# xxlong0/NeuralUDF

Measured on AMD Instinct MI355X. Metric: ray-samples/sec (train step), higher is better.
Workload: dtype f32 emulated on the 16-bit matrix pipe, f32 accumulate, f32 state / epilogues / optimizer.  Forward-order sweeps (UDF value, input gradient, colour / NeRF forward): f16x2 (x = hi + 2^-11 lo in fp16, 3 fp16 MFMA products, correction terms in their own accumulator).  Backward sweeps (tangent, adjoint

## Files before the change

include/nudf.h:

```cpp
#ifndef NUDF_H
#define NUDF_H
#include <stdint.h>

#ifdef __cplusplus
extern "C" {
#endif

int nudf_version(void);
const char* nudf_last_error(void);

enum {
  NUDF_STATUS_NONFINITE_RENDER = 1,
  NUDF_STATUS_NONFINITE_SAMPLES = 2,
  NUDF_STATUS_NONFINITE_LOSS = 4
};
int nudf_set_status_flag(int32_t* device_word);
int32_t* nudf_status_flag(void);

enum {
  NUDF_EPI_NONE = 0,
  NUDF_EPI_SOFTPLUS = 1,
  NUDF_EPI_RELU = 2,
  NUDF_EPI_MUL = 3,
  NUDF_EPI_MULMASK = 4,
// ... 10 lines not shown
typedef struct NudfGemmNN {
  const float* A; int32_t lda;
  const float* B; int32_t ldb;
  const float* bias;
  float* C1; int32_t ldc1;
  float* C2; int32_t ldc2;
  float* C3; int32_t ldc3;
  const float* X1; int32_t ldx1;
  const float* X2; int32_t ldx2;
  int32_t M, N, K;
  int32_t epi;
  int32_t iparam;
  float scale;
  float xscale;
} NudfGemmNN;

int nudf_gemm_nn(const NudfGemmNN* args, void* stream);
int nudf_set_gemm_variant(int variant);

typedef struct NudfGemmTN {
  const float* A1; int32_t lda1; int32_t na1;
  const float* B1; int32_t ldb1;
  const float* A2; int32_t lda2; int32_t na2;
  const float* B2; int32_t ldb2;
  float* C; int32_t ldc;
  float* dbias;
  int32_t M, NA, NB;
  int32_t rows_per_block;
  int32_t prec;
} NudfGemmTN;

int nudf_gemm_tn(const NudfGemmTN* args, void* stream);

#define NUDF_TN_MAX_PROBLEMS 12
typedef struct NudfGemmTNProblem {
  const float* A1; const float* B1;
  float* C; float* dbias;
  int32_t lda1, ldb1, ldc, NA, NB;
  int32_t tile_start;
  int32_t flags;
} NudfGemmTNProblem;
#define NUDF_TN_A16 1
#define NUDF_TN_B16 2
#define NUDF_TN_A_BLK 4
#define NUDF_TN_B_BLK 8
#define NUDF_TN_A_P4 16
#define NUDF_TN_B_P4 32
typedef struct NudfGemmTNGroup {
  int32_t n_problems, M, rows_per_block, total_tiles;
  int32_t prec;
  NudfGemmTNProblem prob[NUDF_TN_MAX_PROBLEMS];
  float* workspace;
  int64_t workspace_floats;
  int32_t assign;
  const float* amax_a;
  const float* amax_b;
} NudfGemmTNGroup;
int nudf_gemm_tn_grouped(const NudfGemmTNGroup* args, void* stream);
int64_t nudf_gemm_tn_grouped_workspace(const NudfGemmTNGroup* args);
int nudf_gemm_tn_grouped_plan(const NudfGemmTNGroup* args, int32_t* out, int capacity);
int nudf_set_tn_flags(int flags);
int nudf_set_tn_debug(void* buf);


typedef struct NudfComposite {
  const float* rays_o; const float* rays_d;
  const float* z;
  const float* udf;
  const float* grad;
  const float* color;
  const float* color_base;
  const float* bg_z;
  const float* bg_sigma;
  const float* bg_color;
  const float* scal;
  const float* sample_dist;
  const float* background_rgb;
  int32_t N, S, n_out, s_nominal;
  int32_t has_anneal; float cos_anneal;
  float flip_saturation;
  int32_t use_norm_grad;
  float sparse_scale;
  int32_t alpha_type;
  float* weights;
  float* out_color; float* out_color_base;
  float* out_depth;
  float* out_normals;
  float* out_wsum; float* out_wsum_all;
  float* sums;
  float* ws;
  float* o_alpha; float* o_alpha_plus; float* o_alpha_minus; float* o_vis_prob;
  float* o_alpha_occ; float* o_raw_occ; float* o_true_cos; float* o_grad_mag;
  float* o_mid_z; float* o_dists; float* o_inside; float* o_flip;
  const float* sched;
  const float* p_variance; const float* p_beta; const float* p_gamma;
  float beta_hi;
  int32_t defer_sums;
  float* scal_out; float* recip_out;
} NudfComposite;

typedef struct NudfCompositeGrad {
  const float* d_color; const float* d_color_base;
  const float* d_weights;
  const float* d_depth;
  const float* d_normals;
  const float* d_wsum; const float* d_wsum_all;
  const float* d_sums;
  float* o_d_udf;
  float* o_d_grad;
  float* o_d_color; float* o_d_color_base;
  float* o_d_bg_sigma;
  float* o_d_bg_color;
  float* o_d_scal;
  float* ws;
  float* o_d_param;
} NudfCompositeGrad;

int nudf_composite_fwd(const NudfComposite* args, void* stream);
int nudf_composite_bwd(const NudfComposite* args, const NudfCompositeGrad* grads, void* stream);
int nudf_partial_sums(const float* ws, int nblk, int K, float* out, void* stream);
int nudf_composite_colour_finish(const float* sums_color, const float* sums_color_base, int N, int S,
                                 const float* background_rgb, const float* wsum_all, float* out_color,
                                 float* out_color_base, void* stream);
void nudf_set_composite_blocked(int on);

typedef struct NudfUpsample {
  const float* rays_o; const float* rays_d;
  const float* z; const float* udf;
  const float* u;
  const float* sample_dist;
  const float* gamma_dev;
  int32_t N, M, K, mode;
  float inv_s, beta, gamma;
  float* z_new;
  float* pts_new;
  float* dbg;
  const float* prev_z; const float* prev_udf;
  const float* add_z; const float* add_udf;
  float* z_merged; float* udf_merged;
  int32_t merge_K;
} NudfUpsample;
#define NUDF_UP_DBG_ROWS 7
#define NUDF_UP_THEORICAL 256
#define NUDF_UP_SERIAL 512
#define NUDF_UP_NOCONTRACT 1024
#define NUDF_UP_SLEEF 2048
#define NUDF_UP_EXPCR 4096
int nudf_upsample(const NudfUpsample* args, void* stream);
int nudf_merge(const float* z, const float* udf, const float* z_new, const float* udf_new, int N, int M,
               int K, float* z_out, float* udf_out, void* stream);
int nudf_merge_points(const float* z, const float* z_new, int N, int M, int K, float* z_out, const float* rays_o,
                      const float* rays_d, const float* sample_dist, float* pts, float* xrows, int ldx, int xcols,
                      void* stream);

typedef struct NudfPixelBlend {
  const float* pts;
  const float* logits; int32_t nl;
  const float* proj;
  const float* imgs;
  int32_t P, V, H, W;
  float* pix;
  int32_t img_layout;
} NudfPixelBlend;
int nudf_pixel_blend_fwd(const NudfPixelBlend* a, void* stream);
int nudf_pixel_blend_bwd(const NudfPixelBlend* a, const float* d_pix, float* d_logits, void* stream);

typedef struct NudfPixelComposite {
  const float* w;
  const float* pix;
  const float* pts;
  const float* bg_in;
  const float* bg_tail;
  int32_t N, S, n_out;
  float* out;
} NudfPixelComposite;
int nudf_pixel_composite_fwd(const NudfPixelComposite* a, void* stream);
int nudf_pixel_composite_bwd(const NudfPixelComposite* a, const float* d_out, float* d_w, float* d_pix,
                             float* d_bg_in, float* d_bg_tail, void* stream);

typedef struct NudfPatchBlend {
  const float* pts;
  const float* grad;
  const float* rays_d;
  const float* uv;
  const float* logits; int32_t nl;
  const float* w; int32_t ldw;
  const float* ref_cam;
  const float* src_cam;
  const float* imgs;
  int32_t N, S, V, H, W, hps;
  float* patch_colors;
  float* patch_mask;
  int32_t img_layout;
} NudfPatchBlend;
int nudf_patch_blend_fwd(const NudfPatchBlend* a, void* stream);
int nudf_patch_blend_bwd(const NudfPatchBlend* a, const float* d_patch, float* d_logits, float* d_w, void* stream);

int nudf_pixel_warp(const NudfPixelBlend* a , float* colors ,
                    float* mask , void* stream);
typedef struct NudfPatchWarp {
  const float* pts;
  const float* normals;
  const float* uv;
  const float* ref_cam;
  const float* src_cam;
  const float* imgs;
  int32_t N, S, V, H, W, hps, img_layout;
  float* colors;
  float* mask;
} NudfPatchWarp;
int nudf_patch_warp(const NudfPatchWarp* a, void* stream);

int nudf_ssim_patch(const float* pred, const float* gt, const float* window, int N, int Npx, float* out,
                    const float* d_out, float* d_pred, void* stream);
int nudf_patch_metric(int type, const float* pred, const float* gt, const float* window, int N, int Npx, float* out,
                      const float* d_out, float* d_pred, void* stream);

typedef struct NudfBlendLoss {
  const float* cb; const float* c; const float* pix; const float* gt;
  const float* err;
  const float* patch_mask;
  const float* weight_sum;
  const float* err_sorted;
  const int64_t* order;
  float* m;
  float* err_masked;
  float* sums;
  const float* sums_ws;
  const float* w_dev;
  float* out;
  const float* d_total;
  float* d_cb; float* d_c; float* d_pix;
  float* d_err;
  float* d_sums;
  int32_t N, sums_nblk;
  float n_rays, trim_ratio;
} NudfBlendLoss;
int nudf_blend_loss_prepare(const NudfBlendLoss* args, void* stream);
int nudf_blend_loss_fwd(const NudfBlendLoss* args, void* stream);
int nudf_blend_loss_bwd(const NudfBlendLoss* args, void* stream);

int nudf_coarse_z(const float* near, const float* far, int nf_stride, const float* t_rand, int N, int S,
                  float* z, float* sample_dist, void* stream);
int nudf_coarse_start(const float* near, const float* far, int nf_stride, const float* t_rand, int center, int N, int S,
                      float* z, float* sample_dist, const float* rays_o, const float* rays_d, float* pts, void* stream);
int nudf_outside_z(const float* far, int f_stride, const float* lin, int N, int n_out, int n_samples,
                   float* z_out, void* stream);
int nudf_ray_points(const float* rays_o, const float* rays_d, const float* z, const float* sample_dist, int N,
                    int S, int mode, float* pts, void* stream);

int nudf_posenc(const float* x, int xld, int xdiv, const float* tangent, int D, int L, float in_scale, int P,
                float* dst1, int ld1, float scale1, float* dst2, int ld2, float scale2, void* stream);
int nudf_posenc_vjp(const float* x, int xld, int D, int L, float in_scale, int P, const float* src1, int ld1,
                    float scale1, const float* src2, int ld2, float scale2, float* g, void* stream);
int nudf_copy_cols(const float* src, int lds, int sdiv, float* dst, int ldd, int ncols, int P, float scale,
                   void* stream);
int nudf_add_cols(const float* a, int lda, const float* b, int ldb, float* out, int ldo, int P, int C, void* stream);

int nudf_udf_grad_seed(const float* sign, const float* w_row0, const float* h, int ldh, float hscale, int P, int C,
                       float inv_scale, float* out, int ldo, void* stream);
int nudf_udf_head_bwd(const float* sign, const float* dudf, const float* dfeat, int ldf, int P, int F,
                      float scale, float* out, int ldo, void* stream);
int nudf_signed_colsum(const float* sign, const float* R, int ldr, int P, int C, float scale, float* out,
                       void* stream);
int nudf_sigmoid_head_bwd(const float* y, const float* dy, const float* dy_extra, int ldx, int nsig,
                          const float* draw, int ldr, int nraw, int P, float* out, int ldo, void* stream);

int nudf_weightnorm_pack(const float* v, const float* g, int out, int in, const int* perm, float* W, int ldw,
                         float* Wt, int ldwt, float* inv_norm, void* stream);
int nudf_weightnorm_unpack_grad(const float* dW, int ldw, const float* v, const float* g, const float* inv_norm,
                                int out, int in, const int* perm, float* dv, float* dg, void* stream);

#define NUDF_ADAM_MAX_TENSORS 64
#define NUDF_ADAM_MAX_GROUPS 4
typedef struct NudfAdamTensor {
  float* p; const float* g; float* m; float* v;
  int32_t n;
  int32_t group;
  float neg_step_size;
  float bc2_sqrt;
} NudfAdamTensor;
typedef struct NudfAdamGroup {
  float one_minus_beta1, beta2, one_minus_beta2, eps;
} NudfAdamGroup;
typedef struct NudfAdam {
  int32_t n_tensors; int32_t pad_;
  NudfAdamTensor t[NUDF_ADAM_MAX_TENSORS];
  int32_t block_start[NUDF_ADAM_MAX_TENSORS + 1];
  int32_t pad2_;
  NudfAdamGroup group[NUDF_ADAM_MAX_GROUPS];
  const float* dyn;
} NudfAdam;
int nudf_adam_step(const NudfAdam* args, void* stream);
int nudf_adam_chunk(void);

enum {
  NUDF_CH_NONE = 0,
  NUDF_CH_SOFTPLUS = 1,
  NUDF_CH_MULSP = 2,
  NUDF_CH_TANGENT = 3,
  NUDF_CH_BWD = 4,
  NUDF_CH_UDFHEAD = 5,
  NUDF_CH_RELU = 6,
  NUDF_CH_SIGMOIDN = 7,
  NUDF_CH_MULMASK = 8,
  NUDF_CH_ADDMASK = 9,
  NUDF_CH_RELUADD = 10
};
enum {
  NUDF_CH_INIT_LOAD = 0,
  NUDF_CH_INIT_POSENC = 1,
  NUDF_CH_INIT_SEED = 2
};
#define NUDF_CH_MAX_STEPS 14
typedef struct NudfChainStep {
  const float* Bp;
  const float* bias;
  const float* X1; const float* X2;
  float* C1; float* C2;
  const float* r1_row;
  const float* r1_col;
  int32_t K, N;
  int32_t epi;
  int32_t iparam;
  int32_t ldx1, ldx2, ldc1, ldc2;
  int32_t ldr1;
  int32_t prec;
  int32_t act_write;
  int32_t act_col0;
  int32_t pe_tail_col;
  int32_t ld_pe;
  float* pe_dst;
  float pe_tail_scale;
  float scale, xscale;
  int32_t layout;
  const float* row_w;
  float* row_sums;
  const float* X3;
  int32_t ldx3;
} NudfChainStep;
#define NUDF_CH_BLK_X1 1
#define NUDF_CH_BLK_X2 2
#define NUDF_CH_BLK_C1 4
#define NUDF_CH_BLK_C2 8
#define NUDF_CH_BLK_PE 16
#define NUDF_CH_STATE16 32
#define NUDF_CH_P4_X1 64
#define NUDF_CH_P4_C1 128
typedef struct NudfChain {
  int32_t P, n_steps;
  int32_t init;
  int32_t k0;
  int32_t x_div;
  int32_t tile_rows;
  int32_t lda0, ldg0;
  int32_t pe_L, pe_jvp;
  int32_t init_state16;
  float pe_in_scale;
  float seed_scale, seed_xscale;
  const float* A0;
  float* G0;
  const float* x;
  const float* v;
  const float* seed_sign;
  const float* seed_wrow;
  unsigned long long* dbg;
  float* absmax_out;
  const float* tile_amax_in;
  float* tile_amax_out;
  int32_t tile_scale;
  int32_t reserved0;
  NudfChainStep step[NUDF_CH_MAX_STEPS];
} NudfChain;
int nudf_mlp_chain(const NudfChain* args, void* stream);
int nudf_set_chain_t16(int on);
int nudf_pack_frag(const float* B, int ldb, int K, int N, float* out, void* stream);

#define NUDF_PACK_MAX_LAYERS 16
#define NUDF_PACK_MAX_FRAGS 4
typedef struct NudfPackFrag {
  float* dst;
  int32_t transpose;
  int32_t o0, i0;
  int32_t K, N;
  int32_t dtype;
} NudfPackFrag;
typedef struct NudfPackLayer {
  const float* v; const float* g;
  const int32_t* perm;
  float* W; float* Wt;
  float* inv_norm;
  int32_t out, in, ldw, ldwt;
  int32_t nfrag, row_start;
  NudfPackFrag frag[NUDF_PACK_MAX_FRAGS];
} NudfPackLayer;
typedef struct NudfPackMulti {
  int32_t n_layers, total_rows;
  NudfPackLayer layer[NUDF_PACK_MAX_LAYERS];
// ... 188 lines not shown
```

neuraludf_amd/_lib.py:

```python
from __future__ import annotations

import ctypes as C
import os

import torch

_HERE = os.path.dirname(os.path.abspath(__file__))
LIB_PATH = os.environ.get("NUDF_LIB") or os.path.join(_HERE, "libnudf.so")
ABI_VERSION = 108

c_fp = C.c_void_p
i32 = C.c_int32
f32 = C.c_float


class NudfError(RuntimeError):
    pass


class GemmNN(C.Structure):
    _fields_ = [("A", c_fp), ("lda", i32), ("B", c_fp), ("ldb", i32), ("bias", c_fp),
                ("C1", c_fp), ("ldc1", i32), ("C2", c_fp), ("ldc2", i32), ("C3", c_fp), ("ldc3", i32),
                ("X1", c_fp), ("ldx1", i32), ("X2", c_fp), ("ldx2", i32),
                ("M", i32), ("N", i32), ("K", i32), ("epi", i32), ("iparam", i32), ("scale", f32), ("xscale", f32)]


class GemmTN(C.Structure):
    _fields_ = [("A1", c_fp), ("lda1", i32), ("na1", i32), ("B1", c_fp), ("ldb1", i32),
                ("A2", c_fp), ("lda2", i32), ("na2", i32), ("B2", c_fp), ("ldb2", i32),
                ("C", c_fp), ("ldc", i32), ("dbias", c_fp), ("M", i32), ("NA", i32), ("NB", i32),
                ("rows_per_block", i32), ("prec", i32)]


TN_MAX_PROBLEMS = 12


class GemmTNProblem(C.Structure):
    _fields_ = [("A1", c_fp), ("B1", c_fp), ("C", c_fp), ("dbias", c_fp), ("lda1", i32), ("ldb1", i32), ("ldc", i32),
                ("NA", i32), ("NB", i32), ("tile_start", i32), ("flags", i32)]


class GemmTNGroup(C.Structure):
    _fields_ = [("n_problems", i32), ("M", i32), ("rows_per_block", i32), ("total_tiles", i32), ("prec", i32),
                ("prob", GemmTNProblem * TN_MAX_PROBLEMS), ("workspace", c_fp), ("workspace_floats", C.c_int64),
                ("assign", i32), ("amax_a", c_fp), ("amax_b", c_fp)]


class BlendLoss(C.Structure):
    _fields_ = [("cb", c_fp), ("c", c_fp), ("pix", c_fp), ("gt", c_fp), ("err", c_fp), ("patch_mask", c_fp),
                ("weight_sum", c_fp), ("err_sorted", c_fp), ("order", c_fp), ("m", c_fp), ("err_masked", c_fp), ("sums", c_fp),
                ("sums_ws", c_fp), ("w_dev", c_fp), ("out", c_fp), ("d_total", c_fp), ("d_cb", c_fp), ("d_c", c_fp),
                ("d_pix", c_fp), ("d_err", c_fp), ("d_sums", c_fp), ("N", i32), ("sums_nblk", i32), ("n_rays", f32),
                ("trim_ratio", f32)]


class RayBatch(C.Structure):
    _fields_ = [("image", c_fp), ("mask", c_fp), ("intrinsics_inv", c_fp), ("pose", c_fp), ("pixels_x", c_fp),
                ("pixels_y", c_fp), ("N", i32), ("H", i32), ("W", i32), ("h_patch_size", i32), ("rays", c_fp),
                ("ndc_uv", c_fp), ("xyz_cam", c_fp), ("near", c_fp), ("far", c_fp), ("patch_color", c_fp),
                ("patch_mask", c_fp)]


class Composite(C.Structure):
    _fields_ = [("rays_o", c_fp), ("rays_d", c_fp), ("z", c_fp), ("udf", c_fp), ("grad", c_fp),
                ("color", c_fp), ("color_base", c_fp), ("bg_z", c_fp), ("bg_sigma", c_fp), ("bg_color", c_fp),
                ("scal", c_fp), ("sample_dist", c_fp), ("background_rgb", c_fp),
                ("N", i32), ("S", i32), ("n_out", i32), ("s_nominal", i32),
                ("has_anneal", i32), ("cos_anneal", f32), ("flip_saturation", f32),
                ("use_norm_grad", i32), ("sparse_scale", f32), ("alpha_type", i32),
                ("weights", c_fp), ("out_color", c_fp), ("out_color_base", c_fp), ("out_depth", c_fp),
                ("out_normals", c_fp), ("out_wsum", c_fp), ("out_wsum_all", c_fp), ("sums", c_fp), ("ws", c_fp),
                ("o_alpha", c_fp), ("o_alpha_plus", c_fp), ("o_alpha_minus", c_fp), ("o_vis_prob", c_fp),
                ("o_alpha_occ", c_fp), ("o_raw_occ", c_fp), ("o_true_cos", c_fp), ("o_grad_mag", c_fp),
                ("o_mid_z", c_fp), ("o_dists", c_fp), ("o_inside", c_fp), ("o_flip", c_fp), ("sched", c_fp),
                ("p_variance", c_fp), ("p_beta", c_fp), ("p_gamma", c_fp), ("beta_hi", f32), ("defer_sums", i32),
                ("scal_out", c_fp), ("recip_out", c_fp)]


class CompositeGrad(C.Structure):
    _fields_ = [("d_color", c_fp), ("d_color_base", c_fp), ("d_weights", c_fp), ("d_depth", c_fp),
                ("d_normals", c_fp), ("d_wsum", c_fp), ("d_wsum_all", c_fp), ("d_sums", c_fp),
                ("o_d_udf", c_fp), ("o_d_grad", c_fp), ("o_d_color", c_fp), ("o_d_color_base", c_fp),
                ("o_d_bg_sigma", c_fp), ("o_d_bg_color", c_fp), ("o_d_scal", c_fp), ("ws", c_fp), ("o_d_param", c_fp)]


class Upsample(C.Structure):
    _fields_ = [("rays_o", c_fp), ("rays_d", c_fp), ("z", c_fp), ("udf", c_fp), ("u", c_fp),
                ("sample_dist", c_fp), ("gamma_dev", c_fp),
                ("N", i32), ("M", i32), ("K", i32), ("mode", i32),
                ("inv_s", f32), ("beta", f32), ("gamma", f32),
                ("z_new", c_fp), ("pts_new", c_fp), ("dbg", c_fp),
                ("prev_z", c_fp), ("prev_udf", c_fp), ("add_z", c_fp), ("add_udf", c_fp),
                ("z_merged", c_fp), ("udf_merged", c_fp), ("merge_K", i32)]


class PixelBlend(C.Structure):
    _fields_ = [("pts", c_fp), ("logits", c_fp), ("nl", i32), ("proj", c_fp), ("imgs", c_fp),
                ("P", i32), ("V", i32), ("H", i32), ("W", i32), ("pix", c_fp), ("img_layout", i32)]


class PixelComposite(C.Structure):
    _fields_ = [("w", c_fp), ("pix", c_fp), ("pts", c_fp), ("bg_in", c_fp), ("bg_tail", c_fp),
                ("N", i32), ("S", i32), ("n_out", i32), ("out", c_fp)]


class PatchBlend(C.Structure):
    _fields_ = [("pts", c_fp), ("grad", c_fp), ("rays_d", c_fp), ("uv", c_fp), ("logits", c_fp), ("nl", i32),
                ("w", c_fp), ("ldw", i32), ("ref_cam", c_fp), ("src_cam", c_fp), ("imgs", c_fp),
                ("N", i32), ("S", i32), ("V", i32), ("H", i32), ("W", i32), ("hps", i32),
                ("patch_colors", c_fp), ("patch_mask", c_fp), ("img_layout", i32)]


class PatchWarp(C.Structure):
    _fields_ = [("pts", c_fp), ("normals", c_fp), ("uv", c_fp), ("ref_cam", c_fp), ("src_cam", c_fp), ("imgs", c_fp),
                ("N", i32), ("S", i32), ("V", i32), ("H", i32), ("W", i32), ("hps", i32), ("img_layout", i32),
                ("colors", c_fp), ("mask", c_fp)]


ADAM_MAX_TENSORS = 64
ADAM_MAX_GROUPS = 4


class AdamTensor(C.Structure):
    _fields_ = [("p", c_fp), ("g", c_fp), ("m", c_fp), ("v", c_fp), ("n", i32), ("group", i32), ("neg_step_size", f32), ("bc2_sqrt", f32)]


class AdamGroup(C.Structure):
    _fields_ = [("one_minus_beta1", f32), ("beta2", f32), ("one_minus_beta2", f32), ("eps", f32)]


class Adam(C.Structure):
    _fields_ = [("n_tensors", i32), ("pad_", i32), ("t", AdamTensor * ADAM_MAX_TENSORS),
                ("block_start", i32 * (ADAM_MAX_TENSORS + 1)), ("pad2_", i32), ("group", AdamGroup * ADAM_MAX_GROUPS),
                ("dyn", c_fp)]


CH_MAX_STEPS = 14
CH_STATE16 = 32
CH_P4_X1, CH_P4_C1 = 64, 128
CH = dict(NONE=0, SOFTPLUS=1, MULSP=2, TANGENT=3, BWD=4, UDFHEAD=5, RELU=6, SIGMOIDN=7, MULMASK=8, ADDMASK=9, RELUADD=10)
CH_INIT = dict(LOAD=0, POSENC=1, SEED=2)


class ChainStep(C.Structure):
    _fields_ = [("Bp", c_fp), ("bias", c_fp), ("X1", c_fp), ("X2", c_fp), ("C1", c_fp), ("C2", c_fp),
                ("r1_row", c_fp), ("r1_col", c_fp), ("K", i32), ("N", i32), ("epi", i32), ("iparam", i32),
                ("ldx1", i32), ("ldx2", i32), ("ldc1", i32), ("ldc2", i32), ("ldr1", i32), ("prec", i32), ("act_write", i32),
                ("act_col0", i32), ("pe_tail_col", i32), ("ld_pe", i32), ("pe_dst", c_fp), ("pe_tail_scale", f32),
                ("scale", f32), ("xscale", f32), ("layout", i32), ("row_w", c_fp), ("row_sums", c_fp), ("X3", c_fp),
                ("ldx3", i32)]


class Chain(C.Structure):
    _fields_ = [("P", i32), ("n_steps", i32), ("init", i32), ("k0", i32), ("x_div", i32), ("tile_rows", i32), ("lda0", i32),
                ("ldg0", i32), ("pe_L", i32), ("pe_jvp", i32), ("init_state16", i32), ("pe_in_scale", f32), ("seed_scale", f32),
                ("seed_xscale", f32), ("A0", c_fp), ("G0", c_fp), ("x", c_fp), ("v", c_fp), ("seed_sign", c_fp),
                ("seed_wrow", c_fp), ("dbg", c_fp), ("absmax_out", c_fp), ("tile_amax_in", c_fp),
                ("tile_amax_out", c_fp), ("tile_scale", C.c_int32), ("reserved0", C.c_int32), ("step", ChainStep * CH_MAX_STEPS)]


PACK_MAX_LAYERS = 16
PACK_MAX_FRAGS = 4


class PackFrag(C.Structure):
    _fields_ = [("dst", c_fp), ("transpose", i32), ("o0", i32), ("i0", i32), ("K", i32), ("N", i32), ("dtype", i32)]


class PackLayer(C.Structure):
    _fields_ = [("v", c_fp), ("g", c_fp), ("perm", c_fp), ("W", c_fp), ("Wt", c_fp), ("inv_norm", c_fp),
                ("out", i32), ("in_", i32), ("ldw", i32), ("ldwt", i32), ("nfrag", i32), ("row_start", i32),
                ("frag", PackFrag * PACK_MAX_FRAGS)]


class PackMulti(C.Structure):
    _fields_ = [("n_layers", i32), ("total_rows", i32), ("layer", PackLayer * PACK_MAX_LAYERS)]


class UnpackLayer(C.Structure):
    _fields_ = [("dW", c_fp), ("v", c_fp), ("g", c_fp), ("inv_norm", c_fp), ("perm", c_fp), ("dv", c_fp),
                ("dg", c_fp), ("db_in", c_fp), ("db_out", c_fp), ("out", i32), ("in_", i32), ("ldw", i32), ("row_start", i32)]


class UnpackMulti(C.Structure):
    _fields_ = [("n_layers", i32), ("total_rows", i32), ("layer", UnpackLayer * PACK_MAX_LAYERS)]


class MeshUDF(C.Structure):
    _fields_ = [("U", c_fp), ("G", c_fp), ("axes", c_fp), ("cell_case", c_fp), ("cell_ntri", c_fp), ("edge_flag", c_fp),
                ("cells", c_fp), ("face_off", c_fp), ("edge_scan", c_fp), ("faces", c_fp), ("edges", c_fp), ("verts", c_fp),
                ("n_cells", C.c_int64), ("n_edges", C.c_int64), ("n_faces", C.c_int64), ("N", i32), ("mean_thr", f32),
                ("max_thr", f32), ("pad_", i32)]


class PointCloud(C.Structure):
    _fields_ = [("verts", c_fp), ("faces", c_fp), ("tri_n", c_fp), ("tri_off", c_fp), ("out", c_fp),
                ("n_verts", C.c_int64), ("n_faces", C.c_int64), ("n_out", C.c_int64), ("out_base", C.c_int64),
                ("cap", C.c_int64), ("density", C.c_double),
                ("pts", c_fp), ("n", C.c_int64), ("origin", C.c_double * 3), ("cell", C.c_double), ("grid", i32 * 3),
                ("pad_", i32), ("keys", c_fp), ("cell_key", c_fp), ("cell_start", c_fp), ("cell_count", c_fp),
                ("n_cells", C.c_int64), ("hash_key", c_fp), ("hash_row", c_fp), ("hash_cap", C.c_int64),
                ("rank", c_fp), ("state", c_fp), ("undecided", c_fp), ("r2", C.c_double),
                ("query", c_fp), ("query_idx", c_fp), ("n_query", C.c_int64), ("bound", C.c_double),
                ("box_bound2", C.c_double), ("box_lo", C.c_double * 3), ("box_hi", C.c_double * 3),
                ("dist", c_fp), ("idx", c_fp)]


class MeshTopo(C.Structure):
    _fields_ = [("faces", c_fp), ("he_key", c_fp), ("he_id", c_fp), ("edge_start", c_fp), ("edges", c_fp), ("he_edge", c_fp),
                ("edge_key", c_fp), ("nbr_off", c_fp), ("nbr", c_fp), ("bverts", c_fp), ("new_count", c_fp), ("new_off", c_fp),
                ("new_faces", c_fp), ("pos", c_fp), ("pos_out", c_fp), ("labels", c_fp), ("changed", c_fp), ("proj", c_fp),
                ("masks", c_fp), ("vis_count", c_fp), ("n_faces", C.c_int64), ("n_verts", C.c_int64), ("n_edges", C.c_int64),
                ("n_bverts", C.c_int64), ("n_new", C.c_int64), ("lam", C.c_double), ("max_loop", i32), ("n_views", i32),
                ("H", i32), ("W", i32), ("border", i32), ("pad_", i32)]


LW = dict(color_base=0, color=1, color_pixel=2, color_patch=3, igr=4, igr_ns=5, sparse=6, mask=7, color_sum=8)
LW_COUNT = 16

EPI = dict(NONE=0, SOFTPLUS=1, RELU=2, MUL=3, MULMASK=4, TANGENT=5, BWD=6, SIGMOID=7, UDFHEAD=8,
           SKIPSPLIT=9, RELU_DUAL=10, ADDMASK=11, MULSP=12)

SYMBOLS = [
    "nudf_version", "nudf_last_error", "nudf_set_status_flag", "nudf_status_flag", "nudf_gemm_nn", "nudf_set_gemm_variant", "nudf_gemm_tn", "nudf_gemm_tn_grouped", "nudf_gemm_tn_grouped_workspace", "nudf_gemm_tn_grouped_plan", "nudf_set_tn_flags", "nudf_patch_metric", "nudf_set_tn_debug", "nudf_composite_fwd",
    "nudf_composite_bwd", "nudf_partial_sums", "nudf_composite_colour_finish", "nudf_set_composite_blocked", "nudf_upsample", "nudf_merge", "nudf_merge_points", "nudf_coarse_z", "nudf_coarse_start", "nudf_outside_z",
    "nudf_ray_points", "nudf_posenc", "nudf_posenc_vjp", "nudf_copy_cols", "nudf_add_cols",
    "nudf_udf_grad_seed", "nudf_udf_head_bwd", "nudf_signed_colsum", "nudf_sigmoid_head_bwd",
    "nudf_weightnorm_pack", "nudf_weightnorm_unpack_grad",
    "nudf_pixel_blend_fwd", "nudf_pixel_blend_bwd", "nudf_pixel_composite_fwd", "nudf_pixel_composite_bwd",
    "nudf_patch_blend_fwd", "nudf_patch_blend_bwd", "nudf_ssim_patch", "nudf_pixel_warp", "nudf_patch_warp",
    "nudf_adam_step", "nudf_adam_chunk", "nudf_mlp_chain", "nudf_set_chain_t16", "nudf_pack_frag",
    "nudf_weightnorm_pack_multi", "nudf_weightnorm_unpack_grad_multi",
    "nudf_scalars_fwd", "nudf_scalars_bwd", "nudf_l1_sum_fwd", "nudf_l1_sum_bwd",
    "nudf_sums_errors_fwd", "nudf_sums_errors_bwd", "nudf_color_loss_fwd", "nudf_color_loss_bwd",
    "nudf_gen_ray_batch", "nudf_color_loss_sums", "nudf_color_loss_finish",
    "nudf_step_loss_fwd", "nudf_step_loss_bwd", "nudf_col0_seed4",
    "nudf_blend_loss_prepare", "nudf_blend_loss_fwd", "nudf_blend_loss_bwd",
    "nudf_meshudf_classify", "nudf_meshudf_emit", "nudf_meshudf_vertices",
    "nudf_pc_tri_count", "nudf_pc_tri_emit", "nudf_pc_keys", "nudf_pc_cells", "nudf_pc_thin_round", "nudf_pc_nearest",
    "nudf_meshtopo_edges", "nudf_meshtopo_fill_count", "nudf_meshtopo_fill_emit", "nudf_meshtopo_smooth",
    "nudf_meshtopo_cc_hook", "nudf_meshtopo_cc_jump", "nudf_meshtopo_views",
]

_P, _I, _F = C.c_void_p, C.c_int, C.c_float
_ARGTYPES = {
    "nudf_gemm_nn": [C.POINTER(GemmNN), _P],
    "nudf_gemm_tn": [C.POINTER(GemmTN), _P],
    "nudf_gemm_tn_grouped": [C.POINTER(GemmTNGroup), _P],
    "nudf_gemm_tn_grouped_workspace": [C.POINTER(GemmTNGroup)],
    "nudf_gemm_tn_grouped_plan": [C.POINTER(GemmTNGroup), C.POINTER(C.c_int32), i32],
    "nudf_set_tn_flags": [i32],
    "nudf_set_tn_debug": [_P],
    "nudf_composite_fwd": [C.POINTER(Composite), _P],
    "nudf_composite_bwd": [C.POINTER(Composite), C.POINTER(CompositeGrad), _P],
    "nudf_partial_sums": [_P, _I, _I, _P, _P],
    "nudf_composite_colour_finish": [_P, _P, _I, _I, _P, _P, _P, _P, _P],
    "nudf_upsample": [C.POINTER(Upsample), _P],
    "nudf_merge": [_P, _P, _P, _P, _I, _I, _I, _P, _P, _P],
    "nudf_coarse_z": [_P, _P, _I, _P, _I, _I, _P, _P, _P],
    "nudf_coarse_start": [_P, _P, _I, _P, _I, _I, _I, _P, _P, _P, _P, _P, _P],
    "nudf_merge_points": [_P, _P, _I, _I, _I, _P, _P, _P, _P, _P, _P, _I, _I, _P],
    "nudf_outside_z": [_P, _I, _P, _I, _I, _I, _P, _P],
    "nudf_ray_points": [_P, _P, _P, _P, _I, _I, _I, _P, _P],
    "nudf_posenc": [_P, _I, _I, _P, _I, _I, _F, _I, _P, _I, _F, _P, _I, _F, _P],
    "nudf_posenc_vjp": [_P, _I, _I, _I, _F, _I, _P, _I, _F, _P, _I, _F, _P, _P],
    "nudf_copy_cols": [_P, _I, _I, _P, _I, _I, _I, _F, _P],
    "nudf_add_cols": [_P, _I, _P, _I, _P, _I, _I, _I, _P],
    "nudf_udf_grad_seed": [_P, _P, _P, _I, _F, _I, _I, _F, _P, _I, _P],
    "nudf_udf_head_bwd": [_P, _P, _P, _I, _I, _I, _F, _P, _I, _P],
    "nudf_signed_colsum": [_P, _P, _I, _I, _I, _F, _P, _P],
    "nudf_sigmoid_head_bwd": [_P, _P, _P, _I, _I, _P, _I, _I, _I, _P, _I, _P],
    "nudf_weightnorm_pack": [_P, _P, _I, _I, _P, _P, _I, _P, _I, _P, _P],
    "nudf_weightnorm_unpack_grad": [_P, _I, _P, _P, _P, _I, _I, _P, _P, _P, _P],
    "nudf_pixel_blend_fwd": [C.POINTER(PixelBlend), _P],
    "nudf_pixel_blend_bwd": [C.POINTER(PixelBlend), _P, _P, _P],
    "nudf_pixel_composite_fwd": [C.POINTER(PixelComposite), _P],
    "nudf_pixel_composite_bwd": [C.POINTER(PixelComposite), _P, _P, _P, _P, _P, _P],
    "nudf_patch_blend_fwd": [C.POINTER(PatchBlend), _P],
    "nudf_patch_blend_bwd": [C.POINTER(PatchBlend), _P, _P, _P, _P],
    "nudf_pixel_warp": [C.POINTER(PixelBlend), _P, _P, _P],
    "nudf_patch_warp": [C.POINTER(PatchWarp), _P],
    "nudf_ssim_patch": [_P, _P, _P, _I, _I, _P, _P, _P, _P],
    "nudf_patch_metric": [_I] + [_P, _P, _P, _I, _I, _P, _P, _P, _P],
    "nudf_adam_step": [C.POINTER(Adam), _P],
    "nudf_mlp_chain": [C.POINTER(Chain), _P],
    "nudf_pack_frag": [_P, _I, _I, _I, _P, _P],
    "nudf_weightnorm_pack_multi": [C.POINTER(PackMulti), _P],
    "nudf_weightnorm_unpack_grad_multi": [C.POINTER(UnpackMulti), _P],
    "nudf_scalars_fwd": [_P, _P, _P, _F, _P, _P, _P],
    "nudf_scalars_bwd": [_P, _P, _P, _F, _P, _P, _P],
    "nudf_l1_sum_fwd": [_P, _P, _I, _P, _P],
    "nudf_l1_sum_bwd": [_P, _P, _I, _P, _P, _P],
    "nudf_sums_errors_fwd": [_P, _F, _P, _P],
    "nudf_sums_errors_bwd": [_P, _F, _P, _P, _P],
    "nudf_color_loss_fwd": [_P, _P, _P, _I, _P, _I, _F, _F, _F, _P, _P, _P, _P],
    "nudf_color_loss_bwd": [_P, _P, _P, _I, _P, _F, _F, _F, _P, _P, _P, _P, _P],
    "nudf_gen_ray_batch": [C.POINTER(RayBatch), _P],
    "nudf_color_loss_sums": [_P, _P, _P, _I, _P, _I, _P, _P],
    "nudf_color_loss_finish": [_P, _I, _F, _F, _F, _P, _P, _P, _P],
    "nudf_step_loss_fwd": [_P, _P, _P, _I, _P, _I, _P, _F, _F, _F, _F, _F, _F, _F, _P, _P, _P, _P, _I, _P],
    "nudf_step_loss_bwd": [_P, _P, _P, _I, _P, _P, _F, _F, _F, _F, _F, _F, _F, _P, _P, _P, _P, _P, _P, _P],
    "nudf_col0_seed4": [_P, _P, _F, _I, _I, _P, _P, _P],
    "nudf_blend_loss_prepare": [C.POINTER(BlendLoss), _P],
    "nudf_blend_loss_fwd": [C.POINTER(BlendLoss), _P],
    "nudf_blend_loss_bwd": [C.POINTER(BlendLoss), _P],
    "nudf_meshudf_classify": [C.POINTER(MeshUDF), _P],
    "nudf_meshudf_emit": [C.POINTER(MeshUDF), _P],
    "nudf_meshudf_vertices": [C.POINTER(MeshUDF), _P],
    **{n: [C.POINTER(PointCloud), _P] for n in ("nudf_pc_tri_count", "nudf_pc_tri_emit", "nudf_pc_keys", "nudf_pc_cells",
                                                "nudf_pc_thin_round", "nudf_pc_nearest")},
    **{n: [C.POINTER(MeshTopo), _P] for n in ("nudf_meshtopo_edges", "nudf_meshtopo_fill_count", "nudf_meshtopo_fill_emit",
                                              "nudf_meshtopo_smooth", "nudf_meshtopo_cc_hook", "nudf_meshtopo_cc_jump",
                                              "nudf_meshtopo_views")},
}

_lib = None


def _bind(l):
    for name, at in _ARGTYPES.items():
        fn = getattr(l, name)
        fn.argtypes = at
        fn.restype = C.c_int


def lib():
    global _lib
    if _lib is None:
        if not os.path.exists(LIB_PATH):
            raise NudfError(
                f"{LIB_PATH} not found: build it with `python -m neuraludf_amd.build` "
                "(the NeuralUDF hot path has no CPU/PyTorch fallback)")
        try:
            _lib = C.CDLL(LIB_PATH)
        except OSError as e:
            raise NudfError(f"cannot load {LIB_PATH}: {e}") from e
        _lib.nudf_last_error.restype = C.c_char_p
        _lib.nudf_version.restype = C.c_int
        _lib.nudf_adam_chunk.restype = C.c_int
        if _lib.nudf_version() != ABI_VERSION:
            v, _lib = _lib.nudf_version(), None
            raise NudfError(f"{LIB_PATH} is ABI version {v}, this package binds {ABI_VERSION}: rebuild with "
                            "`python -m neuraludf_amd.build --force`")
        _bind(_lib)
        _lib.nudf_gemm_tn_grouped_workspace.restype = C.c_int64
        _lib.nudf_set_chain_t16.argtypes = [C.c_int]
        _lib.nudf_set_chain_t16.restype = C.c_int
        _lib.nudf_set_status_flag.argtypes = [C.c_void_p]
        _lib.nudf_set_status_flag.restype = C.c_int
        _lib.nudf_status_flag.argtypes = []
        _lib.nudf_status_flag.restype = C.c_void_p
    return _lib


STATUS_NONFINITE_RENDER, STATUS_NONFINITE_SAMPLES, STATUS_NONFINITE_LOSS = 1, 2, 4
_STATUS_WORDS = {}
_STATUS_BOUND = None


def bind_status(dev):
    global _STATUS_BOUND
    if dev.type != "cuda":
        raise NudfError("libnudf kernels need device tensors (got a CPU tensor): run on an MI355X")
    idx = dev.index if dev.index is not None else torch.cuda.current_device()
    if _STATUS_BOUND == idx:
        return _STATUS_WORDS[idx]
    w = _STATUS_WORDS.get(idx)
    if w is None:
        w = torch.zeros(1, dtype=torch.int32, device=torch.device("cuda", idx))
        _STATUS_WORDS[idx] = w
    check(lib().nudf_set_status_flag(C.c_void_p(w.data_ptr())), "nudf_set_status_flag")
    _STATUS_BOUND = idx
    return w


def read_status(dev, clear=False):
    w = bind_status(dev)
    v = int(w.item())
    if clear and v:
        w.zero_()
    return v


def status_text(bits):
    names = [(STATUS_NONFINITE_SAMPLES, "non-finite new samples in the hierarchical re-sampling (nudf_upsample)"),
             (STATUS_NONFINITE_RENDER, "non-finite composited ray outputs or renderer scalars (nudf_composite_fwd)"),
             (STATUS_NONFINITE_LOSS, "non-finite loss (nudf_step_loss_fwd)")]
    return "; ".join(t for b, t in names if bits & b) or "finite"


def ptr(t):
    if t is None:
        return None
    if not t.is_cuda:
        raise NudfError("libnudf kernels need device tensors (got a CPU tensor): run on an MI355X")
    if not t.is_contiguous():
        raise NudfError("libnudf kernels need contiguous tensors")
    return t.data_ptr()


HOST_FAST = os.environ.get("NUDF_HOST_FAST", "1") != "0"
_raw_stream = getattr(torch._C, "_cuda_getCurrentRawStream", None)
_raw_device = getattr(torch._C, "_cuda_getDevice", None)


def stream():
    if HOST_FAST and _raw_stream is not None and _raw_device is not None:
        return C.c_void_p(_raw_stream(_raw_device()))
    return C.c_void_p(torch.cuda.current_stream().cuda_stream)


def check(rc, what=""):
    if rc != 0:
        msg = lib().nudf_last_error()
# ... 14 lines not shown
```

neuraludf_amd/csrc/rays_embed.hip:

```cpp
#include "nudf_common.h"
#include "../../include/nudf.h"

static inline int nblocks(long long n, int bs) { return (int)((n + bs - 1) / bs); }

__global__ void coarse_z_kernel(const float* near, const float* far, int nf_stride, const float* t_rand,
                                int N, int S, float* z) {
  int idx = blockIdx.x * blockDim.x + threadIdx.x;
  if (idx >= N * S) return;
  int r = idx / S, s = idx - r * S;
  float nr = near[r * nf_stride], fr = far[r * nf_stride];
  float step = 1.0f / (float)(S - 1);
  float t = (s < S / 2) ? s * step : 1.0f - (S - 1 - s) * step;
  float v = nr + (fr - nr) * t;
  if (t_rand) v = v + t_rand[r] * 2.0f / (float)S;
  z[idx] = v;
}

__global__ void sample_dist_kernel(const float* near, const float* far, int n, int S, float* out) {
  __shared__ float red[256];
  float acc = 0.f;
  for (int i = threadIdx.x; i < n; i += blockDim.x) acc += (far[i] - near[i]) / (float)S;
  red[threadIdx.x] = acc;
  __syncthreads();
  for (int s = 128; s > 0; s >>= 1) {
    if (threadIdx.x < s) red[threadIdx.x] += red[threadIdx.x + s];
    __syncthreads();
  }
  if (threadIdx.x == 0) out[0] = red[0] / (float)n;
}

extern "C" int nudf_coarse_z(const float* near, const float* far, int nf_stride, const float* t_rand, int N, int S,
                             float* z, float* sample_dist, void* stream) {
  hipStream_t st = (hipStream_t)stream;
  hipLaunchKernelGGL(coarse_z_kernel, dim3(nblocks((long long)N * S, 256)), dim3(256), 0, st, near, far, nf_stride,
                     t_rand, N, S, z);
  if (sample_dist)
    hipLaunchKernelGGL(sample_dist_kernel, dim3(1), dim3(256), 0, st, near, far, nf_stride ? N : 1, S, sample_dist);
  NUDF_CHECK_LAUNCH("nudf_coarse_z");
  return 0;
}

__global__ __launch_bounds__(256) void coarse_start_kernel(const float* near, const float* far, int nf_stride,
                                                           const float* t_rand, int center, int N, int S, float* z,
                                                           float* sample_dist, const float* __restrict__ o,
                                                           const float* __restrict__ d, float* __restrict__ pts) {
  const int idx = blockIdx.x * blockDim.x + threadIdx.x;
  if (idx < N * S) {
    const int r = idx / S, s = idx - r * S;
    const float nr = near[r * nf_stride], fr = far[r * nf_stride];
    const float step = 1.0f / (float)(S - 1);
    const float t = (s < S / 2) ? s * step : 1.0f - (S - 1 - s) * step;
    float v = nr + (fr - nr) * t;
    if (t_rand) {
      const float tr = center ? __fsub_rn(t_rand[r], 0.5f) : t_rand[r];
      v = v + tr * 2.0f / (float)S;
    }
    z[idx] = v;
    if (pts) {
      pts[(size_t)idx * 3 + 0] = o[r * 3 + 0] + d[r * 3 + 0] * v;
      pts[(size_t)idx * 3 + 1] = o[r * 3 + 1] + d[r * 3 + 1] * v;
      pts[(size_t)idx * 3 + 2] = o[r * 3 + 2] + d[r * 3 + 2] * v;
    }
  }
  if (blockIdx.x == 0 && sample_dist) {
    __shared__ float red[256];
    const int n = nf_stride ? N : 1;
    float acc = 0.f;
    for (int i = threadIdx.x; i < n; i += 256) acc += (far[i] - near[i]) / (float)S;
    red[threadIdx.x] = acc;
    __syncthreads();
    for (int s = 128; s > 0; s >>= 1) {
      if (threadIdx.x < s) red[threadIdx.x] += red[threadIdx.x + s];
      __syncthreads();
    }
    if (threadIdx.x == 0) sample_dist[0] = red[0] / (float)n;
  }
}
extern "C" int nudf_coarse_start(const float* near, const float* far, int nf_stride, const float* t_rand, int center, int N,
                                 int S, float* z, float* sample_dist, const float* rays_o, const float* rays_d, float* pts,
                                 void* stream) {
  if (N <= 0 || S < 2) {
    nudf_set_error("nudf_coarse_start: N >= 1 and S >= 2 required", hipErrorInvalidValue);
    return (int)hipErrorInvalidValue;
  }
  hipLaunchKernelGGL(coarse_start_kernel, dim3(nblocks((long long)N * S, 256)), dim3(256), 0, (hipStream_t)stream, near, far,
                     nf_stride, t_rand, center, N, S, z, sample_dist, rays_o, rays_d, pts);
  NUDF_CHECK_LAUNCH("nudf_coarse_start");
  return 0;
}

__global__ void outside_z_kernel(const float* far, int f_stride, const float* lin, int N, int n_out, float inv_ns,
                                 float* z_out) {
  int idx = blockIdx.x * blockDim.x + threadIdx.x;
  if (idx >= N * n_out) return;
  int r = idx / n_out, j = idx - r * n_out;
  z_out[idx] = far[r * f_stride] / lin[n_out - 1 - j] + inv_ns;
}
extern "C" int nudf_outside_z(const float* far, int f_stride, const float* lin, int N, int n_out, int n_samples,
                              float* z_out, void* stream) {
  hipLaunchKernelGGL(outside_z_kernel, dim3(nblocks((long long)N * n_out, 256)), dim3(256), 0, (hipStream_t)stream,
                     far, f_stride, lin, N, n_out, 1.0f / (float)n_samples, z_out);
  NUDF_CHECK_LAUNCH("nudf_outside_z");
  return 0;
}

__global__ void ray_points_kernel(const float* __restrict__ o, const float* __restrict__ d, const float* __restrict__ z,
                                  const float* sample_dist, int N, int S, int mode, float* __restrict__ pts) {
  int idx = blockIdx.x * blockDim.x + threadIdx.x;
  if (idx >= N * S) return;
  int r = idx / S, s = idx - r * S;
  float t = z[idx];
  if (mode >= 1) {
    float dist = (s < S - 1) ? (z[idx + 1] - t) : sample_dist[0];
    t = t + dist * 0.5f;
  }
  float px = o[r * 3 + 0] + d[r * 3 + 0] * t;
  float py = o[r * 3 + 1] + d[r * 3 + 1] * t;
  float pz = o[r * 3 + 2] + d[r * 3 + 2] * t;
  if (mode == 2) {
    float rr = sqrtf(px * px + py * py + pz * pz);
    rr = fminf(fmaxf(rr, 1.0f), 1e10f);
    pts[(size_t)idx * 4 + 0] = px / rr;
    pts[(size_t)idx * 4 + 1] = py / rr;
    pts[(size_t)idx * 4 + 2] = pz / rr;
    pts[(size_t)idx * 4 + 3] = 1.0f / rr;
  } else {
    pts[(size_t)idx * 3 + 0] = px;
    pts[(size_t)idx * 3 + 1] = py;
    pts[(size_t)idx * 3 + 2] = pz;
  }
}
extern "C" int nudf_ray_points(const float* rays_o, const float* rays_d, const float* z, const float* sample_dist, int N,
                               int S, int mode, float* pts, void* stream) {
  if (N * S == 0) return 0;
  hipLaunchKernelGGL(ray_points_kernel, dim3(nblocks((long long)N * S, 256)), dim3(256), 0, (hipStream_t)stream, rays_o,
                     rays_d, z, sample_dist, N, S, mode, pts);
  NUDF_CHECK_LAUNCH("nudf_ray_points");
  return 0;
}

__global__ void posenc_kernel(const float* __restrict__ x, int xld, int xdiv, const float* __restrict__ v, int D, int L,
                              float in_scale, int P, float* d1, int ld1, float s1, float* d2, int ld2, float s2,
                              int mode) {
  const int E = D * (2 * L + 1);
  long long idx = (long long)blockIdx.x * blockDim.x + threadIdx.x;
  if (idx >= (long long)P * E) return;
  int p = (int)(idx / E), e = (int)(idx - (long long)p * E);
  int blk = e / D, j = e - blk * D;
  float xv = x[(size_t)(p / xdiv) * xld + j] * in_scale;
  float val;
  if (blk == 0) {
    val = (mode == 0) ? xv : v[(size_t)p * D + j] * in_scale;
  } else {
    int k = (blk - 1) >> 1;
    float f = (float)(1 << k);
    float a = xv * f;
    bool is_sin = ((blk - 1) & 1) == 0;
    if (mode == 0) val = is_sin ? sinf(a) : cosf(a);
    else val = (is_sin ? cosf(a) : -sinf(a)) * f * v[(size_t)p * D + j] * in_scale;
  }
  if (d1) d1[(size_t)p * ld1 + e] = val * s1;
  if (d2) d2[(size_t)p * ld2 + e] = val * s2;
}
extern "C" int nudf_posenc(const float* x, int xld, int xdiv, const float* tangent, int D, int L, float in_scale, int P,
                           float* dst1, int ld1, float scale1, float* dst2, int ld2, float scale2, void* stream) {
  if (P == 0) return 0;
  const int E = D * (2 * L + 1);
  hipLaunchKernelGGL(posenc_kernel, dim3(nblocks((long long)P * E, 256)), dim3(256), 0, (hipStream_t)stream, x, xld,
                     xdiv, tangent, D, L, in_scale, P, dst1, ld1, scale1, dst2, ld2, scale2, tangent ? 1 : 0);
  NUDF_CHECK_LAUNCH("nudf_posenc");
  return 0;
}

#define PV_PTS 64
#define PV_MAXE 96
__global__ __launch_bounds__(256) void posenc_vjp_kernel(const float* __restrict__ x, int xld, int D, int L,
                                                         float in_scale, int P, const float* __restrict__ s1, int ld1,
                                                         float c1, const float* __restrict__ s2, int ld2, float c2,
                                                         float* __restrict__ g) {
  __shared__ float de[PV_PTS][PV_MAXE + 1];
  const int E = D * (2 * L + 1);
  const int p0 = blockIdx.x * PV_PTS;
  for (int idx = threadIdx.x; idx < PV_PTS * E; idx += 256) {
    const int r = idx / E, e = idx - r * E;
    const int p = min(p0 + r, P - 1);
    float t = 0.f;
    if (s1) t += s1[(size_t)p * ld1 + e] * c1;
    if (s2) t += s2[(size_t)p * ld2 + e] * c2;
    de[r][e] = t;
  }
  __syncthreads();
  for (int idx = threadIdx.x; idx < PV_PTS * D; idx += 256) {
    const int r = idx / D, j = idx - r * D;
    const int p = p0 + r;
    if (p >= P) continue;
    const float xv = x[(size_t)p * xld + j] * in_scale;
    float acc = de[r][j];
    for (int k = 0; k < L; ++k) {
      const float f = (float)(1 << k);
      float sn, cs;
      sincosf(xv * f, &sn, &cs);
      acc += f * (de[r][D * (1 + 2 * k) + j] * cs - de[r][D * (2 + 2 * k) + j] * sn);
    }
    g[(size_t)p * D + j] = acc * in_scale;
  }
}
extern "C" int nudf_posenc_vjp(const float* x, int xld, int D, int L, float in_scale, int P, const float* src1, int ld1,
                               float scale1, const float* src2, int ld2, float scale2, float* g, void* stream) {
  if (P == 0) return 0;
  if (D * (2 * L + 1) > PV_MAXE) {
    nudf_set_error("nudf_posenc_vjp: encoding wider than 96", hipErrorInvalidValue);
    return (int)hipErrorInvalidValue;
  }
  hipLaunchKernelGGL(posenc_vjp_kernel, dim3(nblocks(P, PV_PTS)), dim3(256), 0, (hipStream_t)stream, x, xld, D, L,
                     in_scale, P, src1, ld1, scale1, src2, ld2, scale2, g);
  NUDF_CHECK_LAUNCH("nudf_posenc_vjp");
  return 0;
}

__global__ void copy_cols_kernel(const float* __restrict__ src, int lds, int sdiv, float* __restrict__ dst, int ldd,
                                 int ncols, int P, float scale) {
  long long idx = (long long)blockIdx.x * blockDim.x + threadIdx.x;
  if (idx >= (long long)P * ncols) return;
  int p = (int)(idx / ncols), c = (int)(idx - (long long)p * ncols);
  dst[(size_t)p * ldd + c] = src[(size_t)(p / sdiv) * lds + c] * scale;
}
extern "C" int nudf_copy_cols(const float* src, int lds, int sdiv, float* dst, int ldd, int ncols, int P, float scale,
                              void* stream) {
  if (P == 0) return 0;
  hipLaunchKernelGGL(copy_cols_kernel, dim3(nblocks((long long)P * ncols, 256)), dim3(256), 0, (hipStream_t)stream, src,
                     lds, sdiv, dst, ldd, ncols, P, scale);
  NUDF_CHECK_LAUNCH("nudf_copy_cols");
  return 0;
}

__global__ void udf_grad_seed_kernel(const float* __restrict__ sign, const float* __restrict__ wrow,
                                     const float* __restrict__ h, int ldh, float hscale, int P, int C,
                                     float inv_scale, float* __restrict__ out, int ldo) {
  long long idx = (long long)blockIdx.x * blockDim.x + threadIdx.x;
  if (idx >= (long long)P * C) return;
// ... 904 lines not shown
```

neuraludf_amd/csrc/upsample.hip:

```cpp
#include "nudf_common.h"
#include "../../include/nudf.h"

#define UP_MAX_M 512
#define UP_NC (UP_MAX_M / 64)

namespace up_fast {
#include "upsample_body.inc"
}
#pragma clang fp contract(off)
namespace up_exact {
#include "upsample_body.inc"
}
#pragma clang fp contract(fast)

extern "C" int nudf_upsample(const NudfUpsample* args, void* stream) {
  const NudfUpsample& p = *args;
  if (p.N <= 0) return 0;
  if (p.M < 2 || p.M > UP_MAX_M || p.K < 1) {
    nudf_set_error("nudf_upsample: 2 <= M <= 512 and K >= 1 required", hipErrorInvalidValue);
    return (int)hipErrorInvalidValue;
  }
  if (p.merge_K < 0 || p.merge_K >= p.M ||
      (p.merge_K > 0 && (!p.prev_z || !p.prev_udf || !p.add_z || !p.add_udf || !p.z_merged || !p.udf_merged))) {
    nudf_set_error("nudf_upsample: merge_K in [0, M) with all six merge arrays required", hipErrorInvalidValue);
    return (int)hipErrorInvalidValue;
  }
  dim3 grid((p.N + 3) / 4), block(256);
  hipStream_t st = (hipStream_t)stream;
  const int nc = (p.M + 63) / 64;
  int32_t* status = nudf_status_flag();
  if (p.mode & NUDF_UP_NOCONTRACT) {
    switch (nc) {
      case 1: hipLaunchKernelGGL(up_exact::upsample_kernel<1>, grid, block, 0, st, p, status); break;
      case 2: hipLaunchKernelGGL(up_exact::upsample_kernel<2>, grid, block, 0, st, p, status); break;
      case 3: hipLaunchKernelGGL(up_exact::upsample_kernel<3>, grid, block, 0, st, p, status); break;
      case 4: hipLaunchKernelGGL(up_exact::upsample_kernel<4>, grid, block, 0, st, p, status); break;
      default: hipLaunchKernelGGL(up_exact::upsample_kernel<8>, grid, block, 0, st, p, status); break;
    }
  } else {
    switch (nc) {
      case 1: hipLaunchKernelGGL(up_fast::upsample_kernel<1>, grid, block, 0, st, p, status); break;
      case 2: hipLaunchKernelGGL(up_fast::upsample_kernel<2>, grid, block, 0, st, p, status); break;
      case 3: hipLaunchKernelGGL(up_fast::upsample_kernel<3>, grid, block, 0, st, p, status); break;
      case 4: hipLaunchKernelGGL(up_fast::upsample_kernel<4>, grid, block, 0, st, p, status); break;
      default: hipLaunchKernelGGL(up_fast::upsample_kernel<8>, grid, block, 0, st, p, status); break;
    }
  }
  NUDF_CHECK_LAUNCH("nudf_upsample");
  return 0;
}

__global__ __launch_bounds__(256) void merge_kernel(const float* __restrict__ za, const float* __restrict__ ua,
                                                    const float* __restrict__ zb, const float* __restrict__ ub, int N,
                                                    int M, int K, float* __restrict__ zo, float* __restrict__ uo) {
  extern __shared__ float sm[];
  const int wave = threadIdx.x >> 6, l = threadIdx.x & 63;
  const int ray = blockIdx.x * 4 + wave;
  if (ray >= N) return;
  float* a = sm + wave * (M + K);
  float* b = a + M;
  for (int i = l; i < M; i += 64) a[i] = za[(size_t)ray * M + i];
  for (int j = l; j < K; j += 64) b[j] = zb[(size_t)ray * K + j];
  __builtin_amdgcn_wave_barrier();
  __threadfence_block();
  const size_t ob = (size_t)ray * (M + K);
  for (int i = l; i < M; i += 64) {
    const float v = a[i];
    int lo = 0, hi = K;
    while (lo < hi) {
      const int mid = (lo + hi) >> 1;
      if (b[mid] < v) lo = mid + 1; else hi = mid;
    }
    zo[ob + i + lo] = v;
    if (uo) uo[ob + i + lo] = ua[(size_t)ray * M + i];
  }
  for (int j = l; j < K; j += 64) {
    const float v = b[j];
    int lo = 0, hi = M;
    while (lo < hi) {
      const int mid = (lo + hi) >> 1;
      if (a[mid] <= v) lo = mid + 1; else hi = mid;
    }
    zo[ob + j + lo] = v;
    if (uo) uo[ob + j + lo] = ub[(size_t)ray * K + j];
  }
}

extern "C" int nudf_merge(const float* z, const float* udf, const float* z_new, const float* udf_new, int N, int M,
                          int K, float* z_out, float* udf_out, void* stream) {
  if (N <= 0) return 0;
  const size_t lds = (size_t)4 * (M + K) * sizeof(float);
  if (lds > 64 * 1024) {
    nudf_set_error("nudf_merge: M + K too large", hipErrorInvalidValue);
    return (int)hipErrorInvalidValue;
  }
  hipLaunchKernelGGL(merge_kernel, dim3((N + 3) / 4), dim3(256), lds, (hipStream_t)stream, z, udf, z_new, udf_new, N, M,
                     K, z_out, udf_out);
  NUDF_CHECK_LAUNCH("nudf_merge");
  return 0;
}

__global__ __launch_bounds__(256) void merge_points_kernel(const float* __restrict__ za, const float* __restrict__ zb,
                                                           int N, int M, int K, float* __restrict__ zo,
                                                           const float* __restrict__ ro, const float* __restrict__ rd,
                                                           const float* __restrict__ sample_dist,
                                                           float* __restrict__ pts, float* __restrict__ xrows, int ldx,
                                                           int xcols) {
  extern __shared__ float sm[];
  const int wave = threadIdx.x >> 6, l = threadIdx.x & 63;
  const int ray = blockIdx.x * 4 + wave;
  if (ray >= N) return;
  const int S = M + K;
  float* a = sm + wave * (5 * S);
  float* b = a + M;
  float* out = a + S;
  float* pl = out + S;
  for (int i = l; i < M; i += 64) a[i] = za[(size_t)ray * M + i];
  for (int j = l; j < K; j += 64) b[j] = zb[(size_t)ray * K + j];
  __builtin_amdgcn_wave_barrier();
  __threadfence_block();
  for (int i = l; i < M; i += 64) {
    const float v = a[i];
    int lo = 0, hi = K;
    while (lo < hi) {
      const int mid = (lo + hi) >> 1;
      if (b[mid] < v) lo = mid + 1; else hi = mid;
    }
    out[i + lo] = v;
  }
  for (int j = l; j < K; j += 64) {
    const float v = b[j];
    int lo = 0, hi = M;
    while (lo < hi) {
      const int mid = (lo + hi) >> 1;
      if (a[mid] <= v) lo = mid + 1; else hi = mid;
    }
    out[j + lo] = v;
  }
  __builtin_amdgcn_wave_barrier();
  __threadfence_block();
  const float ox = ro[ray * 3 + 0], oy = ro[ray * 3 + 1], oz = ro[ray * 3 + 2];
  const float dx = rd[ray * 3 + 0], dy = rd[ray * 3 + 1], dz = rd[ray * 3 + 2];
  const float sd = sample_dist[0];
  const size_t ob = (size_t)ray * S;
  for (int i = l; i < S; i += 64) {
    float t = out[i];
    zo[ob + i] = t;
    const float dist = (i < S - 1) ? (out[i + 1] - t) : sd;
    t = t + dist * 0.5f;
    const float px = ox + dx * t, py = oy + dy * t, pz = oz + dz * t;
    pts[(ob + i) * 3 + 0] = px;
    pts[(ob + i) * 3 + 1] = py;
    pts[(ob + i) * 3 + 2] = pz;
    pl[3 * i + 0] = px; pl[3 * i + 1] = py; pl[3 * i + 2] = pz;
  }
  if (xrows) {
    __builtin_amdgcn_wave_barrier();
    __threadfence_block();
    for (int e = l; e < S * xcols; e += 64) {
      const int r = e / xcols, c = e - r * xcols;
      xrows[(ob + r) * (size_t)ldx + c] = (c < 3) ? pl[3 * r + c] : 0.0f;
    }
  }
}

extern "C" int nudf_merge_points(const float* z, const float* z_new, int N, int M, int K, float* z_out, const float* rays_o,
                                 const float* rays_d, const float* sample_dist, float* pts, float* xrows, int ldx, int xcols,
                                 void* stream) {
  if (N <= 0) return 0;
  const size_t lds = (size_t)4 * 5 * (M + K) * sizeof(float);
  if (lds > 64 * 1024 || M < 1 || K < 0 || (xrows && (xcols < 3 || xcols > ldx))) {
    nudf_set_error("nudf_merge_points: M + K <= 819, 3 <= xcols <= ldx required", hipErrorInvalidValue);
    return (int)hipErrorInvalidValue;
  }
  hipLaunchKernelGGL(merge_points_kernel, dim3((N + 3) / 4), dim3(256), lds, (hipStream_t)stream, z, z_new, N, M, K, z_out,
                     rays_o, rays_d, sample_dist, pts, xrows, ldx, xcols);
  NUDF_CHECK_LAUNCH("nudf_merge_points");
  return 0;
}
```

neuraludf_amd/csrc/upsample_body.inc:

```
__device__ __forceinline__ float clip01u(float x) { return fminf(fmaxf(x, 0.0f), 1.0f); }

__device__ __forceinline__ float sleef_expf_u10(float d) {
  const int q = __float2int_rn(__fmul_rn(d, 1.442695040888963407359924681001892137426645954152985934135449406931f));
  const float qf = (float)q;
  float s = __fmaf_rn(qf, -0.693145751953125f, d);
  s = __fmaf_rn(qf, -1.428606765330187045e-06f, s);
  float u = 0.000198527617612853646278381f;
  u = __fmaf_rn(u, s, 0.00139304355252534151077271f);
  u = __fmaf_rn(u, s, 0.00833336077630519866943359f);
  u = __fmaf_rn(u, s, 0.0416664853692054748535156f);
  u = __fmaf_rn(u, s, 0.166666671633720397949219f);
  u = __fmaf_rn(u, s, 0.5f);
  u = __fadd_rn(1.0f, __fmaf_rn(__fmul_rn(s, s), u, s));
  const int e1 = q >> 1, e2 = q - e1;
  u = __fmul_rn(__fmul_rn(u, __int_as_float((e1 + 127) << 23)), __int_as_float((e2 + 127) << 23));
  if (d < -104.0f) u = 0.0f;
  if (d > 100.0f) u = __int_as_float(0x7f800000);
  return u;
}
__device__ __forceinline__ float up_sigmoid(float x, bool sleef) {
  return sleef ? __fdiv_rn(1.0f, __fadd_rn(1.0f, sleef_expf_u10(-x))) : sigmoidf_(x);
}

__device__ __forceinline__ float up_exp(float x, bool cr) { return cr ? (float)exp((double)x) : expf(x); }

__device__ __forceinline__ float sdf2alpha_plain(float sdf, float cosv, float dist, float inv_s, int theorical, bool sleef,
                                                 bool expcr) {
  if (theorical) {
    const float raw = fabsf(cosv) * inv_s * (1.0f - up_sigmoid(sdf * inv_s, sleef));
    return 1.0f - up_exp(-fmaxf(raw, 0.0f) * dist, expcr);
  }
  const float en = sdf + cosv * dist * 0.5f;
  const float ep = sdf - cosv * dist * 0.5f;
  const float P = up_sigmoid(ep * inv_s, sleef);
  const float Nx = up_sigmoid(en * inv_s, sleef);
  return clip01u((P - Nx + 1e-5f) / (P + 1e-5f));
}

__device__ __forceinline__ void up_serial_excl_prod(float* buf, int n, int lane) {
  __builtin_amdgcn_wave_barrier();
  __threadfence_block();
  if (lane == 0) {
    double acc = 1.0;
    int i = 0;
#pragma unroll 2
    for (; i + 4 <= n; i += 4) {
      const float4 q = *reinterpret_cast<const float4*>(buf + i);
      float4 o;
      o.x = (float)acc; acc *= (double)q.x;
      o.y = (float)acc; acc *= (double)q.y;
      o.z = (float)acc; acc *= (double)q.z;
      o.w = (float)acc; acc *= (double)q.w;
      *reinterpret_cast<float4*>(buf + i) = o;
    }
    for (; i < n; ++i) {
      const float q = buf[i];
      buf[i] = (float)acc;
      acc *= (double)q;
    }
  }
  __builtin_amdgcn_wave_barrier();
  __threadfence_block();
}

template <int NC>
__global__ __launch_bounds__(256) void upsample_kernel(NudfUpsample p, int32_t* status) {
  __shared__ __attribute__((aligned(16))) float s_z[4][NC * 64];
  __shared__ __attribute__((aligned(16))) float s_cdf[4][NC * 64];
  __shared__ float s_u[4][NC * 64];
  const int wave = threadIdx.x >> 6, l = threadIdx.x & 63;
  const int ray = blockIdx.x * 4 + wave;
  if (ray >= p.N) return;
  const int M = p.M;
  float* zs = s_z[wave];
  float* cdf = s_cdf[wave];

  const float ox = p.rays_o[ray * 3 + 0], oy = p.rays_o[ray * 3 + 1], oz = p.rays_o[ray * 3 + 2];
  const float dx = p.rays_d[ray * 3 + 0], dy = p.rays_d[ray * 3 + 1], dz = p.rays_d[ray * 3 + 2];
  const float sdist = p.sample_dist[0];
  const float gamma = p.gamma_dev ? p.gamma_dev[0] : p.gamma;
  const bool serial = (p.mode & NUDF_UP_SERIAL) != 0;
  const bool sleef = (p.mode & NUDF_UP_SLEEF) != 0;
  const bool expcr = (p.mode & NUDF_UP_EXPCR) != 0;
  float* dbg = p.dbg ? p.dbg + (size_t)ray * NUDF_UP_DBG_ROWS * M : nullptr;

  const bool merged = p.merge_K > 0;
  if (merged) {
    const int K0 = p.merge_K, M0 = M - K0;
    float* a = cdf;
    float* b = cdf + M0;
    float* us = s_u[wave];
    for (int i = l; i < M0; i += 64) a[i] = p.prev_z[(size_t)ray * M0 + i];
    for (int j = l; j < K0; j += 64) b[j] = p.add_z[(size_t)ray * K0 + j];
    __builtin_amdgcn_wave_barrier();
    __threadfence_block();
    for (int i = l; i < M0; i += 64) {
      const float v = a[i];
      int lo = 0, hi = K0;
      while (lo < hi) {
        const int mid = (lo + hi) >> 1;
        if (b[mid] < v) lo = mid + 1; else hi = mid;
      }
      zs[i + lo] = v;
      us[i + lo] = p.prev_udf[(size_t)ray * M0 + i];
    }
    for (int j = l; j < K0; j += 64) {
      const float v = b[j];
      int lo = 0, hi = M0;
      while (lo < hi) {
        const int mid = (lo + hi) >> 1;
        if (a[mid] <= v) lo = mid + 1; else hi = mid;
      }
      zs[j + lo] = v;
      us[j + lo] = p.add_udf[(size_t)ray * K0 + j];
    }
    __builtin_amdgcn_wave_barrier();
    __threadfence_block();
  }
  float z[NC], u[NC], rad[NC];
#pragma unroll
  for (int c = 0; c < NC; ++c) {
    const int i = c * 64 + l;
    z[c] = 0.f; u[c] = 0.f; rad[c] = 1e30f;
    if (i < M) {
      if (merged) {
        z[c] = zs[i];
        u[c] = s_u[wave][i];
        p.z_merged[(size_t)ray * M + i] = z[c];
        p.udf_merged[(size_t)ray * M + i] = u[c];
      } else {
        z[c] = p.z[(size_t)ray * M + i];
        u[c] = p.udf[(size_t)ray * M + i];
      }
      const float px = ox + dx * z[c], py = oy + dy * z[c], pz = oz + dz * z[c];
      rad[c] = sqrtf(px * px + py * py + pz * pz);
      zs[i] = z[c];
    }
  }

  float w[NC];
  const int theorical = (p.mode >> 8) & 1;
  if ((p.mode & 0xff) == 1) {
#pragma unroll
    for (int c = 0; c < NC; ++c) {
      const int i = c * 64 + l;
      const float zo = (c + 1 < NC) ? wave_bcast(z[(c + 1 < NC) ? c + 1 : c], 0) : 0.f;
      const float zn = wave_shift_down1(z[c], zo);
      const float dist = (i < M - 1) ? (zn - z[c]) : sdist;
      const float e = up_exp(-p.beta * u[c], expcr);
      const float raw = p.beta * e / ((1.0f + e) * (1.0f + e)) * gamma;
      w[c] = (i < M - 1) ? (1.0f - up_exp(-fmaxf(raw, 0.0f) * dist, expcr)) : 0.0f;
    }
  } else {
    float tc[NC], cosv[NC], aocc[NC], dists[NC], midu[NC];
#pragma unroll
    for (int c = 0; c < NC; ++c) {
      const int i = c * 64 + l;
      const int cn = (c + 1 < NC) ? c + 1 : c;
      const float zo = wave_bcast(z[cn], 0), uo = wave_bcast(u[cn], 0), ro = wave_bcast(rad[cn], 0);
      const float zn = wave_shift_down1(z[c], zo), un = wave_shift_down1(u[c], uo), rn = wave_shift_down1(rad[c], ro);
      const bool sec = i < M - 1;
      dists[c] = sec ? (zn - z[c]) : 0.f;
      midu[c] = (u[c] + un) * 0.5f;
      tc[c] = sec ? (un - u[c]) / (zn - z[c] + 1e-5f) : 0.f;
      const bool inside = (rad[c] < 1.0f) || (rn < 1.0f);
      cosv[c] = inside ? 1.0f : 0.0f;
      const float draw = sec ? (zn - z[c]) : sdist;
      const float e = up_exp(-p.beta * u[c], expcr);
      const float raw = p.beta * e / ((1.0f + e) * (1.0f + e));
      aocc[c] = 1.0f - up_exp(-fmaxf(raw, 0.0f) * gamma * draw, expcr);
    }
    float carry = 1.0f;
    float vis[NC];
#pragma unroll
    for (int c = 0; c < NC; ++c) {
      const int i = c * 64 + l;
      const float cur = -fabsf(tc[c]);
      const int cp = (c > 0) ? c - 1 : c;
      const float prev_o = wave_bcast(-fabsf(tc[cp]), 63), tprev_o = wave_bcast(tc[cp], 63);
      const float prev = wave_shift_up1(cur, (c > 0) ? prev_o : 0.0f);
      const float tprev = wave_shift_up1(tc[c], tprev_o);
      const float inside = cosv[c];
      float cv = fminf(prev, cur);
      cv = fminf(fmaxf(cv, -1e3f), 0.0f) * inside;
      cosv[c] = cv;
      const float vm = (i == 0) ? 1.0f : ((tprev < 0.05f) ? 1.0f : 0.0f);
      const float q = (i < M) ? (clip01u(1.0f - aocc[c] + vm) + 1e-7f) : 1.0f;
      if (serial) {
        if (i < M) cdf[i] = q;
      } else {
        float inc = wave_incl_scan_mul(q) * carry;
        const float exc = wave_shift_up1(inc, carry);
        carry = wave_bcast(inc, 63);
        vis[c] = exc;
      }
    }
    if (serial) {
      up_serial_excl_prod(cdf, M, l);
#pragma unroll
      for (int c = 0; c < NC; ++c) vis[c] = (c * 64 + l < M) ? cdf[c * 64 + l] : 1.0f;
      __builtin_amdgcn_wave_barrier();
      __threadfence_block();
    }
    carry = 1.0f;
#pragma unroll
    for (int c = 0; c < NC; ++c) {
      const int i = c * 64 + l;
      float alpha = 0.f;
      if (i < M - 1) {
        const float ap = sdf2alpha_plain(midu[c], cosv[c], dists[c], p.inv_s, theorical, sleef, expcr);
        const float am = sdf2alpha_plain(-midu[c], cosv[c], dists[c], p.inv_s, theorical, sleef, expcr);
        alpha = ap * vis[c] + am * (1.0f - vis[c]);
        if (dbg) {
          dbg[0 * M + i] = cosv[c]; dbg[1 * M + i] = vis[c]; dbg[2 * M + i] = ap; dbg[3 * M + i] = am;
          dbg[4 * M + i] = alpha;
        }
      }
      const float f = (i < M - 1) ? (1.0f - alpha + 1e-7f) : 1.0f;
      if (serial) {
        if (i < M - 1) cdf[i] = f;
        w[c] = alpha;
      } else {
        float inc = wave_incl_scan_mul(f) * carry;
        const float exc = wave_shift_up1(inc, carry);
        carry = wave_bcast(inc, 63);
        w[c] = (i < M - 1) ? alpha * exc : 0.0f;
      }
    }
    if (serial) {
      up_serial_excl_prod(cdf, M - 1, l);
#pragma unroll
      for (int c = 0; c < NC; ++c) w[c] = (c * 64 + l < M - 1) ? w[c] * cdf[c * 64 + l] : 0.0f;
      __builtin_amdgcn_wave_barrier();
      __threadfence_block();
    }
  }

  float tot = 0.f;
#pragma unroll
  for (int c = 0; c < NC; ++c) {
    const int i = c * 64 + l;
    if (dbg && i < M - 1) dbg[5 * M + i] = w[c];
    w[c] = (i < M - 1) ? (w[c] + 1e-5f) : 0.0f;
    tot += w[c];
  }
  tot = wave_sum(tot);
  float scarry = 0.f;
  if (l == 0) cdf[0] = 0.f;
#pragma unroll
  for (int c = 0; c < NC; ++c) {
    const int i = c * 64 + l;
    const float pdf = w[c] / tot;
    if (serial) {
      if (i < M - 1) cdf[i + 1] = pdf;
    } else {
      float inc = wave_incl_scan_add(pdf) + scarry;
      scarry = wave_bcast(inc, 63);
      if (i < M - 1) cdf[i + 1] = inc;
    }
  }
  __builtin_amdgcn_wave_barrier();
  __threadfence_block();
  if (serial) {
    if (l == 0) {
      double acc = 0.0;
      int i = 1;
#pragma unroll 2
      for (; i + 4 <= M; i += 4) {
        const float a0 = cdf[i], a1 = cdf[i + 1], a2 = cdf[i + 2], a3 = cdf[i + 3];
        acc += (double)a0; const float o0 = (float)acc;
        acc += (double)a1; const float o1 = (float)acc;
        acc += (double)a2; const float o2 = (float)acc;
        acc += (double)a3; const float o3 = (float)acc;
        cdf[i] = o0; cdf[i + 1] = o1; cdf[i + 2] = o2; cdf[i + 3] = o3;
      }
      for (; i < M; ++i) {
        acc += (double)cdf[i];
        cdf[i] = (float)acc;
      }
    }
    __builtin_amdgcn_wave_barrier();
    __threadfence_block();
  }

  if (dbg)
    for (int i = l; i < M; i += 64) dbg[6 * M + i] = cdf[i];
  for (int k = l; k < p.K; k += 64) {
    const float uq = p.u[k];
    int lo = 0, hi = M;
    while (lo < hi) {
      const int mid = (lo + hi) >> 1;
      if (cdf[mid] <= uq) lo = mid + 1; else hi = mid;
    }
    const int below = max(lo - 1, 0);
    const int above = min(lo, M - 1);
    const float c0 = cdf[below], c1 = cdf[above];
    const float b0 = zs[below], b1 = zs[above];
    float den = c1 - c0;
    if (den < 1e-5f) den = 1.0f;
    const float t = (uq - c0) / den;
    const float zn = b0 + t * (b1 - b0);
    p.z_new[(size_t)ray * p.K + k] = zn;
    if (status && !(fabsf(zn) <= 3.0e38f)) atomicOr(status, NUDF_STATUS_NONFINITE_SAMPLES);
    if (p.pts_new) {
      const size_t o = ((size_t)ray * p.K + k) * 3;
      p.pts_new[o + 0] = ox + dx * zn;
      p.pts_new[o + 1] = oy + dy * zn;
      p.pts_new[o + 2] = oz + dz * zn;
    }
  }
}
```

neuraludf_amd/mlp.py:

```python
from __future__ import annotations

import math
from typing import List, Optional

import ctypes as C

import torch

from . import _lib
import os

from ._lib import CH, CH_INIT, CH_MAX_STEPS, EPI, Chain, GemmNN, GemmTN, call, ptr


def pad32(n: int) -> int:
    return (n + 31) // 32 * 32


def pad_rows(P: int) -> int:
    return (P + 63) // 64 * 64


def _buf(P, width, dev, zero=None, dtype=torch.float32, blocked=False):
    if blocked:
        assert zero is False and dtype == torch.float32
        t = torch.empty((pad_rows(P), pad32(width)), device=dev, dtype=dtype)
        t._nudf_blk = True
        return t
    ld = pad32(width)
    if dtype == torch.bfloat16:
        t = (torch.zeros if zero else torch.empty)((pad_rows(P), ld), device=dev, dtype=dtype)
        if zero is None and ld != width:
            t.view(pad_rows(P) // 4, ld, 4)[:, width:, :].zero_()
        t._nudf_p4 = True
        return t
    if zero is None:
        t = torch.empty((pad_rows(P), ld), device=dev, dtype=dtype)
        if ld != width:
            t[:, width:].zero_()
        return t
    return (torch.zeros if zero else torch.empty)((pad_rows(P), ld), device=dev, dtype=dtype)


def _is16(t):
    return t is not None and t.dtype == torch.bfloat16


def _isblk(t):
    return t is not None and getattr(t, "_nudf_blk", False)


def _isp4(t):
    return t is not None and getattr(t, "_nudf_p4", False)


def pack16(t):
    R, ld = t.shape
    assert R % 4 == 0
    b = t.to(torch.bfloat16).reshape(R // 4, 4, ld).permute(0, 2, 1).reshape(R, ld).contiguous()
    b._nudf_p4 = True
    return b


def unpack16(t):
    R, ld = t.shape
    assert _isp4(t) and R % 4 == 0
    return t.reshape(R // 4, ld, 4).permute(0, 2, 1).reshape(R, ld).float()


def block(t):
    R, ld = t.shape
    assert R % 32 == 0 and ld % 4 == 0 and t.dtype == torch.float32
    b = t.reshape(R // 32, 32, ld // 4, 4).permute(0, 2, 1, 3).reshape(R, ld).contiguous()
    b._nudf_blk = True
    return b


def unblock(t):
    if not _isblk(t):
        return t
    R, ld = t.shape
    return t.reshape(R // 32, ld // 4, 32, 4).permute(0, 2, 1, 3).reshape(R, ld).contiguous()


def _zero_cols(t, c0):
    if c0 < t.shape[1]:
        t[:, c0:].zero_()
    return t


def alloc_grads(layers, zero=True):
    sizes = [(pl.out_pad * pl.in_pad, pl.out_pad) for pl in layers]
    flat = (torch.zeros if zero else torch.empty)(sum(a + b for a, b in sizes), device=layers[0].W.device)
    out, off = [], 0
    for pl, (a, b) in zip(layers, sizes):
        dW = flat[off:off + a].view(pl.out_pad, pl.in_pad)
        db = flat[off + a:off + a + pl.out]
        out.append((dW, db))
        off += a + b
    return out


def gemm_nn(A, B, M, N, K, epi, C1=None, ldc1=0, C2=None, ldc2=0, C3=None, ldc3=0, X1=None, ldx1=0, X2=None, ldx2=0,
            bias=None, lda=None, ldb=None, iparam=0, scale=1.0, xscale=1.0, c1_off=0, c2_off=0, x1_off=0, x2_off=0):
    a = GemmNN()
    a.A, a.lda = ptr(A), (lda if lda is not None else A.shape[1])
    a.B, a.ldb = ptr(B), (ldb if ldb is not None else B.shape[1])
    a.bias = ptr(bias)
    a.C1 = (ptr(C1) + 4 * c1_off) if C1 is not None else None
    a.ldc1 = ldc1 or (C1.shape[1] if (C1 is not None and C1.dim() == 2) else 0)
    a.C2 = (ptr(C2) + 4 * c2_off) if C2 is not None else None
    a.ldc2 = ldc2 or (C2.shape[1] if (C2 is not None and C2.dim() == 2) else 0)
    a.C3 = ptr(C3)
    a.ldc3 = ldc3 or (C3.shape[1] if (C3 is not None and C3.dim() == 2) else 0)
    a.X1 = (ptr(X1) + 4 * x1_off) if X1 is not None else None
    a.ldx1 = ldx1 or (X1.shape[1] if (X1 is not None and X1.dim() == 2) else 0)
    a.X2 = (ptr(X2) + 4 * x2_off) if X2 is not None else None
    a.ldx2 = ldx2 or (X2.shape[1] if (X2 is not None and X2.dim() == 2) else 0)
    a.M, a.N, a.K, a.epi, a.iparam, a.scale, a.xscale = M, N, K, EPI[epi], iparam, scale, xscale
    if PROFILE is not None:
        _timed("gemm_nn", 2.0 * M * N * getattr(B, "k_true", K), lambda: call("nudf_gemm_nn", a))
        return
    call("nudf_gemm_nn", a)


MFMA_PRODUCTS = {0: 1, 1: 1, 2: 1, 3: 6, 4: 3}

PROFILE = None


def _timed(name, flops, fn, detail=None, nbytes=0.0, xflops=None):
    s = torch.cuda.Event(enable_timing=True)
    e = torch.cuda.Event(enable_timing=True)
    s.record()
    fn()
    e.record()
    PROFILE.append((name, flops, s, e, detail or name, nbytes, xflops))


def call_timed(cls, detail, nbytes, name, *args, units=0.0):
    if PROFILE is None:
        call(name, *args)
    else:
        _timed(cls, -float(units), lambda: call(name, *args), detail, float(nbytes))


def gemm_tn(A1, na1, B1, C, NA, NB, M, dbias=None, A2=None, na2=0, B2=None):
    for t in (A1, B1, A2, B2):
        if t is not None and (_is16(t) or _isblk(t)):
            raise _lib.NudfError("gemm_tn: bf16-stored / blocked-layout operands need gemm_tn_grouped (per-problem "
                                 "NUDF_TN_A16 / _B16 / _A_BLK / _B_BLK flags); set NUDF_STATE16=0 / NUDF_BLOCKED_STATE=0 "
                                 "with NUDF_UDF_TN_GROUPED=0")
    a = GemmTN()
    a.A1, a.lda1, a.na1 = ptr(A1), A1.shape[1], na1
    a.B1, a.ldb1 = ptr(B1), B1.shape[1]
    if A2 is not None:
        a.A2, a.lda2, a.na2 = ptr(A2), A2.shape[1], na2
        a.B2, a.ldb2 = ptr(B2), B2.shape[1]
    a.C, a.ldc = ptr(C), C.shape[1]
    a.dbias = ptr(dbias)
    a.M, a.NA, a.NB, a.rows_per_block = M, NA, NB, 0
    a.prec = _tn_prec()
    if PROFILE is not None:
        _timed("gemm_tn", 2.0 * M * NA * NB * (2 if A2 is not None else 1), lambda: call("nudf_gemm_tn", a))
        return
    call("nudf_gemm_tn", a)


USE_CHAIN = os.environ.get("NUDF_CHAIN", "1") != "0"
CHAIN_DEBUG = None
CHAIN_TILE = int(os.environ.get("NUDF_CHAIN_TILE", "0"))
COLOR_TILE = int(os.environ.get("NUDF_COLOR_TILE", "0"))


def k8(n: int) -> int:
    return (n + 15) // 16 * 16


def pack_frag(B, ldb, K, N, off=0):
    out = torch.empty(k8(K) // 8 * ((N + 31) // 32) * 256, device=B.device, dtype=torch.float32)
    call("nudf_pack_frag", ptr(B) + 4 * off, ldb, K, N, ptr(out))
    out.k_true, out.n_true = K, N
    return out


_PLAIN_TYPES = frozenset((int, float, str, bool, type(None)))
_CHAIN_MEMO = {}
CHAIN_MEMO = os.environ.get("NUDF_CHAIN_MEMO", "1") != "0" and _lib.HOST_FAST
chain_memo_hits = 0


def _memo_token(engine):
    t = engine.__dict__.get("_site_token")
    if t is None:
        t = engine.__dict__["_site_token"] = object()
    return t


class ChainBuilder:

    def __init__(self, P, init, k0, tile_rows=0, site=None):
        self.P, self.init, self.k0, self.tile_rows = P, init, k0, (tile_rows or CHAIN_TILE)
        self.site = site
        self.rec = []
        self.c = None
        self.n = 0
        self.flops = 0.0
        self.xflops = 0.0
        self.nbytes = 0.0
        self.epis = []
        self.blocked = False
        self.keep = []

    def posenc(self, *a, **kw):
        self.rec.append((0, a, kw))

    def init_store(self, *a, **kw):
        self.rec.append((1, a, kw))

    def init_load(self, *a, **kw):
        self.rec.append((2, a, kw))

    def init_seed(self, *a, **kw):
        self.rec.append((3, a, kw))

    def step(self, *a, **kw):
        self.rec.append((4, a, kw))

    def absmax(self, *a, **kw):
        self.rec.append((5, a, kw))

    def tile_scale(self, *a, **kw):
        self.rec.append((6, a, kw))

    _PARAMS = (("x", "L", "in_scale", "tangent", "x_div"), ("G0",), ("A0", "lda0"),
               ("A0", "lda0", "sign", "wrow", "scale", "xscale"), ("epi", "Bp", "K", "N"), ("t",), ("amax_in", "amax_out"))
    _CHAIN_FIELD = ({"x": "x", "tangent": "v"}, {"G0": "G0"}, {"A0": "A0"}, {"A0": "A0", "sign": "seed_sign", "wrow": "seed_wrow"},
                    None, {"t": "absmax_out"}, {"amax_in": "tile_amax_in", "amax_out": "tile_amax_out"})

    def _signature(self):
        T, PT, plain = torch.Tensor, torch.nn.Parameter, _PLAIN_TYPES
        sig = [self.P, self.init, self.k0, self.tile_rows, PRECISION, FWD_F16X2, BWD_F16X2, HEAD16, STATE16, BLOCKED_STATE, TN_SPLIT]
        ptrs = []
        add, addp = sig.append, ptrs.append
        for kind, a, kw in self.rec:
            add(kind)
            for vals in (a, kw.values()):
                for v in vals:
                    tv = type(v)
                    if tv in plain:
                        add(v)
                    elif tv is T or tv is PT or isinstance(v, T):
                        if not (v.is_cuda and v.is_contiguous()):
                            return None, None
                        addp(v.data_ptr())
                        add(v.numel())
                    else:
                        add(v)
            add(tuple(kw))
        return sig, ptrs

    def _fill(self):
        self.c = Chain()
        self.c.P, self.c.init, self.c.k0, self.c.tile_rows = self.P, CH_INIT[self.init], self.k0, self.tile_rows
        self.c.x_div = 1
        fns = (self._do_posenc, self._do_init_store, self._do_init_load, self._do_init_seed, self._do_step, self._do_absmax,
               self._do_tile_scale)
        T = torch.Tensor
        slots = []
        for kind, a, kw in self.rec:
            n0 = self.n
            fns[kind](*a, **kw)
            obj = self.c.step[n0] if kind == 4 else self.c
            names = list(self._PARAMS[kind][:len(a)]) + list(kw)
            vals = list(a) + list(kw.values())
            for nm, v in zip(names, vals):
                if isinstance(v, T):
                    field = nm if kind == 4 else self._CHAIN_FIELD[kind][nm]
                    cur = getattr(obj, field)
                    slots.append((obj, field, cur - v.data_ptr()) if cur is not None else None)
        return slots

    def _p(self, t, off=0):
        if t is None:
            return None
        self.keep.append(t)
        return ptr(t) + t.element_size() * off

    def _do_posenc(self, x, L, in_scale, tangent=None, x_div=1):
        self.c.x, self.c.v = self._p(x), self._p(tangent)
# ... 619 lines not shown
    def mark_stale(self):
        for pl in self.layers:
            pl._ver = None

    def _embed(self, x, P, X, tangent=None):
        net = self.net
        skip_dst = [X[s] for s in sorted(self.skip)]
        d2 = skip_dst[0] if skip_dst else None
        off2 = (self.layers[sorted(self.skip)[0]].inp - self.E) if skip_dst else 0
        call("nudf_posenc", ptr(x), 3, 1, ptr(tangent), net.d_in, net.multires, float(net.scale), P,
             ptr(X[0]), X[0].shape[1], 1.0,
             (ptr(d2) + 4 * off2) if d2 is not None else None, d2.shape[1] if d2 is not None else 0, self.inv_sqrt2)
        for s, dst in zip(sorted(self.skip)[1:], skip_dst[1:]):
            off = self.layers[s].inp - self.E
            call("nudf_posenc", ptr(x), 3, 1, ptr(tangent), net.d_in, net.multires, float(net.scale), P,
                 ptr(dst) + 4 * off, dst.shape[1], self.inv_sqrt2, None, 0, 0.0)

    def _chain_ok(self):
        net = self.net
        widths_ok = all(pl.out <= 256 and pl.inp <= 256 for pl in self.layers[:-1]) and self.layers[-1].inp <= 256 \
            and self.layers[-1].out - 1 <= 256
        skip_ok = len(self.skip) <= 1 and all(0 < s < self.L for s in self.skip)
        return USE_CHAIN and net.multires > 0 and net.d_in == 3 and widths_ok and skip_ok and self.L + 2 <= CH_MAX_STEPS

    def forward(self, x, need_grad_state, feat_ld=0, udf_only=False, feat_buf=None):
        if self._chain_ok():
            return self._forward_chain(x, need_grad_state, feat_ld, udf_only, feat_buf)
        return self._forward_layers(x, need_grad_state, feat_ld, udf_only)

    def gradient(self, x, st):
        if self._chain_ok():
            return self._gradient_chain(x, st)
        return self._gradient_layers(x, st)

    def backward(self, x, st, DA, d_udf, d_feat, d_feat_ld, d_g):
        if self._chain_ok():
            return self._backward_chain(x, st, DA, d_udf, d_feat, d_feat_ld, d_g)
        return self._backward_layers(x, st, DA, d_udf, d_feat, d_feat_ld, d_g)

    def _frag_kinds(self):
        kc = self.__dict__.setdefault("_kinds_cache", {})
        k = kc.get(_mode_key())
        if k is None:
            k = kc[_mode_key()] = tuple(tuple(dict.fromkeys(ks)) for ks in self._frag_kinds_build())
        return k

    def _frag_kinds_build(self):
        kinds = []
        for l, pl in enumerate(self.layers):
            if l == self.L:
                ks = [_head_kind(), _kind("fwd_feat", "fwd"), _kind("bwd_feat", "bwd")]
            elif l in self.skip:
                ks = [_kind("fwd", "fwd"), _kind("bwd", "grad"), _kind("bwd_hid:%d" % self.layers[l - 1].out, "bwd")]
                if PRECISION != "fp32":
                    ks.append(_kind("fwd", "bwd"))
            else:
                ks = [_kind("fwd", "fwd"), _kind("bwd", "grad")]
                if PRECISION != "fp32":
                    ks += [_kind("fwd", "bwd"), _kind("bwd", "bwd")]
            kinds.append(tuple(ks))
        return kinds

    def _skip_col(self, l):
        return self.layers[l].inp - self.E

    def _forward_chain(self, x, need_grad_state, feat_ld=0, udf_only=False, feat_buf=None):
        P, dev, L = x.shape[0], x.device, self.L
        net = self.net
        pack_group(self.layers, self._frag_kinds())
        sd = _state_dtype()
        blk = _state_blocked(P)
        X = ([_buf(P, self.layers[0].inp, dev, zero=False)] +
             [_buf(P, pl.inp, dev, zero=False, dtype=sd, blocked=blk) for pl in self.layers[1:]]) if need_grad_state else None
        cb = ChainBuilder(P, "POSENC", k8(self.E), site=("udf_fwd", _memo_token(self)))
        cb.posenc(x, net.multires, float(net.scale))
        if need_grad_state:
            cb.init_store(X[0])
        for l in range(L):
            pl = self.layers[l]
            nxt_skip = (l + 1) in self.skip
            cb.step("SOFTPLUS", pl.frag(_kind("fwd", "fwd")), k8(pl.inp), pl.out, bias=pl.bias,
                    C1=X[l + 1] if need_grad_state else None,
                    scale=self.inv_sqrt2 if nxt_skip else 1.0,
                    pe_tail_col=self._skip_col(l + 1) if nxt_skip else -1, pe_tail_scale=self.inv_sqrt2,
                    pe_dst=X[l + 1] if (need_grad_state and nxt_skip) else None)
        pl = self.layers[L]
        Pp = pad_rows(P)
        udf = torch.empty(Pp, device=dev)
        sign = torch.empty(Pp, device=dev) if need_grad_state else None
        F = pl.out - 1
        feat = None
        if not udf_only:
            ld = max(feat_ld, F)
            if feat_buf is not None and tuple(feat_buf.shape) == (Pp, ld) and ld >= F + 3 and feat_buf.is_contiguous():
                feat = feat_buf
            else:
                feat = torch.empty((Pp, ld), device=dev)
                if ld >= F + 3:
                    call("nudf_copy_cols", ptr(x), 3, 1, ptr(feat) + 4 * F, ld, 3, P, 1.0)
                    _zero_cols(feat, F + 3)
                else:
                    _zero_cols(feat, F)
            cb.step("NONE", pl.frag(_kind("fwd_feat", "fwd")), k8(pl.inp), F, bias=pl.bias, bias_off=1, C1=feat,
                    act_write=0)
        cb.step("UDFHEAD", pl.frag(_head_kind()), k8(pl.inp), 1, bias=pl.bias, C1=sign, C2=udf, ldc1=1, ldc2=1,
                act_write=0, scale=1.0 / float(net.scale), iparam=self.head_type)
        cb.launch()
        return dict(udf=udf[:P], sign=(sign[:P] if sign is not None else None),
                    feat=(feat[:P] if feat is not None else None), X=X, P=P)

    def _gradient_chain(self, x, st):
        P, L, dev = st["P"], self.L, x.device
        X = st["X"]
        net = self.net
        DA = [_buf(P, self.layers[l].out, dev, zero=False, dtype=X[L].dtype, blocked=_isblk(X[L])) for l in range(L)]
        plL = self.layers[L]
        Epad = pad32(self.E)
        cb = ChainBuilder(P, "SEED", k8(self.layers[L - 1].out), site=("udf_grad", _memo_token(self)))
        cb.init_seed(X[L], X[L].shape[1], st["sign"], plL.W, 1.0 / float(net.scale), self._xs(L - 1))
        cb.init_store(DA[L - 1])
        demb_skip = None
        for l in range(L - 1, 0, -1):
            pl = self.layers[l]
            if l in self.skip:
                demb_skip = torch.empty(pad_rows(P), Epad, device=dev)
                cb.step("MULSP", pl.frag(_kind("bwd", "grad")), k8(pl.out), pl.inp, X1=X[l], C1=DA[l - 1], C2=demb_skip,
                        iparam=self.layers[l - 1].out, scale=self.inv_sqrt2, xscale=self._xs(l - 1))
            else:
                cb.step("MULSP", pl.frag(_kind("bwd", "grad")), k8(pl.out), pl.inp, X1=X[l], C1=DA[l - 1],
                        xscale=self._xs(l - 1))
        demb0 = torch.empty(pad_rows(P), Epad, device=dev)
        pl0 = self.layers[0]
        cb.step("NONE", pl0.frag(_kind("bwd", "grad")), k8(pl0.out), pl0.inp, C1=demb0, act_write=0)
        cb.launch()
        g = torch.empty(P, 3, device=dev)
        call("nudf_posenc_vjp", ptr(x), 3, net.d_in, net.multires, float(net.scale), P,
             ptr(demb0), Epad, 1.0, ptr(demb_skip), Epad, 1.0, ptr(g))
        return g, DA

    def _backward_chain(self, x, st, DA, d_udf, d_feat, d_feat_ld, d_g):
        P, L, dev = st["P"], self.L, x.device
        X, sign = st["X"], st["sign"]
        layers = self.layers
        net = self.net
        grouped = os.environ.get("NUDF_UDF_TN_GROUPED", "1") == "1"
        head4_path = grouped and os.environ.get("NUDF_UDF_HEAD4", "1") == "1"
        assign = head4_path and tn_can_assign()
        grads = alloc_grads(layers, zero=not assign)
        second = d_g is not None and DA is not None
        R = EX = None
        ex_fly = second and EX_FLY and PRECISION != "fp32" and not _isblk(X[L]) and CHAIN_TILE in (0, 32, 64)
        tn2 = (TN_F16X2 and PRECISION == "bf16x3" and TN_SPLIT and grouped and head4_path and not _isblk(X[L]) and not _is16(X[L])
               and CHAIN_TILE in (0, 32, 64))
        amax = torch.zeros(2, device=dev) if tn2 else None
        bsc = _sweep_dtype("bwd") == "f16x2"
        TA = torch.empty(pad_rows(P) // 32, device=dev) if (bsc and second) else None
        if second:
            sd, blk = X[L].dtype, _isblk(X[L])
            R = ([_buf(P, layers[0].inp, dev, zero=False)] +
                 [_buf(P, pl.inp, dev, zero=False, dtype=sd, blocked=blk) for pl in layers[1:]])
            EX = None if ex_fly else [_buf(P, layers[l].out, dev, zero=False, dtype=sd, blocked=blk) for l in range(L)]
            cb = ChainBuilder(P, "POSENC", k8(self.E), site=("udf_tangent", _memo_token(self)))
            cb.posenc(x, net.multires, float(net.scale), tangent=d_g.contiguous())
            cb.init_store(R[0])
            if tn2:
                cb.absmax(amax[1:2])
            if bsc:
                cb.tile_scale(amax_out=TA)
            for l in range(L):
                pl = layers[l]
                nxt_skip = (l + 1) in self.skip
                if ex_fly:
                    cb.step("MULSP", pl.frag(_kind("fwd", "bwd")), k8(pl.inp), pl.out, X1=X[l + 1], C1=R[l + 1],
                            scale=self.inv_sqrt2 if nxt_skip else 1.0, xscale=self._xs(l),
                            pe_tail_col=self._skip_col(l + 1) if nxt_skip else -1, pe_tail_scale=self.inv_sqrt2,
                            pe_dst=R[l + 1] if nxt_skip else None)
                else:
                    cb.step("TANGENT", pl.frag(_kind("fwd", "bwd")), k8(pl.inp), pl.out, X1=X[l + 1], X2=DA[l], C1=R[l + 1],
                            C2=EX[l],
                            scale=self.inv_sqrt2 if nxt_skip else 1.0, xscale=self._xs(l),
                            pe_tail_col=self._skip_col(l + 1) if nxt_skip else -1, pe_tail_scale=self.inv_sqrt2,
                            pe_dst=R[l + 1] if nxt_skip else None)
            cb.launch()
        inv_scale = 1.0 / float(net.scale)
        if second and not head4_path:
            call("nudf_signed_colsum", ptr(sign), ptr(R[L]), R[L].shape[1], P, layers[L].inp, inv_scale, ptr(grads[L][0]))
        plL = layers[L]
        F = plL.out - 1
        ABAR = [None] * (L + 1)
        if head4_path:
            head4 = torch.empty(pad_rows(P), 4, device=dev)
            sg4 = torch.empty(pad_rows(P), 4, device=dev) if second else None
            if d_udf is not None:
                call("nudf_col0_seed4", ptr(sign), ptr(d_udf.reshape(-1).contiguous()), float(inv_scale), P, pad_rows(P),
                     ptr(head4), ptr(sg4))
            else:
                head4.zero_()
                if second:
                    call("nudf_col0_seed4", ptr(sign), None, float(inv_scale), P, pad_rows(P), ptr(sg4), None)
            r1, ldr1 = head4, 4
        else:
            ABAR[L] = _buf(P, plL.out, dev, zero=False)
            call("nudf_udf_head_bwd", ptr(sign), ptr(d_udf), ptr(d_feat), d_feat_ld, P, F, inv_scale, ptr(ABAR[L]),
                 ABAR[L].shape[1])
            r1, ldr1 = ABAR[L], ABAR[L].shape[1]
        for l in range(L):
            ABAR[l] = _buf(P, layers[l].out, dev, zero=False, dtype=X[L].dtype, blocked=_isblk(X[L]))
        cb = ChainBuilder(P, "LOAD", k8(F), site=("udf_adjoint", _memo_token(self)))
        if d_feat is None:
            d_feat, d_feat_ld = torch.zeros(P, k8(F), device=dev), k8(F)
        cb.init_load(d_feat, d_feat_ld)
        if tn2:
            cb.absmax(amax[0:1])
        if bsc:
            cb.tile_scale(amax_in=TA)
        for l in range(L, 0, -1):
            pl = layers[l]
            sc = self.inv_sqrt2 if l in self.skip else 1.0
            x2 = (R[l] if ex_fly else EX[l - 1]) if second else None
            x3 = DA[l - 1] if ex_fly else None
            if l == L:
                cb.step("BWD", pl.frag(_kind("bwd_feat", "bwd")), k8(F), layers[l - 1].out, X1=X[l], X2=x2, X3=x3,
                        C1=ABAR[l - 1], r1_row=r1, ldr1=ldr1, r1_col=pl.W, scale=sc,
                        xscale=self._xs(l - 1))
            else:
                n_hid = layers[l - 1].out
                cb.step("BWD", pl.frag(_kind("bwd" if n_hid == pl.inp else "bwd_hid:%d" % n_hid, "bwd")), k8(pl.out),
                        n_hid, X1=X[l], X2=x2, X3=x3, C1=ABAR[l - 1], scale=sc, xscale=self._xs(l - 1))
        cb.launch()
        if grouped:
            dWL, dbL = grads[L]
            jobs = [(ABAR[l], layers[l].out, X[l], layers[l].in_pad, grads[l][0], grads[l][1]) for l in range(L)]
            if head4_path:
                assert d_feat.shape[1] == d_feat_ld and d_feat.is_contiguous()
                jobs.append((d_feat, F, X[L], plL.in_pad, dWL[1:], dbL[1:]))
                jobs.append((head4, 1, X[L], plL.in_pad, dWL[:1], dbL[:1]))
            else:
                jobs.append((ABAR[L], plL.out, X[L], plL.in_pad, dWL, dbL))
            gemm_tn_grouped(jobs, P, assign=assign, f16x2=tn2, amax_a=amax[0:1] if tn2 else None)
            if second:
                jobs = [(DA[l], layers[l].out, R[l], layers[l].in_pad, grads[l][0], None) for l in range(L)]
                if head4_path:
                    jobs.append((sg4, 1, R[L], plL.in_pad, dWL[:1], None))
                gemm_tn_grouped(jobs, P, f16x2=tn2, amax_b=amax[1:2] if tn2 else None)
            return unpack_group(layers, grads, claim_grad_slot(self, layers))
        for l, pl in enumerate(layers):
            dW, db = grads[l]
            if second and l < L:
                gemm_tn(ABAR[l], pl.out, X[l], dW, pl.out, pl.in_pad, P, dbias=db, A2=DA[l], na2=pl.out, B2=R[l])
            else:
                gemm_tn(ABAR[l], pl.out, X[l], dW, pl.out, pl.in_pad, P, dbias=db)
        return unpack_group(layers, grads, claim_grad_slot(self, layers))

    def _forward_layers(self, x, need_grad_state, feat_ld=0, udf_only=False):
        P = x.shape[0]
        dev = x.device
        L = self.L
        pack_group(self.layers)
        X = [_buf(P, pl.inp, dev) for pl in self.layers]
        self._embed(x, P, X)
        for l in range(L):
            pl = self.layers[l]
            sc = self.inv_sqrt2 if (l + 1) in self.skip else 1.0
            gemm_nn(X[l], pl.Wt, P, pl.out, pl.in_pad, "SOFTPLUS", C1=X[l + 1], bias=pl.bias, scale=sc)
        pl = self.layers[L]
        udf = torch.empty(P, device=dev)
        sign = torch.empty(P, device=dev) if need_grad_state else None
        F = pl.out - 1
        feat = None
        if not udf_only:
            ld = max(feat_ld, F)
            feat = (torch.zeros if ld > F else torch.empty)((P, ld), device=dev)
            if ld >= F + 3:
                call("nudf_copy_cols", ptr(x), 3, 1, ptr(feat) + 4 * F, ld, 3, P, 1.0)
        gemm_nn(X[L], pl.Wt, P, 1 if udf_only else pl.out, pl.in_pad, "UDFHEAD", C1=feat, C2=udf, ldc2=1, C3=sign,
                ldc3=1, bias=pl.bias, scale=1.0 / float(self.net.scale), iparam=self.head_type)
        return dict(udf=udf, sign=sign, feat=feat, X=X, P=P)

    def _xs(self, j):
        return math.sqrt(2.0) if (j + 1) in self.skip else 1.0

    def _gradient_layers(self, x, st):
        P, L, dev = st["P"], self.L, x.device
        X = st["X"]
        DA = [_buf(P, self.layers[l].out, dev) for l in range(L)]
        plL = self.layers[L]
        call("nudf_udf_grad_seed", ptr(st["sign"]), ptr(plL.W), ptr(X[L]), X[L].shape[1], self._xs(L - 1), P,
             self.layers[L - 1].out, 1.0 / float(self.net.scale), ptr(DA[L - 1]), DA[L - 1].shape[1])
        Epad = pad32(self.E)
        demb_skip = None
        for l in range(L - 1, 0, -1):
            pl = self.layers[l]
            if l in self.skip:
                if demb_skip is not None:
                    raise NotImplementedError("more than one skip layer")
                demb_skip = torch.zeros(P, Epad, device=dev)
                gemm_nn(DA[l], pl.W, P, pl.inp, pl.out_pad, "SKIPSPLIT", C1=DA[l - 1], C2=demb_skip, X1=X[l],
                        iparam=self.layers[l - 1].out, scale=self.inv_sqrt2, xscale=self._xs(l - 1))
            else:
                gemm_nn(DA[l], pl.W, P, pl.inp, pl.out_pad, "MULSP", C1=DA[l - 1], X1=X[l], xscale=self._xs(l - 1))
        demb0 = torch.zeros(P, Epad, device=dev)
        pl0 = self.layers[0]
        gemm_nn(DA[0], pl0.W, P, pl0.inp, pl0.out_pad, "NONE", C1=demb0)
        g = torch.empty(P, 3, device=dev)
        call("nudf_posenc_vjp", ptr(x), 3, self.net.d_in, self.net.multires, float(self.net.scale), P,
             ptr(demb0), Epad, 1.0, ptr(demb_skip), Epad, 1.0, ptr(g))
        return g, DA
# ... 36 lines not shown
                gemm_tn(ABAR[l], pl.out, X[l], dW, pl.out, pl.in_pad, P, dbias=db)
            out += pl.unpack_grads(dW, db)
        return out


def relu_chain_bwd(layers, inputs, outs, D_last, P, first_needs_input_grad, add_at=None):
    n = len(layers)
    grads = alloc_grads(layers)
    D = D_last
    d_in0 = None
    tn_jobs = []
    for i in range(n - 1, -1, -1):
        pl = layers[i]
        tn_jobs.append((D, pl.out, inputs[i], pl.in_pad, grads[i][0], grads[i][1]))
        if i > 0:
            prev = layers[i - 1]
            Dn = _buf(P, prev.out, D.device)
            extra = add_at.get(i - 1) if add_at else None
            if extra is not None:
                gemm_nn(D, pl.W, P, prev.out, pl.out_pad, "ADDMASK", C1=Dn, X1=outs[i - 1], ldx1=outs[i - 1].shape[1],
                        X2=extra[0], ldx2=extra[1], x2_off=extra[2])
            else:
                gemm_nn(D, pl.W, P, prev.out, pl.out_pad, "MULMASK", C1=Dn, X1=outs[i - 1], ldx1=outs[i - 1].shape[1])
            D = Dn
        elif first_needs_input_grad:
            d_in0 = _buf(P, pl.inp, D.device, zero=False)
            gemm_nn(D, pl.W, P, pl.inp, pl.out_pad, "NONE", C1=d_in0)
    gemm_tn_grouped(tn_jobs, P)
    return grads, d_in0


class ColorEngine:

    def __init__(self, net):
        self.net = net
        n = net.num_layers - 1
        self.n = n
        F, H, dout = net.d_feature, net.d_hidden, net.d_out
        self.F, self.H, self.dout = F, H, dout
        self.npe = net.view_dim
        self.nrm = 0 if net.mode == "no_normal" else 6
        perm_b0 = [F + i for i in range(3 + self.nrm)] + list(range(F))
        perm_v0 = [H + i for i in range(self.npe)] + [H + self.npe + j for j in range(dout)] + list(range(H))
        self.base = [PackedLinear(getattr(net, f"lin_base{l}"), perm_b0 if l == 0 else None) for l in range(n)]
        self.view = [PackedLinear(getattr(net, f"lin{l}"), perm_v0 if l == 0 else None) for l in range(n)]

    def params(self):
        out = []
        for pl in self.view + self.base:
            out += pl.params()
        return out

    def invalidate(self):
        for pl in self.view + self.base:
            pl.invalidate()

    def mark_stale(self):
        for pl in self.view + self.base:
            pl._ver = None

    @property
    def cin_ld(self):
        return pad32(self.F + 3 + self.nrm)

    def _chain_ok(self):
        n = self.n
        ok = USE_CHAIN and n >= 2 and 2 * n <= CH_MAX_STEPS and self.H <= 256 and self.net.embedview_fn is not None
        ok = ok and k8(self.base[0].inp) <= 288 and k8(self.H + self.npe + self.dout) <= 288 and self.F % 4 == 0
        ok = ok and self.view[n - 1].out <= 32 and self.dout <= 32
        return ok

    def _kinds(self):
        kc = self.__dict__.setdefault("_kinds_cache", {})
        k = kc.get(_mode_key())
        if k is None:
            k = kc[_mode_key()] = tuple(tuple(dict.fromkeys(ks)) for ks in self._kinds_build())
        return k

    def _kinds_build(self):
        fw, bw = _kind("fwd", "fwd"), _kind("bwd", "bwd")
        kinds = [(fw, _kind("bwd_hid:%d" % self.F, "bwd"))]
        kinds += [(fw, bw)] * (self.n - 1)
        kinds += [(fw, bw)] * self.n
        return kinds

    def forward(self, CIN, rays_d, S, P, keep_state=True, row_w=None):
        if self._chain_ok():
            return self._forward_chain(CIN, rays_d, S, P, keep_state, row_w)
        if row_w is not None:
            raise _lib.NudfError("the compositing sum inside the colour heads needs the fused chain launch")
        return self._forward_layers(CIN, rays_d, S, P, keep_state)

    def backward(self, st, color_base, color, d_cb, d_color, d_logits):
        if "chain" in st:
            return self._backward_chain(st, color_base, color, d_cb, d_color, d_logits)
        return self._backward_layers(st, color_base, color, d_cb, d_color, d_logits)

    def _forward_chain(self, CIN, rays_d, S, P, keep_state=True, row_w=None):
        dev, n = CIN.device, self.n
        fused = row_w is not None
        assert not (fused and keep_state)
        H, npe, dout = self.H, self.npe, self.dout
        pack_group(self.base + self.view, self._kinds())
        Pp = pad_rows(P)
        VIN = torch.empty(Pp, pad32(H + npe + dout), device=dev) if keep_state else None
        sd = _state_dtype()
        HB = [CIN] + [_buf(P, H, dev, zero=False, dtype=sd) for _ in range(n - 1)] if keep_state else None
        HV = [VIN] + [_buf(P, H, dev, zero=False, dtype=sd) for _ in range(n - 1)] if keep_state else None
        cb = ChainBuilder(P, "LOAD", k8(self.base[0].inp), tile_rows=COLOR_TILE, site=("col_fwd", _memo_token(self)))
        cb.init_load(CIN, CIN.shape[1])
        cb.posenc(rays_d, self.net.multires_view, 1.0, x_div=S)
        for l in range(n - 1):
            pl = self.base[l]
            tap = (l == n - 2)
            cb.step("RELU", pl.frag(_kind("fwd", "fwd")), k8(pl.inp), pl.out, bias=pl.bias, C1=HB[l + 1] if keep_state else None,
                    C2=VIN if (tap and keep_state) else None, pe_tail_col=H if tap else -1, pe_tail_scale=1.0,
                    pe_dst=VIN if (tap and keep_state) else None)
        color_base = None if fused else torch.empty(Pp, dout, device=dev)
        sums_b = torch.empty(Pp // 32, 4, device=dev) if fused else None
        sums_c = torch.empty(Pp // 32, 4, device=dev) if fused else None
        pl = self.base[n - 1]
        cb.step("SIGMOIDN", pl.frag(_kind("fwd", "fwd")), k8(pl.inp), pl.out, bias=pl.bias, C1=color_base, C2=VIN if keep_state else None,
                c2_off=H + npe, iparam=dout, act_write=1, act_col0=H + npe, row_w=row_w, row_sums=sums_b)
        for l in range(n - 1):
            pl = self.view[l]
            cb.step("RELU", pl.frag(_kind("fwd", "fwd")), k8(pl.inp), pl.out, bias=pl.bias, C1=HV[l + 1] if keep_state else None)
        pl = self.view[n - 1]
        nb = pl.out - dout
        color = None if fused else torch.empty(Pp, dout, device=dev)
        logits = torch.empty(Pp, max(nb, 1), device=dev)
        cb.step("SIGMOIDN", pl.frag(_kind("fwd", "fwd")), k8(pl.inp), pl.out, bias=pl.bias, C1=color, C2=logits if nb > 0 else None,
                iparam=dout, act_write=0, row_w=row_w, row_sums=sums_c)
        cb.launch()
        if fused:
            return sums_b, sums_c, (logits[:P] if nb > 0 else None), None
        st = dict(HB=HB, HV=HV, P=P, chain=True) if keep_state else None
        return color_base[:P], color[:P], (logits[:P] if nb > 0 else None), st

    def _backward_chain(self, st, color_base, color, d_cb, d_color, d_logits):
        P, n = st["P"], self.n
        HB, HV = st["HB"], st["HV"]
        dev = color.device
        H, npe, dout = self.H, self.npe, self.dout
        assign = tn_can_assign()
        grads = alloc_grads(self.view + self.base, zero=not assign)
        plv = self.view[n - 1]
        nb = plv.out - dout
        sd = HV[1].dtype
        Dv = [_buf(P, H, dev, zero=False, dtype=sd) for _ in range(n - 1)] + [_buf(P, plv.out, dev, zero=False)]
        call("nudf_sigmoid_head_bwd", ptr(color), ptr(d_color), None, 0, dout, ptr(d_logits), max(nb, 1), nb, P,
             ptr(Dv[n - 1]), Dv[n - 1].shape[1])
        dVIN = _buf(P, self.view[0].inp, dev, zero=False)
        tn2 = TN_F16X2 and PRECISION == "bf16x3" and TN_SPLIT and not _is16(HV[1]) and COLOR_TILE in (0, 32, 64)
        amax = torch.zeros(1, device=dev) if tn2 else None
        cb = ChainBuilder(P, "LOAD", k8(plv.out), tile_rows=COLOR_TILE, site=("col_bwd_view", _memo_token(self)))
        cb.init_load(Dv[n - 1], Dv[n - 1].shape[1])
        if tn2:
            cb.absmax(amax)
        bsc = _sweep_dtype("bwd") == "f16x2"
        TV = torch.empty(pad_rows(P) // 32, device=dev) if bsc else None
        if bsc:
            cb.tile_scale(amax_out=TV)
        for i in range(n - 1, 0, -1):
            pl = self.view[i]
            cb.step("MULMASK", pl.frag(_kind("bwd", "bwd")), k8(pl.out), pl.inp, X1=HV[i], C1=Dv[i - 1])
        pl0 = self.view[0]
        cb.step("NONE", pl0.frag(_kind("bwd", "bwd")), k8(pl0.out), pl0.inp, C1=dVIN, act_write=0)
        cb.launch()
        plb = self.base[n - 1]
        Db = [_buf(P, H, dev, zero=False, dtype=sd) for _ in range(n - 1)] + [_buf(P, plb.out, dev, zero=False)]
        call("nudf_sigmoid_head_bwd", ptr(color_base), ptr(d_cb), ptr(dVIN) + 4 * (H + npe), dVIN.shape[1],
             dout, None, 0, 0, P, ptr(Db[n - 1]), Db[n - 1].shape[1])
        dCIN = torch.empty(pad_rows(P), self.cin_ld, device=dev)
        cb = ChainBuilder(P, "LOAD", k8(plb.out), tile_rows=COLOR_TILE, site=("col_bwd_base", _memo_token(self)))
        cb.init_load(Db[n - 1], Db[n - 1].shape[1])
        if tn2:
            cb.absmax(amax)
        if bsc:
            cb.tile_scale(amax_in=TV)
        for i in range(n - 1, 0, -1):
            pl = self.base[i]
            if i == n - 1:
                cb.step("ADDMASK", pl.frag(_kind("bwd", "bwd")), k8(pl.out), pl.inp, X1=HB[i], X2=dVIN, C1=Db[i - 1])
            else:
                cb.step("MULMASK", pl.frag(_kind("bwd", "bwd")), k8(pl.out), pl.inp, X1=HB[i], C1=Db[i - 1])
        pb0 = self.base[0]
        cb.step("NONE", pb0.frag(_kind("bwd_hid:%d" % self.F, "bwd")), k8(pb0.out), self.F, C1=dCIN, act_write=0)
        cb.launch()
        jobs = []
        for i, pl in enumerate(self.view):
            jobs.append((Dv[i], pl.out, HV[i], pl.in_pad, grads[i][0], grads[i][1]))
        for i, pl in enumerate(self.base):
            jobs.append((Db[i], pl.out, HB[i], pl.in_pad, grads[n + i][0], grads[n + i][1]))
        gemm_tn_grouped(jobs, P, assign=assign, f16x2=tn2, amax_a=amax)
        return unpack_group(self.view + self.base, grads, claim_grad_slot(self, self.view + self.base)), dCIN[:P]

    def _forward_layers(self, CIN, rays_d, S, P, keep_state=True):
        dev = CIN.device
        n = self.n
        pack_group(self.base + self.view)
        VIN = _zero_cols(torch.empty(P, pad32(self.H + self.npe + self.dout), device=dev), self.H + self.npe + self.dout)
        call("nudf_posenc", ptr(rays_d), 3, S, None, 3, self.net.multires_view, 1.0, P,
             ptr(VIN) + 4 * self.H, VIN.shape[1], 1.0, None, 0, 0.0)
        HB = [CIN]
        for l in range(n - 1):
            pl = self.base[l]
            h = _buf(P, pl.out, dev)
            if l == n - 2:
                gemm_nn(HB[l], pl.Wt, P, pl.out, pl.in_pad, "RELU_DUAL", C1=h, C2=VIN, bias=pl.bias)
            else:
                gemm_nn(HB[l], pl.Wt, P, pl.out, pl.in_pad, "RELU", C1=h, bias=pl.bias)
            HB.append(h)
        color_base = torch.empty(P, self.dout, device=dev)
        pl = self.base[n - 1]
        gemm_nn(HB[n - 1], pl.Wt, P, pl.out, pl.in_pad, "SIGMOID", C1=color_base, C2=VIN, c2_off=self.H + self.npe,
                bias=pl.bias, iparam=self.dout)
        HV = [VIN]
        for l in range(n - 1):
            pl = self.view[l]
            h = _buf(P, pl.out, dev)
            gemm_nn(HV[l], pl.Wt, P, pl.out, pl.in_pad, "RELU", C1=h, bias=pl.bias)
            HV.append(h)
        pl = self.view[n - 1]
        color = torch.empty(P, self.dout, device=dev)
        nb = pl.out - self.dout
        logits = torch.empty(P, max(nb, 1), device=dev)
        gemm_nn(HV[n - 1], pl.Wt, P, pl.out, pl.in_pad, "SIGMOID", C1=color, C3=logits, bias=pl.bias,
                iparam=self.dout)
        st = dict(HB=HB, HV=HV, P=P) if keep_state else None
        return color_base, color, (logits if nb > 0 else None), st

    def _backward_layers(self, st, color_base, color, d_cb, d_color, d_logits):
        P, n = st["P"], self.n
        HB, HV = st["HB"], st["HV"]
        dev = color.device
        plv = self.view[n - 1]
        nb = plv.out - self.dout
        D = _buf(P, plv.out, dev, zero=False)
        call("nudf_sigmoid_head_bwd", ptr(color), ptr(d_color), None, 0, self.dout, ptr(d_logits), max(nb, 1), nb, P,
             ptr(D), D.shape[1])
        gv, dVIN = relu_chain_bwd(self.view, HV, HV[1:], D, P, True)
        Db = _buf(P, self.dout, dev, zero=False)
        call("nudf_sigmoid_head_bwd", ptr(color_base), ptr(d_cb), ptr(dVIN) + 4 * (self.H + self.npe), dVIN.shape[1],
             self.dout, None, 0, 0, P, ptr(Db), Db.shape[1])
        gb, dCIN = relu_chain_bwd(self.base, HB, HB[1:], Db, P, True, add_at={n - 2: (dVIN, dVIN.shape[1], 0)})
        return unpack_group(self.view + self.base, gv + gb), dCIN[:P]


class PlainColorEngine:

    def __init__(self, net):
        self.net = net
        self.layers = [PackedLinear(getattr(net, f"lin{l}")) for l in range(net.num_layers - 1)]
        self.dout = net.d_out

    def params(self):
        out = []
        for pl in self.layers:
            out += pl.params()
        return out

    def forward(self, Xin, P, keep_state=True):
        dev, n = Xin.device, len(self.layers)
        pack_group(self.layers)
        X = _buf(P, self.layers[0].inp, dev)
        X[:P, :Xin.shape[1]] = Xin
        H = [X]
        for l in range(n - 1):
            pl = self.layers[l]
            h = _buf(P, pl.out, dev)
            gemm_nn(H[l], pl.Wt, P, pl.out, pl.in_pad, "RELU", C1=h, bias=pl.bias)
            H.append(h)
        pl = self.layers[n - 1]
        nb = pl.out - self.dout
        color = torch.empty(P, self.dout, device=dev)
        logits = torch.empty(P, max(nb, 1), device=dev)
        if self.net.squeeze_out:
            gemm_nn(H[n - 1], pl.Wt, P, pl.out, pl.in_pad, "SIGMOID", C1=color, C3=logits, bias=pl.bias, iparam=self.dout)
        else:
            raw = _buf(P, pl.out, dev)
            gemm_nn(H[n - 1], pl.Wt, P, pl.out, pl.in_pad, "NONE", C1=raw, bias=pl.bias)
            color, logits = raw[:P, :self.dout].contiguous(), raw[:P, self.dout:pl.out].contiguous()
        st = dict(H=H, P=P) if keep_state else None
        return color, (logits if nb > 0 else None), st

    def backward(self, st, color, d_color, d_logits):
        P, H = st["P"], st["H"]
        dev = color.device
        pl = self.layers[-1]
        nb = pl.out - self.dout
        D = _buf(P, pl.out, dev, zero=True)
        if self.net.squeeze_out:
            if d_color is None:
                d_color = torch.zeros_like(color)
            if nb > 0 and d_logits is None:
                d_logits = torch.zeros(P, nb, device=dev)
            call("nudf_sigmoid_head_bwd", ptr(color), ptr(d_color.contiguous()), None, 0, self.dout,
                 ptr(d_logits.contiguous()) if nb > 0 else None, max(nb, 1), nb, P, ptr(D), D.shape[1])
        else:
            if d_color is not None:
                D[:P, :self.dout] = d_color
            if nb > 0 and d_logits is not None:
                D[:P, self.dout:pl.out] = d_logits
        grads, dX = relu_chain_bwd(self.layers, H, H[1:], D, P, True)
        return unpack_group(self.layers, grads), dX[:P, :self.layers[0].inp]


# ... 226 lines not shown
```

neuraludf_amd/models/udf_renderer_blending.py:

```python
from __future__ import annotations

import numpy as np
import torch

import os

from .. import _lib
from .._lib import Composite, CompositeGrad, Upsample, call, ptr
from .. import dist as nudf_dist
from .. import mlp

UPSAMPLE_FLAGS = int(os.environ.get("NUDF_UP_FLAGS", str(512 | 1024 | 2048 | 4096)))
FUSE_SCALARS = os.environ.get("NUDF_FUSE_SCALARS", "1") == "1"
FUSE_COLOUR = os.environ.get("NUDF_FUSE_COLOUR", "1") == "1"

_DIAG = ["alpha", "alpha_plus", "alpha_minus", "vis_prob", "alpha_occ", "raw_occ", "true_cos", "grad_mag", "mid_z",
         "dists", "inside", "flip"]


def _fill_composite(a, c, N, S, n_out):
    a.N, a.S, a.n_out, a.s_nominal = N, S, n_out, c["s_nominal"]
    a.has_anneal = 0 if c["cos_anneal"] is None else 1
    a.cos_anneal = 0.0 if c["cos_anneal"] is None else float(c["cos_anneal"])
    a.flip_saturation = float(c["flip_saturation"])
    a.use_norm_grad = 1 if c["use_norm_grad"] else 0
    a.sparse_scale = float(c["sparse_scale"])
    a.alpha_type = int(c.get("alpha_type", 0))
    a.sched = ptr(c.get("sched"))


class _CompositeFn(torch.autograd.Function):

    @staticmethod
    def forward(ctx, c, rays_o, rays_d, z, sample_dist, background_rgb, udf, grad, color, color_base, bg_z, bg_sigma,
                bg_color, scal, p_var=None, p_beta=None, p_gamma=None):
        ctx.set_materialize_grads(False)
        N, S = z.shape
        n_out = 0 if bg_z is None else bg_z.shape[1]
        dev = z.device
        t = lambda x: None if x is None else x.detach().contiguous()
        rays_o, rays_d, z, udf, grad, color, color_base = map(t, (rays_o, rays_d, z, udf, grad, color, color_base))
        bg_z, bg_sigma, bg_color, scal = map(t, (bg_z, bg_sigma, bg_color, scal))
        p_var, p_beta, p_gamma = map(t, (p_var, p_beta, p_gamma))
        a = Composite()
        a.rays_o, a.rays_d, a.z, a.udf, a.grad = ptr(rays_o), ptr(rays_d), ptr(z), ptr(udf), ptr(grad)
        a.color, a.color_base = ptr(color), ptr(color_base)
        a.bg_z, a.bg_sigma, a.bg_color = ptr(bg_z), ptr(bg_sigma), ptr(bg_color)
        a.scal, a.sample_dist, a.background_rgb = ptr(scal), ptr(sample_dist), ptr(t(background_rgb))
        _fill_composite(a, c, N, S, n_out)
        scal_out = recip = None
        if p_var is not None:
            scal_out, recip = torch.empty(3, device=dev), torch.empty(2, device=dev)
            a.p_variance, a.p_beta, a.p_gamma, a.beta_hi = ptr(p_var), ptr(p_beta), ptr(p_gamma), float(c["beta_hi"])
            a.scal_out, a.recip_out = ptr(scal_out), ptr(recip)
        weights = torch.empty(N, S + n_out, device=dev)
        out_color = torch.empty(N, 3, device=dev)
        out_cb = torch.empty(N, 3, device=dev)
        depth = torch.empty(N, 1, device=dev)
        normals = torch.empty(N, 3, device=dev)
        wsum = torch.empty(N, 1, device=dev)
        wsum_all = torch.empty(N, 1, device=dev)
        sums = torch.empty(5, device=dev)
        ws = torch.empty(5 * ((N + 3) // 4), device=dev)
        a.ws = ptr(ws)
        a.weights, a.out_color, a.out_color_base = ptr(weights), ptr(out_color), ptr(out_cb)
        a.out_depth, a.out_normals, a.out_wsum, a.out_wsum_all, a.sums = (ptr(depth), ptr(normals), ptr(wsum),
                                                                          ptr(wsum_all), ptr(sums))
        diag = []
        if c["diagnostics"]:
            for k in _DIAG:
                d = torch.empty(N, S, device=dev)
                setattr(a, "o_" + k, ptr(d))
                diag.append(d)
        if c.get("defer_sums"):
            a.defer_sums = 1
            sums.fill_(float("nan"))
            sums._nudf_ws = (ws, (N + 3) // 4)
        ST = weights.shape[1]
        mlp.call_timed("composite", "composite_fwd N=%d S=%d" % (N, ST), (48.0 if color is not None else 24.0) * N * ST + 68.0 * N,
                       "nudf_composite_fwd", a, units=N * ST)
        ctx.c = c
        ctx.save_for_backward(rays_o, rays_d, z, sample_dist, t(background_rgb), udf, grad, color, color_base, bg_z,
                              bg_sigma, bg_color, scal, p_var, p_beta, p_gamma)
        extra = () if p_var is None else (scal_out, recip)
        ctx.mark_non_differentiable(*diag, *extra)
        return (out_color, out_cb, weights, depth, normals, wsum, wsum_all, sums) + tuple(diag) + extra

    @staticmethod
    def backward(ctx, d_color, d_cb, d_weights, d_depth, d_normals, d_wsum, d_wsum_all, d_sums, *_):
        (rays_o, rays_d, z, sample_dist, background_rgb, udf, grad, color, color_base, bg_z, bg_sigma, bg_color,
         scal, p_var, p_beta, p_gamma) = ctx.saved_tensors
        c = ctx.c
        N, S = z.shape
        n_out = 0 if bg_z is None else bg_z.shape[1]
        dev = z.device
        a = Composite()
        a.rays_o, a.rays_d, a.z, a.udf, a.grad = ptr(rays_o), ptr(rays_d), ptr(z), ptr(udf), ptr(grad)
        a.color, a.color_base = ptr(color), ptr(color_base)
        a.bg_z, a.bg_sigma, a.bg_color = ptr(bg_z), ptr(bg_sigma), ptr(bg_color)
        a.scal, a.sample_dist, a.background_rgb = ptr(scal), ptr(sample_dist), ptr(background_rgb)
        _fill_composite(a, c, N, S, n_out)
        if p_var is not None:
            a.p_variance, a.p_beta, a.p_gamma, a.beta_hi = ptr(p_var), ptr(p_beta), ptr(p_gamma), float(c["beta_hi"])
        g = CompositeGrad()
        cg = lambda x: None if x is None else x.contiguous()
        keep = [cg(x) for x in (d_color, d_cb, d_weights, d_depth, d_normals, d_wsum, d_wsum_all, d_sums)]
        (g.d_color, g.d_color_base, g.d_weights, g.d_depth, g.d_normals, g.d_wsum, g.d_wsum_all,
         g.d_sums) = [ptr(x) for x in keep]
        o_udf = torch.empty(N, S, device=dev)
        o_grad = torch.empty(N, S, 3, device=dev)
        o_col = torch.empty(N, S, 3, device=dev)
        o_cb = torch.empty(N, S, 3, device=dev)
        o_sig = torch.empty(N, n_out, device=dev) if n_out else None
        o_bgc = torch.empty(N, n_out, 3, device=dev) if n_out else None
        o_scal = o_par = None
        if p_var is not None:
            o_par = torch.empty(3, device=dev)
        else:
            o_scal = torch.empty(3, device=dev)
        ws = torch.empty(3 * ((N + 3) // 4), device=dev)
        g.ws = ptr(ws)
        g.o_d_udf, g.o_d_grad, g.o_d_color, g.o_d_color_base = ptr(o_udf), ptr(o_grad), ptr(o_col), ptr(o_cb)
        g.o_d_bg_sigma, g.o_d_bg_color, g.o_d_scal, g.o_d_param = ptr(o_sig), ptr(o_bgc), ptr(o_scal), ptr(o_par)
        mlp.call_timed("composite", "composite_bwd N=%d S=%d" % (N, S + n_out), 84.0 * N * (S + n_out) + 68.0 * N,
                       "nudf_composite_bwd", a, g, units=N * (S + n_out))
        d_par = (None, None, None) if o_par is None else (o_par[0:1].reshape(p_var.shape), o_par[1:2].reshape(p_beta.shape),
                                                         o_par[2:3].reshape(p_gamma.shape))
        return (None, None, None, None, None, None, o_udf, o_grad, o_col, o_cb, None, o_sig, o_bgc, o_scal) + d_par


class _ScalarsFn(torch.autograd.Function):

    @staticmethod
    def forward(ctx, variance, beta, gamma, beta_hi):
        ctx.set_materialize_grads(False)
        v, b, g = variance.detach().contiguous(), beta.detach().contiguous(), gamma.detach().contiguous()
        scal = torch.empty(3, device=v.device)
        recip = torch.empty(2, device=v.device)
        call("nudf_scalars_fwd", ptr(v), ptr(b), ptr(g), float(beta_hi), ptr(scal), ptr(recip))
        ctx.save_for_backward(v, b, g)
        ctx.beta_hi = float(beta_hi)
        ctx.mark_non_differentiable(recip)
        return scal, recip

    @staticmethod
    def backward(ctx, d_scal, _d_recip):
        if d_scal is None:
            return None, None, None, None
        v, b, g = ctx.saved_tensors
        d = torch.empty(3, device=v.device)
        call("nudf_scalars_bwd", ptr(v), ptr(b), ptr(g), ctx.beta_hi, ptr(d_scal.contiguous()), ptr(d))
        return d[0:1].reshape(v.shape), d[1:2].reshape(b.shape), d[2:3].reshape(g.shape), None


class _ErrorsFn(torch.autograd.Function):

    @staticmethod
    def forward(ctx, sums, n_rays):
        ctx.set_materialize_grads(False)
        sums = sums.detach().contiguous()
        err = torch.empty(3, device=sums.device)
        call("nudf_sums_errors_fwd", ptr(sums), float(n_rays), ptr(err))
        ctx.save_for_backward(sums)
        ctx.n_rays = float(n_rays)
        return err[0], err[1], err[2]

    @staticmethod
    def backward(ctx, d0, d1, d2):
        if d0 is None and d1 is None and d2 is None:
            return None, None
        (sums,) = ctx.saved_tensors
        z = sums.new_zeros(())
        d_err = torch.stack([d if d is not None else z for d in (d0, d1, d2)])
        d = torch.empty(5, device=sums.device)
        call("nudf_sums_errors_bwd", ptr(sums), ctx.n_rays, ptr(d_err), ptr(d))
        return d, None


GRID_CHUNK_POINTS = 1 << 21


def _grid_axes(bound_min, bound_max, resolution, device):
    return torch.stack([torch.linspace(float(bound_min[k]), float(bound_max[k]), int(resolution), device=device)
                        for k in range(3)])


def _grid_query_device(bound_min, bound_max, resolution, query_func, device, channels):
    dev = torch.device(device)
    R = int(resolution)
    axes = _grid_axes(bound_min, bound_max, R, dev)
    shape = (R, R, R) if channels == 1 else (R, R, R, channels)
    vol = torch.empty(shape, dtype=torch.float32, device=dev)
    planes = max(1, (GRID_CHUNK_POINTS // (1 if channels == 1 else 4)) // (R * R))
    yz = torch.stack([axes[1][:, None].expand(R, R), axes[2][None, :].expand(R, R)], -1).reshape(1, R * R, 2)
    for x0 in range(0, R, planes):
        xs = axes[0][x0:x0 + planes]
        pts = torch.cat([xs[:, None, None].expand(len(xs), R * R, 1), yz.expand(len(xs), R * R, 2)], -1).reshape(-1, 3)
        val = query_func(pts).detach()
        vol[x0:x0 + len(xs)] = val.reshape((len(xs),) + shape[1:])
    return vol


def _grid_query(bound_min, bound_max, resolution, query_func, device, channels):
    return _grid_query_device(bound_min, bound_max, resolution, query_func, device, channels).cpu().numpy()


def extract_fields(bound_min, bound_max, resolution, query_func, device='cuda'):
    with torch.no_grad():
        return _grid_query(bound_min, bound_max, resolution, query_func, device, 1)


def extract_gradient_fields(bound_min, bound_max, resolution, query_func, device='cuda'):
    return _grid_query(bound_min, bound_max, resolution, query_func, device, 3)


def extract_geometry(bound_min, bound_max, resolution, threshold, query_func, device):
    u = extract_fields(bound_min, bound_max, resolution, query_func, device)
    try:
        import mcubes
    except ImportError as e:
        raise ImportError("extract_geometry needs PyMCubes (`mcubes`), like the reference; the field grid itself is "
                          "available from extract_fields()") from e
    vertices, triangles = mcubes.marching_cubes(u, threshold)
    b_max = np.asarray([float(v) for v in bound_max], dtype=np.float64)
    b_min = np.asarray([float(v) for v in bound_min], dtype=np.float64)
    vertices = vertices / (resolution - 1.0) * (b_max - b_min)[None, :] + b_min[None, :]
    return vertices, triangles


class UDFRendererBlending:
    def __init__(self, nerf, udf_network, deviation_network, color_network, beta_network, n_samples, n_importance,
                 n_outside, up_sample_steps, perturb, sdf2alpha_type='numerical', upsampling_type='classical',
                 sparse_scale_factor=25000, h_patch_size=3, use_norm_grad_for_cosine=False):
        self.nerf = nerf
        self.udf_network = udf_network
        self.deviation_network = deviation_network
        self.color_network = color_network
        self.beta_network = beta_network
        self.n_samples = n_samples
        self.n_importance = n_importance
        self.n_outside = n_outside
        self.perturb = perturb
        self.up_sample_steps = up_sample_steps
        if sdf2alpha_type not in ('numerical', 'theorical'):
            raise ValueError("sdf2alpha_type %r (the reference knows 'numerical' and 'theorical')" % sdf2alpha_type)
        self.sdf2alpha_type = sdf2alpha_type
        self.upsampling_type = upsampling_type
        self.sparse_scale_factor = sparse_scale_factor
        self.h_patch_size = h_patch_size
        self.use_norm_grad_for_cosine = use_norm_grad_for_cosine
        self.diagnostics = True
        self.compute_sparse_random = False
        self.data_parallel = False
        self.defer_loss_sums = False
        self.defer_sums_reduce = False
        from .patch_projector import PatchProjector
        self.patch_projector = PatchProjector(self.h_patch_size)
        self._u_cache = {}
        self._mid = None

    def _scalars(self, dev):
        dn, bn = self.deviation_network, self.beta_network
        if (isinstance(getattr(dn, "variance", None), torch.Tensor) and dn.variance.numel() == 1 and dn.variance.is_cuda
                and isinstance(getattr(bn, "beta", None), torch.Tensor) and hasattr(bn, "gamma")
                and hasattr(bn, "beta_min")):
            return _ScalarsFn.apply(dn.variance, bn.beta, bn.gamma, 1.0 / bn.beta_min)
        inv_s = dn(torch.zeros([1, 3], device=dev))[:, :1].clip(1e-6, 1e6).reshape(1)
        beta = bn.get_beta().clip(1e-6, 1e6).reshape(1)
        gamma = bn.get_gamma().clip(1e-6, 1e6).reshape(1)
        scal = torch.cat([inv_s, beta, gamma])
        return scal, torch.stack([1.0 / inv_s[0], 1.0 / beta[0]]).detach()

    def _scalar_params(self):
        dn, bn = self.deviation_network, self.beta_network
        from . import fields as _fields
        if not (FUSE_SCALARS and type(dn) is _fields.SingleVarianceNetwork and type(bn) is _fields.BetaNetwork):
            return None
        ps = (dn.variance, bn.beta, bn.gamma)
        dev = ps[0].device
        if all(isinstance(t, torch.Tensor) and t.numel() == 1 and t.is_cuda and t.device == dev and t.dtype == torch.float32
               and t.is_contiguous() for t in ps):
            return dn.variance, bn.beta, bn.gamma, 1.0 / bn.beta_min
        return None

    @staticmethod
    def finish_sums(sums):
        pend = getattr(sums, "_nudf_ws", None)
        if pend is not None:
            del sums._nudf_ws
            call("nudf_partial_sums", ptr(pend[0]), pend[1], 5, ptr(sums))
        return sums

    def errors_from_sums(self, sums, n_local):
        n_rays = float(n_local) * (nudf_dist.world_size() if self.data_parallel else 1)
        return _ErrorsFn.apply(self.finish_sums(sums), n_rays)

    def _quantiles(self, k, dev):
        key = (k, str(dev))
        if key not in self._u_cache:
            self._u_cache[key] = torch.linspace(0. + 0.5 / k, 1. - 0.5 / k, steps=k).to(dev).contiguous()
        return self._u_cache[key]

    def _udf_at(self, rays_o, rays_d, z, sample_dist, pts=None):
        N, M = z.shape
        if pts is None:
            pts = torch.empty(N * M, 3, device=z.device)
            call("nudf_ray_points", ptr(rays_o), ptr(rays_d), ptr(z), ptr(sample_dist), N, M, 0, ptr(pts))
        return self.udf_network.udf_only(pts).reshape(N, M)

    def _upsample(self, rays_o, rays_d, z, udf, sample_dist, k, mode, inv_s, beta, gamma, gamma_dev=None, dbg=None,
                  pending=None):
        dev = rays_o.device
        a = Upsample()
        keep = None
        if pending is not None:
            zp, up, za, ua = keep = [t.contiguous() for t in pending]
            N, M = zp.shape[0], zp.shape[1] + za.shape[1]
            z = torch.empty(N, M, device=dev)
            udf = torch.empty(N, M, device=dev)
            a.prev_z, a.prev_udf, a.add_z, a.add_udf = ptr(zp), ptr(up), ptr(za), ptr(ua)
            a.z_merged, a.udf_merged, a.merge_K = ptr(z), ptr(udf), za.shape[1]
        else:
            N, M = z.shape
        a.rays_o, a.rays_d, a.z, a.udf = ptr(rays_o), ptr(rays_d), ptr(z), ptr(udf)
        a.u, a.sample_dist, a.gamma_dev = ptr(self._quantiles(k, dev)), ptr(sample_dist), ptr(gamma_dev)
        a.N, a.M, a.K, a.mode = N, M, k, mode | (256 if self.sdf2alpha_type == 'theorical' else 0) | UPSAMPLE_FLAGS
        a.inv_s, a.beta, a.gamma = float(inv_s), float(beta), float(gamma)
        z_new = torch.empty(N, k, device=dev)
        pts_new = torch.empty(N * k, 3, device=dev)
        a.z_new, a.pts_new, a.dbg = ptr(z_new), ptr(pts_new), ptr(dbg)
        mlp.call_timed("upsample", "upsample N=%d M=%d K=%d" % (N, M, k), float(N) * (8 * M + 4 * k + 8 * (M + k) + 24),
                       "nudf_upsample", a, units=N * M)
        if pending is not None:
            return z_new, pts_new, z, udf
        return z_new, pts_new

    def _merge(self, z, udf, z_new, udf_new):
        N, M = z.shape
        K = z_new.shape[1]
        zo = torch.empty(N, M + K, device=z.device)
        uo = torch.empty(N, M + K, device=z.device) if udf_new is not None else None
        call("nudf_merge", ptr(z), ptr(udf) if uo is not None else None, ptr(z_new), ptr(udf_new), N, M, K, ptr(zo),
             ptr(uo))
        return zo, uo

    def _merge_last(self, rays_o, rays_d, z, z_new, sample_dist, for_render=False):
        if not for_render:
            return self._merge(z, None, z_new, None)[0]
        N, M = z.shape
        K = z_new.shape[1]
        S = M + K
        dev = z.device
        zo = torch.empty(N, S, device=dev)
        pts = torch.empty(N * S, 3, device=dev)
        ceng = self.color_network.engine()
        F, ld = ceng.F, ceng.cin_ld
        feat = None
        if ld >= F + 3:
            feat = torch.empty(mlp.pad_rows(N * S), ld, device=dev)
        call("nudf_merge_points", ptr(z.contiguous()), ptr(z_new), N, M, K, ptr(zo), ptr(rays_o), ptr(rays_d),
             ptr(sample_dist), ptr(pts), (ptr(feat) + 4 * F) if feat is not None else None, ld, ld - F)
        self._mid = (zo, pts, feat)
        return zo

    @torch.no_grad()
    def importance_sample(self, rays_o, rays_d, z_vals, sample_dist, pts0=None, for_render=False):
        N = rays_o.shape[0]
        udf = self._udf_at(rays_o, rays_d, z_vals, sample_dist, pts0)
        steps = self.up_sample_steps
        k = self.n_importance // steps
        pend = None
        for i in range(steps):
            gamma = float(np.clip(20 * 2 ** (steps - i), 20, 320))
            if pend is None:
                z_new, pts_new = self._upsample(rays_o, rays_d, z_vals, udf, sample_dist, k, 0, 64 * 2 ** i,
                                                64 * 2 ** (i + 1), gamma)
            else:
                z_new, pts_new, z_vals, udf = self._upsample(rays_o, rays_d, None, None, sample_dist, k, 0, 64 * 2 ** i,
                                                             64 * 2 ** (i + 1), gamma, pending=pend)
            if i + 1 == steps:
                return self._merge_last(rays_o, rays_d, z_vals, z_new, sample_dist, for_render)
            pend = (z_vals, udf, z_new, self.udf_network.udf_only(pts_new).reshape(N, k))
        return z_vals

    @torch.no_grad()
    def importance_sample_mix(self, rays_o, rays_d, z_vals, sample_dist, pts0=None, for_render=False):
        N = rays_o.shape[0]
        udf = self._udf_at(rays_o, rays_d, z_vals, sample_dist, pts0)
        steps = self.up_sample_steps
        k = self.n_importance // (steps + 1)
        gamma_dev = self.beta_network.get_gamma().clip(1e-6, 1e6).detach().reshape(1).contiguous()
        pend = None
        for i in range(steps):
            if pend is None:
                z_new, pts_new = self._upsample(rays_o, rays_d, z_vals, udf, sample_dist, k, 1, 64 * 2 ** i,
                                                64 * 2 ** (i + 1), 0.0, gamma_dev)
            else:
                z_new, pts_new, z_vals, udf = self._upsample(rays_o, rays_d, None, None, sample_dist, k, 1, 64 * 2 ** i,
                                                             64 * 2 ** (i + 1), 0.0, gamma_dev, pending=pend)
            pend = (z_vals, udf, z_new, self.udf_network.udf_only(pts_new).reshape(N, k))
        i = steps - 1
        if pend is None:
            z_new, _ = self._upsample(rays_o, rays_d, z_vals, udf, sample_dist, k, 0, 64 * 2 ** i, 64 * 2 ** (i + 1),
                                      20 if i < 4 else 10)
        else:
            z_new, _, z_vals, udf = self._upsample(rays_o, rays_d, None, None, sample_dist, k, 0, 64 * 2 ** i,
                                                   64 * 2 ** (i + 1), 20 if i < 4 else 10, pending=pend)
        return self._merge_last(rays_o, rays_d, z_vals, z_new, sample_dist, for_render)

    def render_core_outside(self, rays_o, rays_d, z_out, sample_dist, z_in=None):
        N, n_out = z_out.shape
        zf = z_out if z_in is None else torch.cat([z_in, z_out], dim=-1).contiguous()
        M = zf.shape[1]
        pts4 = torch.empty(N * M, 4, device=z_out.device)
        call("nudf_ray_points", ptr(rays_o), ptr(rays_d), ptr(zf), ptr(sample_dist), N, M, 2, ptr(pts4))
        sigma, rgb = self.nerf.evaluate(pts4, rays_d, M)
        sigma, rgb = sigma.reshape(N, M), rgb.reshape(N, M, 3)
        if z_in is None:
            return sigma, rgb, None
        S = z_in.shape[1]
        return sigma[:, S:].contiguous(), rgb[:, S:].contiguous(), rgb[:, :S].contiguous()

    def render_core(self, rays_o, rays_d, z_vals, sample_dist, cos_anneal_ratio=None, background_rgb=None,
                    bg_z=None, bg_sigma=None, bg_color=None, flip_saturation=0.0, color_maps=None, w2cs=None,
                    intrinsics=None, query_c2w=None, img_index=None, rays_uv=None, s_nominal=None, bg_color_in=None,
                    patch_cams=None):
        N, S = z_vals.shape
        dev = z_vals.device
        P = N * S
        mid, self._mid = getattr(self, "_mid", None), None
        feat_buf = None
        if mid is not None and mid[0] is z_vals:
            pts, feat_buf = mid[1], mid[2]
        else:
            pts = torch.empty(P, 3, device=dev)
            call("nudf_ray_points", ptr(rays_o), ptr(rays_d), ptr(z_vals), ptr(sample_dist), N, S, 1, ptr(pts))
        ceng = self.color_network.engine()
        udf, CIN, grad = self.udf_network.evaluate(pts, want_grad=True, feat_ld=ceng.cin_ld,
                                                   normals_col=(ceng.F + 3) if ceng.nrm else -1, feat_buf=feat_buf)
        fuse_colour = (FUSE_COLOUR and not torch.is_grad_enabled() and bg_z is None and color_maps is None and S % 32 == 0
                       and S >= 32 and isinstance(ceng, mlp.ColorEngine) and ceng._chain_ok() and not self.data_parallel)
        cb = col = logits = None
        if not fuse_colour:
            cb, col, logits = self.color_network.evaluate(CIN, rays_d, S)
        spar = self._scalar_params()
        scal = recip = None
        if spar is None:
            scal, recip = self._scalars(dev)
        defer = self.defer_loss_sums and (not self.data_parallel or nudf_dist.exchanging())
        c = dict(s_nominal=(s_nominal if s_nominal is not None else S), cos_anneal=cos_anneal_ratio,
                 beta_hi=(spar[3] if spar is not None else 0.0),
                 defer_sums=bool(defer and not self.data_parallel and self.defer_sums_reduce),
                 flip_saturation=flip_saturation, use_norm_grad=self.use_norm_grad_for_cosine,
                 sparse_scale=self.sparse_scale_factor, diagnostics=self.diagnostics,
                 alpha_type=1 if self.sdf2alpha_type == 'theorical' else 0,
                 sched=getattr(self, "sched_scalars", None))
        outs = _CompositeFn.apply(c, rays_o, rays_d, z_vals, sample_dist, background_rgb, udf.reshape(N, S),
                                  grad.reshape(N, S, 3), None if fuse_colour else col.reshape(N, S, 3),
                                  None if fuse_colour else cb.reshape(N, S, 3), bg_z, bg_sigma,
                                  bg_color, scal, *(spar[:3] if spar is not None else ()))
        color, color_base, weights, depth, normals, wsum, wsum_all, sums = outs[:8]
        if fuse_colour:
            Pp = mlp.pad_rows(P)
            row_w = weights.reshape(-1)
            if Pp != P:
                row_w = torch.zeros(Pp, device=dev)
                row_w[:P] = weights.reshape(-1)
            sums_b, sums_c, logits, _ = ceng.forward(CIN.detach(), rays_d, S, P, keep_state=False, row_w=row_w)
            color, color_base = torch.empty(N, 3, device=dev), torch.empty(N, 3, device=dev)
            call("nudf_composite_colour_finish", ptr(sums_c), ptr(sums_b), N, S, ptr(background_rgb), ptr(wsum_all), ptr(color),
                 ptr(color_base))
        if spar is not None:
            scal, recip = outs[-2:]
        diag = dict(zip(_DIAG, outs[8:8 + len(_DIAG)])) if self.diagnostics else {}
        local_sums = None
        if defer:
            local_sums = sums
            gradient_error = gradient_error_ns = sparse_error = None
        else:
            if self.data_parallel:
                sums = nudf_dist.all_reduce_sum(sums)
            gradient_error, gradient_error_ns, sparse_error = self.errors_from_sums(sums, N)

        color_pixel = patch_colors = patch_mask = None
        if color_maps is not None:
            from . import blend
            if img_index is not None:
                raise NotImplementedError("img_index: the reference's own branch (fields.py:507-511) is shape-inconsistent "
                                          "and unused; every call site passes None")
            color_pixel, patch_colors, patch_mask = blend.blend_and_composite(
                self.h_patch_size, pts.reshape(N, S, 3), logits.reshape(N, S, -1), weights, grad.reshape(N, S, 3).detach(),
                rays_d, color_maps, w2cs, intrinsics, query_c2w, rays_uv, bg_in=bg_color_in, bg_tail=bg_color,
                patch_cams=patch_cams)

        g3 = grad.reshape(N, S, 3)
        ret = {
            'color_base': color_base, 'color': color, 'color_pixel': color_pixel, 'patch_colors': patch_colors,
            'patch_mask': patch_mask, 'weights': weights, 's_val': recip[0:1].reshape(1, 1),
            'beta': recip[1:2], 'gamma': scal[2:3], 'depth': depth, 'gradient_error': gradient_error,
            'gradient_error_near_surface': gradient_error_ns, 'normals': normals, 'gradients': g3,
            'udf': udf.reshape(N, S), 'sparse_error': sparse_error, 'weight_sum': wsum, 'weight_sum_fg_bg': wsum_all,
        }
        if local_sums is not None:
            ret['_loss_sums'] = local_sums
        if self.diagnostics:
            ret.update({
                'gradients_flip': diag["flip"][:, :, None] * g3, 'inside_sphere': diag["inside"],
                'gradient_mag': diag["grad_mag"], 'true_cos': diag["true_cos"], 'vis_prob': diag["vis_prob"],
                'alpha': diag["alpha"], 'alpha_plus': diag["alpha_plus"], 'alpha_minus': diag["alpha_minus"],
                'mid_z_vals': diag["mid_z"], 'dists': diag["dists"], 'alpha_occ': diag["alpha_occ"],
                'raw_occ': diag["raw_occ"]})
        else:
            for k in ['gradients_flip', 'inside_sphere', 'gradient_mag', 'true_cos', 'vis_prob', 'alpha', 'alpha_plus',
                      'alpha_minus', 'mid_z_vals', 'dists', 'alpha_occ', 'raw_occ']:
                ret[k] = None
        return ret

    def _device(self):
        return next(self.udf_network.parameters()).device

    def status(self, clear=False):
        return _lib.read_status(self._device(), clear=clear)

    def clear_status(self):
        _lib.read_status(self._device(), clear=True)

    def check_finite(self):
        bits = self.status(clear=True)
        if bits:
            raise FloatingPointError("NeuralUDF renderer: " + _lib.status_text(bits))

    def render(self, rays_o, rays_d, near, far, cos_anneal_ratio=None, perturb_overwrite=-1, background_rgb=None,
               flip_saturation=0, color_maps=None, w2cs=None, intrinsics=None, query_c2w=None, img_index=None,
               rays_uv=None, z_vals_override=None, patch_cams=None):
        dev = rays_o.device
        N = len(rays_o)
        if N == 0:
            return self._empty_result(dev, color_maps is not None, rays_uv is not None)
        _lib.bind_status(dev)
        rays_o = rays_o.detach().float().contiguous()
        rays_d = rays_d.detach().float().contiguous()
        if not isinstance(near, torch.Tensor):
            near = torch.tensor([float(near)], device=dev).view(1, 1)
            far = torch.tensor([float(far)], device=dev).view(1, 1)
        near = near.detach().float().contiguous()
        far = far.detach().float().contiguous()
        nf_stride = 0 if near.numel() == 1 else 1

        perturb = self.perturb if perturb_overwrite < 0 else perturb_overwrite
        t_rand = None
        lin = None
        if self.n_outside > 0:
            lin = torch.linspace(1e-3, 1.0 - 1.0 / (self.n_outside + 1.0), self.n_outside, device=dev)
        if perturb > 0:
            t_rand = torch.rand([N, 1], device=dev)
            if self.n_outside > 0:
                mids = .5 * (lin[..., 1:] + lin[..., :-1])
                upper = torch.cat([mids, lin[..., -1:]], -1)
                lower = torch.cat([lin[..., :1], mids], -1)
                lin = lower + (upper - lower) * torch.rand(lin.shape, device=dev)
        z_vals = torch.empty(N, self.n_samples, device=dev)
        sample_dist = torch.empty(1, device=dev)
        want_pts0 = z_vals_override is None and self.n_importance > 0 and self.upsampling_type in ('classical', 'mix')
        pts0 = torch.empty(N * self.n_samples, 3, device=dev) if want_pts0 else None
        call("nudf_coarse_start", ptr(near), ptr(far), nf_stride, ptr(t_rand), 1, N, self.n_samples, ptr(z_vals),
             ptr(sample_dist), ptr(rays_o), ptr(rays_d), ptr(pts0))
        z_out = None
        if self.n_outside > 0:
            z_out = torch.empty(N, self.n_outside, device=dev)
            call("nudf_outside_z", ptr(far), nf_stride, ptr(lin.float().contiguous()), N, self.n_outside,
                 self.n_samples, ptr(z_out))
        self._z_vals_outside = z_out

        n_samples = self.n_samples
        if z_vals_override is not None:
            z_vals = z_vals_override.detach().float().contiguous()
            n_samples = z_vals.shape[1]
        elif self.n_importance > 0:
            if self.upsampling_type == 'classical':
                z_vals = self.importance_sample(rays_o, rays_d, z_vals, sample_dist, pts0, for_render=True)
            elif self.upsampling_type == 'mix':
                z_vals = self.importance_sample_mix(rays_o, rays_d, z_vals, sample_dist, pts0, for_render=True)
            n_samples = self.n_samples + self.n_importance

        bg_sigma = bg_color = bg_color_in = None
        if self.n_outside > 0:
            bg_sigma, bg_color, bg_color_in = self.render_core_outside(
                rays_o, rays_d, z_out, sample_dist, z_vals if color_maps is not None else None)

        bgrgb = None
        if background_rgb is not None:
            bgrgb = torch.as_tensor(background_rgb, dtype=torch.float32, device=dev).reshape(-1)[:3].contiguous()
        ret = self.render_core(rays_o, rays_d, z_vals, sample_dist, cos_anneal_ratio, bgrgb, z_out, bg_sigma,
                               bg_color, flip_saturation, color_maps, w2cs, intrinsics, query_c2w, img_index, rays_uv,
                               s_nominal=n_samples, bg_color_in=bg_color_in, patch_cams=patch_cams)

        sparse_random_error = 0.0
        if True:
            pts_random = torch.rand([1024, 3], device=dev)
            if self.compute_sparse_random:
                with torch.no_grad():
                    udf_random = self.udf_network.udf(pts_random * 2 - 1)
                if (udf_random < 0.01).sum() > 10:
                    sparse_random_error = torch.exp(-self.sparse_scale_factor * udf_random[udf_random < 0.01]).mean()
        ret['variance'] = ret.pop('s_val')
        ret['z_vals'] = z_vals
        ret['sparse_random_error'] = sparse_random_error
        return ret

    def _empty_result(self, dev, pixel, patch):
        S = self.n_samples + (self.n_importance if self.n_importance > 0 else 0)
        e = lambda *shape: torch.zeros(*shape, device=dev)
        npx = (2 * self.h_patch_size + 1) ** 2
        ret = {
            'color_base': e(0, 3), 'color': e(0, 3), 'color_pixel': e(0, 3) if pixel else None,
            'patch_colors': e(0, npx, 3) if patch else None, 'patch_mask': e(0) if patch else None,
            'weights': e(0, S + self.n_outside), 'variance': e(1, 1), 'beta': e(1), 'gamma': e(1), 'depth': e(0, 1),
            'gradient_error': e(()), 'gradient_error_near_surface': e(()), 'normals': e(0, 3), 'gradients': e(0, S, 3),
            'udf': e(0, S), 'sparse_error': e(()), 'weight_sum': e(0, 1), 'weight_sum_fg_bg': e(0, 1),
            'z_vals': e(0, S), 'sparse_random_error': 0.0,
        }
        for k in ['gradients_flip', 'inside_sphere', 'gradient_mag', 'true_cos', 'vis_prob', 'alpha', 'alpha_plus',
                  'alpha_minus', 'mid_z_vals', 'dists', 'alpha_occ', 'raw_occ']:
            ret[k] = e(0, S, 3) if k == 'gradients_flip' else e(0, S)
        return ret

    def extract_udf_geometry(self, bound_min, bound_max, resolution, dist_threshold_ratio=1.0, **clean):
        from .. import meshing
        return meshing.extract_udf_mesh(self.udf_network, resolution, bound_min, bound_max,
                                        dist_threshold_ratio=dist_threshold_ratio, **clean)

    def extract_geometry(self, bound_min, bound_max, resolution, threshold=0.01, device='cpu'):
        dev = next(self.udf_network.parameters()).device
        return extract_geometry(bound_min, bound_max, resolution, threshold,
                                lambda pts: self.udf_network.udf(pts)[:, 0], dev)
```

neuraludf_amd/train.py:

```python
from __future__ import annotations

import contextlib
import io

import os

import torch

from . import dist as nudf_dist
from ._lib import LW, LW_COUNT
from .loss.loss import ColorLoss
from .models import fields
from .models.udf_renderer_blending import UDFRendererBlending

def other_scalars(var, beta):
    return list(var.parameters()) + list(beta.parameters())


DTU_MODEL_CONF = dict(
    nerf=dict(D=8, d_in=4, d_in_view=3, W=256, multires=10, multires_view=4, output_ch=4, skips=[4],
              use_viewdirs=True),
    udf_network=dict(d_out=257, d_in=3, d_hidden=256, n_layers=8, skip_in=[4], multires=6, bias=0.5, scale=1.0,
                     geometric_init=True, weight_norm=True, udf_type="abs"),
    variance_network=dict(init_val=0.3),
    rendering_network=dict(d_feature=256, mode="no_normal", d_in=6, d_out=3, d_hidden=128, n_layers=4,
                           weight_norm=True, multires_view=4, squeeze_out=True, blending_cand_views=10),
    beta_network=dict(init_var_beta=0.5, init_var_gamma=0.3, init_var_zeta=0.3, beta_min=0.00005,
                      requires_grad_beta=True, requires_grad_gamma=False, requires_grad_zeta=False),
)


class StepScalars:
    SCHED, LOSSW, ADAM = 0, 8, 8 + LW_COUNT

    def __init__(self, device, n_adam=96, slots=8):
        n = self.ADAM + 2 * n_adam
        self.n_adam = n_adam
        self.dev = torch.zeros(n, device=device)
        self.host = [torch.zeros(n).pin_memory() for _ in range(slots)]
        self.events = [None] * slots
        self.k = 0

    def upload(self, sched, lossw, adam):
        i = self.k % len(self.host)
        self.k += 1
        if self.events[i] is not None:
            self.events[i].synchronize()
        h = self.host[i].numpy()
        h[self.SCHED:self.SCHED + len(sched)] = sched
        h[self.LOSSW:self.LOSSW + len(lossw)] = lossw
        if len(adam) > 2 * self.n_adam:
            raise ValueError("too many optimizer tensors for the step-scalar buffer")
        h[self.ADAM:self.ADAM + len(adam)] = adam
        self.dev.copy_(self.host[i], non_blocking=True)
        ev = torch.cuda.Event()
        ev.record()
        self.events[i] = ev


SINGLE_THREAD_BACKWARD = os.environ.get("NUDF_HOST_FAST", "1") != "0"


class GraphedStep:

    def __init__(self, trainer, eager_steps=2, max_graphs=4, capture_collectives=False):
        from .optim import FusedAdam
        self.tr = trainer
        self.eager_steps = eager_steps
        self.max_graphs = max_graphs
        self.graphs = {}
        self.enabled = isinstance(trainer.optimizer, FusedAdam) and (capture_collectives or not trainer.data_parallel)
        self.scalars = None
        self.replays = 0
        self.captures = 0
        self._last = None
        self._epoch = getattr(trainer.optimizer, "state_epoch", 0)

    def invalidate(self):
        self.graphs.clear()
        self._last = None

    def _key(self, batch, blend, has_anneal, perturb_overwrite):
        tr = self.tr
        sig = lambda d: tuple(sorted((k, tuple(v.shape), str(v.dtype)) for k, v in d.items() if torch.is_tensor(v)))
        live = tuple(p.requires_grad for g in tr.param_groups for p in g)
        cw = tr.color_loss
        terms = (cw.color_pixel_weight > 0, cw.color_patch_weight > 0, tr.lc["color_pixel_weight"] > 0,
                 tr.lc["color_patch_weight"] > 0, tr.tc["mask_weight"] > 0)
        static = tuple(sorted((k, v) for k, v in tr.lc.items() if not k.endswith("_weight")))
        return (sig(batch), sig(blend) if blend is not None else None, bool(has_anneal), perturb_overwrite, terms, static,
                live)

    def __call__(self, batch, cos_anneal_ratio=1.0, flip_saturation=1.0, blend=None, perturb_overwrite=-1):
        tr = self.tr
        kw = dict(cos_anneal_ratio=cos_anneal_ratio, flip_saturation=flip_saturation, blend=blend,
                  perturb_overwrite=perturb_overwrite)
        if not self.enabled:
            return tr.step(batch, **kw)
        if getattr(tr.optimizer, "state_epoch", 0) != self._epoch:
            self._epoch = tr.optimizer.state_epoch
            self.invalidate()
        if (blend is not None and "ref_cam" not in blend and tr.lc["color_pixel_weight"] > 0
                and tr.lc["color_patch_weight"] > 0):
            from .models import blend as _blend
            blend = dict(blend)
            blend["ref_cam"], blend["src_cam"] = _blend.patch_cameras(blend["intrinsics"][0], blend["intrinsics"],
                                                                      blend["query_c2w"], torch.inverse(blend["w2cs"]))
            kw["blend"] = blend
        key = self._key(batch, blend, cos_anneal_ratio is not None, perturb_overwrite)
        ent = self.graphs.get(key)
        if ent is None:
            if len(self.graphs) >= self.max_graphs:
                self.graphs.pop(next(iter(self.graphs)))
            ent = self.graphs[key] = dict(calls=0, graph=None)
        ent["calls"] += 1
        self._last = ent
        if ent["graph"] is None:
            if ent["calls"] <= self.eager_steps or ent.get("failed"):
                return tr.step(batch, **kw)
            prev_stream = torch.cuda.current_stream()
            try:
                self._capture(ent, batch, blend, cos_anneal_ratio is not None, flip_saturation, perturb_overwrite)
            except Exception as e:
                import warnings
                ent["failed"], ent["graph"] = True, None
                torch.cuda.set_stream(prev_stream)
                torch.cuda.synchronize()
                warnings.warn("GraphedStep: capture failed (%s); this configuration keeps running eagerly" % (e,))
                return tr.step(batch, **kw)
        for k, v in ent["batch"].items():
            src = batch[k]
            if torch.is_tensor(v) and src is not v and src.data_ptr() != v.data_ptr():
                v.copy_(src)
        if blend is not None:
            for k, v in ent["blend"].items():
                src = blend[k]
                if torch.is_tensor(v) and src is not v and src.data_ptr() != v.data_ptr():
                    v.copy_(src)
        tr.optimizer._order = ent["order"]
        ent["scalars"].upload([0.0 if cos_anneal_ratio is None else float(cos_anneal_ratio), float(flip_saturation)],
                              tr.loss_weights().values(), tr.optimizer.dyn_values())
        ent["graph"].replay()
        tr.optimizer.advance()
        self.replays += 1
        return ent["loss"], ent["out"]

    def static_inputs(self):
        ent = self._last
        if ent is None or ent.get("graph") is None:
            return None
        return ent["batch"], ent["blend"]

    def _capture(self, ent, batch, blend, has_anneal, flip_saturation, perturb_overwrite):
        tr = self.tr
        dev = batch["rays_o"].device
        n_adam = sum(len(g) for g in tr.param_groups)
        if self.scalars is None or self.scalars.n_adam < n_adam:
            self.scalars = StepScalars(dev, n_adam=max(96, n_adam))
        ent["scalars"] = self.scalars
        ent["batch"] = {k: (v.clone() if torch.is_tensor(v) else v) for k, v in batch.items()}
        ent["blend"] = ({k: (v.clone() if torch.is_tensor(v) else v) for k, v in blend.items()}
                        if blend is not None else None)
        for m in tr.modules().values():
            e = getattr(m, "_engine", None)
            if e is not None and hasattr(e, "mark_stale"):
                e.mark_stale()
        sc = self.scalars
        tr.renderer.sched_scalars = sc.dev[sc.SCHED:sc.SCHED + 2]
        tr.optimizer.dyn_base = sc.dev.data_ptr() + 4 * sc.ADAM
        tr.loss_weights().bind(sc.dev[sc.LOSSW:sc.LOSSW + LW_COUNT])
        if blend is not None:
            tr.color_loss.prefill_constants(dev)
        g = torch.cuda.CUDAGraph()
        torch.cuda.synchronize()
        import gc
        gc_was_on = gc.isenabled()
        gc.disable()
        try:
            with torch.cuda.graph(g):
                loss, out = tr.step(ent["batch"], cos_anneal_ratio=(1.0 if has_anneal else None),
                                    flip_saturation=flip_saturation, blend=ent["blend"],
                                    perturb_overwrite=perturb_overwrite)
        finally:
            if gc_was_on:
                gc.enable()
            tr.renderer.sched_scalars = None
            tr.optimizer.dyn_base = None
            tr.loss_weights().unbind()
        ent["graph"], ent["loss"], ent["out"], ent["order"] = g, loss, out, list(tr.optimizer._order)
        self.captures += 1


class Trainer:
    def __init__(self, device, renderer_conf, color_loss_conf=None, train_conf=None, seed=0, data_parallel=False,
                 fields_mod=fields, renderer_cls=UDFRendererBlending, loss_cls=ColorLoss, fused_adam=False,
                 model_conf=None):
        torch.manual_seed(seed)
        c = dict(DTU_MODEL_CONF)
        if model_conf is not None:
            c.update({k: dict(model_conf[k]) for k in DTU_MODEL_CONF if k in model_conf})
        with contextlib.redirect_stdout(io.StringIO()):
            self.nerf = fields_mod.NeRF(**c["nerf"]).to(device)
            self.udf = fields_mod.UDFNetwork(**c["udf_network"]).to(device)
            self.var = fields_mod.SingleVarianceNetwork(**c["variance_network"]).to(device)
            self.color = fields_mod.ResidualRenderingNetwork(**c["rendering_network"]).to(device)
            self.beta = fields_mod.BetaNetwork(**c["beta_network"]).to(device)
        tc = dict(learning_rate=5e-4, learning_rate_geo=1e-4, igr_weight=0.1, igr_ns_weight=0.0, mask_weight=0.0,
                  sparse_weight=0.0)
        tc.update(train_conf or {})
        self.tc = tc
        geo = list(self.udf.parameters())
        other = list(self.var.parameters()) + list(self.color.parameters()) + list(self.beta.parameters())
        nerf = list(self.nerf.parameters())
        self.param_groups = [geo, other, nerf]
        groups = [{'params': geo, 'lr': tc["learning_rate_geo"]}, {'params': other}, {'params': nerf}]
        if fused_adam:
            from .optim import FusedAdam
            self.optimizer = FusedAdam(groups, lr=tc["learning_rate"])
        else:
            self.optimizer = torch.optim.Adam(groups, lr=tc["learning_rate"])
        self.renderer = renderer_cls(self.nerf, self.udf, self.var, self.color, self.beta, **renderer_conf)
        lc = dict(color_base_weight=0.01, color_weight=1.0, color_pixel_weight=0.0, color_patch_weight=0.0,
                  pixel_loss_type="l1", patch_loss_type="ssim", h_patch_size=3)
        lc.update(color_loss_conf or {})
        self.lc = lc
        with contextlib.redirect_stdout(io.StringIO()):
            self.color_loss = loss_cls(**lc)
        self.data_parallel = data_parallel
        self.status_every = 100
        self._beta_flag = True
        self.fuse_loss = not data_parallel
        self._one = {}
        self.defer_sums_reduce = True
        import os
        self.fuse_blend_loss = os.environ.get("NUDF_FUSE_BLEND_LOSS", "1") != "0"
        if data_parallel:
            self.renderer.data_parallel = True
            self.renderer.defer_loss_sums = True
            self.color_loss.set_data_parallel(True)
            def seg(m):
                e = m.engine() if hasattr(m, "engine") else None
                ps = list(e.params()) if e is not None else list(m.parameters())
                assert {id(p) for p in ps} == {id(p) for p in m.parameters()}
                return ps, e
            self.bucket = nudf_dist.GradBucket([(other_scalars(self.var, self.beta), None), seg(self.color), seg(self.udf),
                                                seg(self.nerf)], device=device)

    def modules(self):
        return dict(nerf=self.nerf, udf=self.udf, var=self.var, color=self.color, beta=self.beta)

    def enable_graph(self, eager_steps=2):
        self.graphed = GraphedStep(self, eager_steps=eager_steps)
        return self.graphed

    def loss_weights(self):
        lw = self.color_loss.weights
        tc = self.tc
        lw.set(igr=tc["igr_weight"], igr_ns=tc["igr_ns_weight"], sparse=tc["sparse_weight"], mask=tc["mask_weight"])
        return lw

    def loss(self, batch, cos_anneal_ratio=1.0, flip_saturation=1.0, blend=None, perturb_overwrite=-1):
        tc, lc = self.tc, self.lc
        w = self.loss_weights().device(batch["rays_o"].device)
        kw = {}
        if blend is not None and lc["color_pixel_weight"] > 0:
            kw = dict(color_maps=blend["color_maps"], w2cs=blend["w2cs"], intrinsics=blend["intrinsics"],
                      query_c2w=blend["query_c2w"],
                      rays_uv=batch["rays_uv"].clone() if lc["color_patch_weight"] > 0 else None)
            if "ref_cam" in blend:
                kw["patch_cams"] = (blend["ref_cam"], blend["src_cam"])
        defer, defer_r = self.renderer.defer_loss_sums, self.renderer.defer_sums_reduce
        if self.fuse_loss:
            self.renderer.defer_loss_sums = True
            self.renderer.defer_sums_reduce = self.defer_sums_reduce
        try:
            out = self.renderer.render(batch["rays_o"], batch["rays_d"], batch["near"], batch["far"],
                                       flip_saturation=flip_saturation, cos_anneal_ratio=cos_anneal_ratio,
                                       perturb_overwrite=perturb_overwrite, **kw)
        finally:
            self.renderer.defer_loss_sums, self.renderer.defer_sums_reduce = defer, defer_r
        weight_sum = out["weight_sum"]
        pixel_mask = batch["mask"] if tc["mask_weight"] > 0 else None
        if (self.fuse_blend_loss and "_loss_sums" in out and not self.data_parallel and tc["mask_weight"] <= 0
                and out["patch_mask"] is not None
                and self.color_loss.blend_fusable(out["color_base"], out["color"], batch["true_rgb"], out["color_pixel"],
                                                  pixel_mask, out["patch_colors"], batch.get("gt_patch_colors"))):
            sums = out.pop("_loss_sums")
            r = self.color_loss.blend_step_loss(out["color_base"], out["color"], batch["true_rgb"], out["color_pixel"],
                                                out["patch_colors"], batch["gt_patch_colors"], out["patch_mask"], weight_sum,
                                                sums, float(weight_sum.shape[0]), w)
            out["gradient_error"], out["gradient_error_near_surface"], out["sparse_error"] = r[6], r[7], r[8]
            return r[0], out
        patch_mask = None
        if out["patch_mask"] is not None:
            patch_mask = (out["patch_mask"].float()[:, None] * (weight_sum > 0.5).float()) > 0.
        cargs = (out["color_base"], out["color"], batch["true_rgb"], out["color_pixel"], pixel_mask, out["patch_colors"],
                 batch.get("gt_patch_colors"), patch_mask)
        bce_sum = None
        if tc["mask_weight"] > 0:
            bce_sum = torch.nn.functional.binary_cross_entropy(weight_sum.clip(1e-3, 1.0 - 1e-3), batch["mask"],
                                                               reduction="sum")
        if "_loss_sums" in out and not self.data_parallel:
            sums = out.pop("_loss_sums")
            if bce_sum is None and self.color_loss.fusable(out["color_base"], out["color"], batch["true_rgb"],
                                                           out["color_pixel"], out["patch_colors"]):
                from .loss.loss import _StepLossFn
                loss, _, _, _, ge, gens, se = _StepLossFn.apply(
                    out["color_base"], out["color"], batch["true_rgb"], pixel_mask, sums, float(weight_sum.shape[0]), w)
                out["gradient_error"], out["gradient_error_near_surface"], out["sparse_error"] = ge, gens, se
                return loss, out
            ge, gens, se = self.renderer.errors_from_sums(sums, weight_sum.shape[0])
            out["gradient_error"], out["gradient_error_near_surface"], out["sparse_error"] = ge, gens, se
            cl = self.color_loss(*cargs)
            mask_loss = bce_sum / float(weight_sum.numel()) if bce_sum is not None else None
        elif "_loss_sums" in out:
            parts = [out.pop("_loss_sums")]
            fused = self.color_loss.fusable(out["color_base"], out["color"], batch["true_rgb"], out["color_pixel"],
                                            out["patch_colors"])
            if fused:
                parts.append(self.color_loss.local_sums(out["color_base"], out["color"], batch["true_rgb"], pixel_mask))
            if bce_sum is not None:
                parts.append(torch.stack([bce_sum, torch.full_like(bce_sum, float(weight_sum.numel()))]))
            packed = nudf_dist.all_reduce_sum(torch.cat([p.reshape(-1) for p in parts]))
            ge, gens, se = self.renderer.errors_from_sums(packed[:5], weight_sum.shape[0])
            out["gradient_error"], out["gradient_error_near_surface"], out["sparse_error"] = ge, gens, se
            k = 5
            if fused:
                cl = self.color_loss.from_global_sums(out["color_base"], out["color"], batch["true_rgb"], pixel_mask,
                                                      packed[k:k + 3])
                k += 3
            else:
                cl = self.color_loss(*cargs)
            mask_loss = packed[k] / packed[k + 1] if bce_sum is not None else None
        else:
            cl = self.color_loss(*cargs)
            mask_loss = bce_sum / float(weight_sum.numel()) if bce_sum is not None else None
        loss = cl["loss"] + out["gradient_error_near_surface"] * w[LW["igr_ns"]] \
            + out["sparse_error"] * w[LW["sparse"]] + out["gradient_error"] * w[LW["igr"]]
        if mask_loss is not None:
            loss = loss + mask_loss * w[LW["mask"]]
        return loss, out

    def step(self, batch, **kw):
        loss, out = self.loss(batch, **kw)
        self.optimizer.zero_grad(set_to_none=True)
        one = self._one.get(loss.device)
        if one is None or one.dtype != loss.dtype:
            one = self._one[loss.device] = torch.ones((), device=loss.device, dtype=loss.dtype)
        with torch.autograd.set_multithreading_enabled(not SINGLE_THREAD_BACKWARD):
            loss.backward(gradient=one)
        if self.data_parallel:
            self.bucket.all_reduce()
        self.optimizer.step()
        return loss.detach(), {k: (v.detach() if torch.is_tensor(v) else v) for k, v in out.items()}

    def iteration(self, source, iter_step, schedules, image_perm=None, batch_size=512, num_src=8):
        schedules.apply_learning_rates(self.optimizer, iter_step)
        a = schedules.at(iter_step)
        self.color_loss.set_color_weights(a["color_base_weight"], a["color_weight"], a["color_pixel_weight"],
                                          a["color_patch_weight"])
        self.lc.update(color_pixel_weight=a["color_pixel_weight"], color_patch_weight=a["color_patch_weight"])
        self.tc.update(igr_ns_weight=a["igr_ns_weight"], sparse_weight=a["sparse_weight"])
        n = source.n_images
        img_idx = int(image_perm[iter_step % len(image_perm)]) if image_perm is not None else iter_step % n
        s = source.gen_random_rays_patches_at(img_idx, batch_size, crop_patch=a["color_patch_weight"] > 0.0,
                                              h_patch_size=self.color_loss.h_patch_size, with_near_far=True)
        data = s["rays"]
        batch = dict(rays_o=data[:, :3], rays_d=data[:, 3:6], true_rgb=data[:, 6:9], mask=(data[:, 9:10] > 0.5).float(),
                     near=s["near"], far=s["far"], rays_uv=s["rays_ndc_uv"], gt_patch_colors=s["rays_patch_color"])
        blend = None
        if a["color_pixel_weight"] > 0.0 or a["color_patch_weight"] > 0.0:
            ref_c2w, src_c2ws, src_intr, src_images, _ = source.get_ref_src_info(img_idx, num_src)
            blend = dict(color_maps=src_images, w2cs=source.src_w2cs(img_idx, num_src), intrinsics=src_intr, query_c2w=ref_c2w)
        stepper = self.graphed if getattr(self, "graphed", None) is not None else self.step
        loss, out = stepper(batch, cos_anneal_ratio=a["cos_anneal_ratio"], flip_saturation=a["flip_saturation"],
                            blend=blend)
        self._trainability_toggles(out, iter_step)
        if self.status_every and iter_step % self.status_every == 0:
            self.check_finite(loss)
        return loss, out, s

    def check_finite(self, loss=None):
        if not self.data_parallel:
            return self.renderer.check_finite()
        import torch.distributed as dist
        bits = self.renderer.status(clear=True)
        if loss is not None and not bool(torch.isfinite(loss.detach()).all()):
            from neuraludf_amd import _lib as _l
            bits |= _l.STATUS_NONFINITE_LOSS
        if dist.is_available() and dist.is_initialized() and dist.get_world_size() > 1:
            dev = self.renderer._device()
            t = torch.tensor([float((bits >> b) & 1) for b in range(3)], device=dev if dist.get_backend() == "nccl" else "cpu")
            dist.all_reduce(t, op=dist.ReduceOp.MAX)
            bits = sum(int(v) << b for b, v in enumerate(t.tolist()))
        if bits:
            from neuraludf_amd import _lib
            raise FloatingPointError("NeuralUDF renderer (some rank of the ray-sharded job): " + _lib.status_text(bits))

    def _trainability_toggles(self, out, iter_step):
        var_p = getattr(self.var, "variance", None)
        beta_p = getattr(self.beta, "beta", None)
        if (self._beta_flag and beta_p is not None and not beta_p.requires_grad and var_p is not None
                and var_p.requires_grad):
            variance, beta = float(out["variance"].mean()), float(out["beta"].reshape(-1)[0])
            if variance < 2 * beta and variance < 0.01:
                self.beta.set_beta_trainable()
                self._beta_flag = False
        if var_p is not None and var_p.requires_grad is False and iter_step > 20000:
            self.var.set_trainable()

    def extract_udf_mesh(self, resolution=256, world_space=False, scale_mat=None, dist_threshold_ratio=1.0, **clean):
        from . import meshing
        if world_space and scale_mat is None:
            raise ValueError("world_space=True needs scale_mat (the dataset's scale_mats_np[0])")
        return meshing.extract_udf_mesh(self.udf, resolution, dist_threshold_ratio=dist_threshold_ratio,
                                        scale_mat=scale_mat if world_space else None, **clean)

    @torch.no_grad()
    def render_image(self, source, img_idx, resolution_level=4, chunk=65536, cos_anneal_ratio=1.0):
        rays_o, rays_d = source.gen_rays_at(img_idx, resolution_level=resolution_level)
        Hh, Ww, _ = rays_o.shape
        rays_o, rays_d = rays_o.reshape(-1, 3).contiguous(), rays_d.reshape(-1, 3).contiguous()
        outs = {"color": [], "depth": [], "normals": []}
        for i in range(0, rays_o.shape[0], chunk):
            o, d = rays_o[i:i + chunk], rays_d[i:i + chunk]
            near, far = source.near_far_from_sphere(o, d)
            r = self.renderer.render(o, d, near, far, cos_anneal_ratio=cos_anneal_ratio, perturb_overwrite=0,
                                     flip_saturation=1.0)
            outs["color"].append(r["color"]); outs["depth"].append(r["depth"].reshape(-1)); outs["normals"].append(r["normals"])
        return {"color": torch.cat(outs["color"]).reshape(Hh, Ww, 3), "depth": torch.cat(outs["depth"]).reshape(Hh, Ww),
                "normals": torch.cat(outs["normals"]).reshape(Hh, Ww, 3)}
```

Before: 19.72 million.

## Fold last merge_points into upsample kernel and small fills into coarse start

The final upsample pass can now also merge the coarse and new samples and write the merged z values, points and colour-network input rows. It keeps the new samples in dynamic LDS, so the separate nudf_merge_points launch is no longer needed. Separately, a per-step scratch buffer is zeroed and NaN-poisoned inside the coarse_start kernel, and small fills such as the deferred sums NaN fill draw from it instead of launching their own fill kernels. The aim is fewer tiny kernel launches per train step, at the cost of extra LDS per upsample block and a more involved scratch-lifetime protocol.

```diff
diff --git a/include/nudf.h b/include/nudf.h
--- a/include/nudf.h
+++ b/include/nudf.h
@@ -186,6 +186,11 @@
 int nudf_merge_points(const float* z, const float* z_new, int N, int M, int K, float* z_out, const float* rays_o,
                       const float* rays_d, const float* sample_dist, float* pts, float* xrows, int ldx, int xcols,
                       void* stream);
+typedef struct NudfUpsampleTail {
+  float* z_out; float* pts; float* xrows;
+  int32_t ldx, xcols;
+} NudfUpsampleTail;
+int nudf_upsample_merge_points(const NudfUpsample* args, const NudfUpsampleTail* tail, void* stream);
 
 typedef struct NudfPixelBlend {
   const float* pts;
@@ -278,6 +283,9 @@
                   float* z, float* sample_dist, void* stream);
 int nudf_coarse_start(const float* near, const float* far, int nf_stride, const float* t_rand, int center, int N, int S,
                       float* z, float* sample_dist, const float* rays_o, const float* rays_d, float* pts, void* stream);
+int nudf_coarse_start_scratch(const float* near, const float* far, int nf_stride, const float* t_rand, int center, int N,
+                              int S, float* z, float* sample_dist, const float* rays_o, const float* rays_d, float* pts,
+                              void* scratch, int zero_words, int nan_words, void* stream);
 int nudf_outside_z(const float* far, int f_stride, const float* lin, int N, int n_out, int n_samples,
                    float* z_out, void* stream);
 int nudf_ray_points(const float* rays_o, const float* rays_d, const float* z, const float* sample_dist, int N,
diff --git a/neuraludf_amd/_lib.py b/neuraludf_amd/_lib.py
--- a/neuraludf_amd/_lib.py
+++ b/neuraludf_amd/_lib.py
@@ -94,6 +94,10 @@
                 ("z_merged", c_fp), ("udf_merged", c_fp), ("merge_K", i32)]
 
 
+class UpsampleTail(C.Structure):
+    _fields_ = [("z_out", c_fp), ("pts", c_fp), ("xrows", c_fp), ("ldx", i32), ("xcols", i32)]
+
+
 class PixelBlend(C.Structure):
     _fields_ = [("pts", c_fp), ("logits", c_fp), ("nl", i32), ("proj", c_fp), ("imgs", c_fp),
                 ("P", i32), ("V", i32), ("H", i32), ("W", i32), ("pix", c_fp), ("img_layout", i32)]
@@ -224,6 +228,7 @@
 SYMBOLS = [
     "nudf_version", "nudf_last_error", "nudf_set_status_flag", "nudf_status_flag", "nudf_gemm_nn", "nudf_set_gemm_variant", "nudf_gemm_tn", "nudf_gemm_tn_grouped", "nudf_gemm_tn_grouped_workspace", "nudf_gemm_tn_grouped_plan", "nudf_set_tn_flags", "nudf_patch_metric", "nudf_set_tn_debug", "nudf_composite_fwd",
     "nudf_composite_bwd", "nudf_partial_sums", "nudf_composite_colour_finish", "nudf_set_composite_blocked", "nudf_upsample", "nudf_merge", "nudf_merge_points", "nudf_coarse_z", "nudf_coarse_start", "nudf_outside_z",
+    "nudf_upsample_merge_points", "nudf_coarse_start_scratch",
     "nudf_ray_points", "nudf_posenc", "nudf_posenc_vjp", "nudf_copy_cols", "nudf_add_cols",
     "nudf_udf_grad_seed", "nudf_udf_head_bwd", "nudf_signed_colsum", "nudf_sigmoid_head_bwd",
     "nudf_weightnorm_pack", "nudf_weightnorm_unpack_grad",
@@ -260,6 +265,8 @@
     "nudf_coarse_z": [_P, _P, _I, _P, _I, _I, _P, _P, _P],
     "nudf_coarse_start": [_P, _P, _I, _P, _I, _I, _I, _P, _P, _P, _P, _P, _P],
     "nudf_merge_points": [_P, _P, _I, _I, _I, _P, _P, _P, _P, _P, _P, _I, _I, _P],
+    "nudf_upsample_merge_points": [C.POINTER(Upsample), C.POINTER(UpsampleTail), _P],
+    "nudf_coarse_start_scratch": [_P, _P, _I, _P, _I, _I, _I, _P, _P, _P, _P, _P, _P, _I, _I, _P],
     "nudf_outside_z": [_P, _I, _P, _I, _I, _I, _P, _P],
     "nudf_ray_points": [_P, _P, _P, _P, _I, _I, _I, _P, _P],
     "nudf_posenc": [_P, _I, _I, _P, _I, _I, _F, _I, _P, _I, _F, _P, _I, _F, _P],
diff --git a/neuraludf_amd/csrc/rays_embed.hip b/neuraludf_amd/csrc/rays_embed.hip
--- a/neuraludf_amd/csrc/rays_embed.hip
+++ b/neuraludf_amd/csrc/rays_embed.hip
@@ -43,8 +43,10 @@
 __global__ __launch_bounds__(256) void coarse_start_kernel(const float* near, const float* far, int nf_stride,
                                                            const float* t_rand, int center, int N, int S, float* z,
                                                            float* sample_dist, const float* __restrict__ o,
-                                                           const float* __restrict__ d, float* __restrict__ pts) {
+                                                           const float* __restrict__ d, float* __restrict__ pts,
+                                                           uint32_t* __restrict__ scratch, int zero_words, int nan_words) {
   const int idx = blockIdx.x * blockDim.x + threadIdx.x;
+  for (int i = idx; i < zero_words + nan_words; i += gridDim.x * blockDim.x) scratch[i] = i < zero_words ? 0u : 0x7fc00000u;
   if (idx < N * S) {
     const int r = idx / S, s = idx - r * S;
     const float nr = near[r * nf_stride], fr = far[r * nf_stride];
@@ -84,8 +86,22 @@
     return (int)hipErrorInvalidValue;
   }
   hipLaunchKernelGGL(coarse_start_kernel, dim3(nblocks((long long)N * S, 256)), dim3(256), 0, (hipStream_t)stream, near, far,
-                     nf_stride, t_rand, center, N, S, z, sample_dist, rays_o, rays_d, pts);
+                     nf_stride, t_rand, center, N, S, z, sample_dist, rays_o, rays_d, pts, (uint32_t*)nullptr, 0, 0);
   NUDF_CHECK_LAUNCH("nudf_coarse_start");
+  return 0;
+}
+extern "C" int nudf_coarse_start_scratch(const float* near, const float* far, int nf_stride, const float* t_rand, int center,
+                                         int N, int S, float* z, float* sample_dist, const float* rays_o, const float* rays_d,
+                                         float* pts, void* scratch, int zero_words, int nan_words, void* stream) {
+  if (N <= 0 || S < 2 || zero_words < 0 || nan_words < 0 || (!scratch && zero_words + nan_words > 0)) {
+    nudf_set_error("nudf_coarse_start_scratch: N >= 1, S >= 2, word counts >= 0 (0 without a scratch) required",
+                   hipErrorInvalidValue);
+    return (int)hipErrorInvalidValue;
+  }
+  hipLaunchKernelGGL(coarse_start_kernel, dim3(nblocks((long long)N * S, 256)), dim3(256), 0, (hipStream_t)stream, near, far,
+                     nf_stride, t_rand, center, N, S, z, sample_dist, rays_o, rays_d, pts, (uint32_t*)scratch, zero_words,
+                     nan_words);
+  NUDF_CHECK_LAUNCH("nudf_coarse_start_scratch");
   return 0;
 }
 
diff --git a/neuraludf_amd/csrc/upsample.hip b/neuraludf_amd/csrc/upsample.hip
--- a/neuraludf_amd/csrc/upsample.hip
+++ b/neuraludf_amd/csrc/upsample.hip
@@ -3,6 +3,11 @@
 
 #define UP_MAX_M 512
 #define UP_NC (UP_MAX_M / 64)
+
+__device__ __forceinline__ void merge_points_ray(const float* a, const float* b, float* out, float* pl, int ray, int l, int M,
+                                                 int K, float ox, float oy, float oz, float dx, float dy, float dz, float sd,
+                                                 float* __restrict__ zo, float* __restrict__ pts, float* __restrict__ xrows,
+                                                 int ldx, int xcols);
 
 namespace up_fast {
 #include "upsample_body.inc"
@@ -13,8 +18,9 @@
 }
 #pragma clang fp contract(fast)
 
-extern "C" int nudf_upsample(const NudfUpsample* args, void* stream) {
-  const NudfUpsample& p = *args;
+static size_t up_static_lds(int nc) { return (size_t)3 * 4 * 64 * (nc <= 4 ? nc : 8) * sizeof(float); }
+
+static int up_launch(const NudfUpsample& p, const NudfUpsampleTail& t, const char* who, void* stream) {
   if (p.N <= 0) return 0;
   if (p.M < 2 || p.M > UP_MAX_M || p.K < 1) {
     nudf_set_error("nudf_upsample: 2 <= M <= 512 and K >= 1 required", hipErrorInvalidValue);
@@ -28,26 +34,45 @@
   dim3 grid((p.N + 3) / 4), block(256);
   hipStream_t st = (hipStream_t)stream;
   const int nc = (p.M + 63) / 64;
+  const size_t lds = t.z_out ? (size_t)4 * (p.K + 4 * (p.M + p.K)) * sizeof(float) : 0;
+  if (t.z_out && (!t.pts || lds + up_static_lds(nc) > 64 * 1024 || (t.xrows && (t.xcols < 3 || t.xcols > t.ldx)))) {
+    nudf_set_error("nudf_upsample_merge_points: pts, 3 <= xcols <= ldx and 16 (K + 4 (M + K)) bytes of LDS next to the "
+                   "kernel's own required", hipErrorInvalidValue);
+    return (int)hipErrorInvalidValue;
+  }
   int32_t* status = nudf_status_flag();
   if (p.mode & NUDF_UP_NOCONTRACT) {
     switch (nc) {
-      case 1: hipLaunchKernelGGL(up_exact::upsample_kernel<1>, grid, block, 0, st, p, status); break;
-      case 2: hipLaunchKernelGGL(up_exact::upsample_kernel<2>, grid, block, 0, st, p, status); break;
-      case 3: hipLaunchKernelGGL(up_exact::upsample_kernel<3>, grid, block, 0, st, p, status); break;
-      case 4: hipLaunchKernelGGL(up_exact::upsample_kernel<4>, grid, block, 0, st, p, status); break;
-      default: hipLaunchKernelGGL(up_exact::upsample_kernel<8>, grid, block, 0, st, p, status); break;
+      case 1: hipLaunchKernelGGL(up_exact::upsample_kernel<1>, grid, block, lds, st, p, t, status); break;
+      case 2: hipLaunchKernelGGL(up_exact::upsample_kernel<2>, grid, block, lds, st, p, t, status); break;
+      case 3: hipLaunchKernelGGL(up_exact::upsample_kernel<3>, grid, block, lds, st, p, t, status); break;
+      case 4: hipLaunchKernelGGL(up_exact::upsample_kernel<4>, grid, block, lds, st, p, t, status); break;
+      default: hipLaunchKernelGGL(up_exact::upsample_kernel<8>, grid, block, lds, st, p, t, status); break;
     }
   } else {
     switch (nc) {
-      case 1: hipLaunchKernelGGL(up_fast::upsample_kernel<1>, grid, block, 0, st, p, status); break;
-      case 2: hipLaunchKernelGGL(up_fast::upsample_kernel<2>, grid, block, 0, st, p, status); break;
-      case 3: hipLaunchKernelGGL(up_fast::upsample_kernel<3>, grid, block, 0, st, p, status); break;
-      case 4: hipLaunchKernelGGL(up_fast::upsample_kernel<4>, grid, block, 0, st, p, status); break;
-      default: hipLaunchKernelGGL(up_fast::upsample_kernel<8>, grid, block, 0, st, p, status); break;
-    }
-  }
-  NUDF_CHECK_LAUNCH("nudf_upsample");
+      case 1: hipLaunchKernelGGL(up_fast::upsample_kernel<1>, grid, block, lds, st, p, t, status); break;
+      case 2: hipLaunchKernelGGL(up_fast::upsample_kernel<2>, grid, block, lds, st, p, t, status); break;
+      case 3: hipLaunchKernelGGL(up_fast::upsample_kernel<3>, grid, block, lds, st, p, t, status); break;
+      case 4: hipLaunchKernelGGL(up_fast::upsample_kernel<4>, grid, block, lds, st, p, t, status); break;
+      default: hipLaunchKernelGGL(up_fast::upsample_kernel<8>, grid, block, lds, st, p, t, status); break;
+    }
+  }
+  NUDF_CHECK_LAUNCH(who);
   return 0;
+}
+
+extern "C" int nudf_upsample(const NudfUpsample* args, void* stream) {
+  const NudfUpsampleTail none = {nullptr, nullptr, nullptr, 0, 0};
+  return up_launch(*args, none, "nudf_upsample", stream);
+}
+
+extern "C" int nudf_upsample_merge_points(const NudfUpsample* args, const NudfUpsampleTail* tail, void* stream) {
+  if (!tail || !tail->z_out) {
+    nudf_set_error("nudf_upsample_merge_points: tail->z_out required", hipErrorInvalidValue);
+    return (int)hipErrorInvalidValue;
+  }
+  return up_launch(*args, *tail, "nudf_upsample_merge_points", stream);
 }
 
 __global__ __launch_bounds__(256) void merge_kernel(const float* __restrict__ za, const float* __restrict__ ua,
@@ -98,6 +123,53 @@
                      K, z_out, udf_out);
   NUDF_CHECK_LAUNCH("nudf_merge");
   return 0;
+}
+
+__device__ __forceinline__ void merge_points_ray(const float* a, const float* b, float* out, float* pl, int ray, int l, int M,
+                                                 int K, float ox, float oy, float oz, float dx, float dy, float dz, float sd,
+                                                 float* __restrict__ zo, float* __restrict__ pts, float* __restrict__ xrows,
+                                                 int ldx, int xcols) {
+  const int S = M + K;
+  for (int i = l; i < M; i += 64) {
+    const float v = a[i];
+    int lo = 0, hi = K;
+    while (lo < hi) {
+      const int mid = (lo + hi) >> 1;
+      if (b[mid] < v) lo = mid + 1; else hi = mid;
+    }
+    out[i + lo] = v;
+  }
+  for (int j = l; j < K; j += 64) {
+    const float v = b[j];
+    int lo = 0, hi = M;
+    while (lo < hi) {
+      const int mid = (lo + hi) >> 1;
+      if (a[mid] <= v) lo = mid + 1; else hi = mid;
+    }
+    out[j + lo] = v;
+  }
+  __builtin_amdgcn_wave_barrier();
+  __threadfence_block();
+  const size_t ob = (size_t)ray * S;
+  for (int i = l; i < S; i += 64) {
+    float t = out[i];
+    zo[ob + i] = t;
+    const float dist = (i < S - 1) ? (out[i + 1] - t) : sd;
+    t = t + dist * 0.5f;
+    const float px = ox + dx * t, py = oy + dy * t, pz = oz + dz * t;
+    pts[(ob + i) * 3 + 0] = px;
+    pts[(ob + i) * 3 + 1] = py;
+    pts[(ob + i) * 3 + 2] = pz;
+    pl[3 * i + 0] = px; pl[3 * i + 1] = py; pl[3 * i + 2] = pz;
+  }
+  if (xrows) {
+    __builtin_amdgcn_wave_barrier();
+    __threadfence_block();
+    for (int e = l; e < S * xcols; e += 64) {
+      const int r = e / xcols, c = e - r * xcols;
+      xrows[(ob + r) * (size_t)ldx + c] = (c < 3) ? pl[3 * r + c] : 0.0f;
+    }
+  }
 }
 
 __global__ __launch_bounds__(256) void merge_points_kernel(const float* __restrict__ za, const float* __restrict__ zb,
@@ -119,49 +191,9 @@
   for (int j = l; j < K; j += 64) b[j] = zb[(size_t)ray * K + j];
   __builtin_amdgcn_wave_barrier();
   __threadfence_block();
-  for (int i = l; i < M; i += 64) {
-    const float v = a[i];
-    int lo = 0, hi = K;
-    while (lo < hi) {
-      const int mid = (lo + hi) >> 1;
-      if (b[mid] < v) lo = mid + 1; else hi = mid;
-    }
-    out[i + lo] = v;
-  }
-  for (int j = l; j < K; j += 64) {
-    const float v = b[j];
-    int lo = 0, hi = M;
-    while (lo < hi) {
-      const int mid = (lo + hi) >> 1;
-      if (a[mid] <= v) lo = mid + 1; else hi = mid;
-    }
-    out[j + lo] = v;
-  }
-  __builtin_amdgcn_wave_barrier();
-  __threadfence_block();
   const float ox = ro[ray * 3 + 0], oy = ro[ray * 3 + 1], oz = ro[ray * 3 + 2];
   const float dx = rd[ray * 3 + 0], dy = rd[ray * 3 + 1], dz = rd[ray * 3 + 2];
-  const float sd = sample_dist[0];
-  const size_t ob = (size_t)ray * S;
-  for (int i = l; i < S; i += 64) {
-    float t = out[i];
-    zo[ob + i] = t;
-    const float dist = (i < S - 1) ? (out[i + 1] - t) : sd;
-    t = t + dist * 0.5f;
-    const float px = ox + dx * t, py = oy + dy * t, pz = oz + dz * t;
-    pts[(ob + i) * 3 + 0] = px;
-    pts[(ob + i) * 3 + 1] = py;
-    pts[(ob + i) * 3 + 2] = pz;
-    pl[3 * i + 0] = px; pl[3 * i + 1] = py; pl[3 * i + 2] = pz;
-  }
-  if (xrows) {
-    __builtin_amdgcn_wave_barrier();
-    __threadfence_block();
-    for (int e = l; e < S * xcols; e += 64) {
-      const int r = e / xcols, c = e - r * xcols;
-      xrows[(ob + r) * (size_t)ldx + c] = (c < 3) ? pl[3 * r + c] : 0.0f;
-    }
-  }
+  merge_points_ray(a, b, out, pl, ray, l, M, K, ox, oy, oz, dx, dy, dz, sample_dist[0], zo, pts, xrows, ldx, xcols);
 }
 
 extern "C" int nudf_merge_points(const float* z, const float* z_new, int N, int M, int K, float* z_out, const float* rays_o,
diff --git a/neuraludf_amd/csrc/upsample_body.inc b/neuraludf_amd/csrc/upsample_body.inc
--- a/neuraludf_amd/csrc/upsample_body.inc
+++ b/neuraludf_amd/csrc/upsample_body.inc
@@ -64,7 +64,8 @@
 }
 
 template <int NC>
-__global__ __launch_bounds__(256) void upsample_kernel(NudfUpsample p, int32_t* status) {
+__global__ __launch_bounds__(256) void upsample_kernel(NudfUpsample p, NudfUpsampleTail tl, int32_t* status) {
+  extern __shared__ float s_tail[];
   __shared__ __attribute__((aligned(16))) float s_z[4][NC * 64];
   __shared__ __attribute__((aligned(16))) float s_cdf[4][NC * 64];
   __shared__ float s_u[4][NC * 64];
@@ -285,6 +286,7 @@
 
   if (dbg)
     for (int i = l; i < M; i += 64) dbg[6 * M + i] = cdf[i];
+  float* tb = tl.z_out ? s_tail + wave * (p.K + 4 * (M + p.K)) : nullptr;
   for (int k = l; k < p.K; k += 64) {
     const float uq = p.u[k];
     int lo = 0, hi = M;
@@ -301,6 +303,7 @@
     const float t = (uq - c0) / den;
     const float zn = b0 + t * (b1 - b0);
     p.z_new[(size_t)ray * p.K + k] = zn;
+    if (tb) tb[k] = zn;
     if (status && !(fabsf(zn) <= 3.0e38f)) atomicOr(status, NUDF_STATUS_NONFINITE_SAMPLES);
     if (p.pts_new) {
       const size_t o = ((size_t)ray * p.K + k) * 3;
@@ -309,4 +312,10 @@
       p.pts_new[o + 2] = oz + dz * zn;
     }
   }
-}
+  if (tb) {
+    __builtin_amdgcn_wave_barrier();
+    __threadfence_block();
+    merge_points_ray(zs, tb, tb + p.K, tb + p.K + M + p.K, ray, l, M, p.K, ox, oy, oz, dx, dy, dz, sdist, tl.z_out, tl.pts,
+                     tl.xrows, tl.ldx, tl.xcols);
+  }
+}
diff --git a/neuraludf_amd/mlp.py b/neuraludf_amd/mlp.py
--- a/neuraludf_amd/mlp.py
+++ b/neuraludf_amd/mlp.py
@@ -136,6 +136,73 @@
     fn()
     e.record()
     PROFILE.append((name, flops, s, e, detail or name, nbytes, xflops))
+
+
+FOLD_FILLS = os.environ.get("NUDF_FOLD_FILLS", "1") == "1"
+
+
+class StepScratch:
+    ZERO_WORDS, NAN_WORDS = 32, 8
+
+    def __init__(self, dev):
+        self.buf = torch.zeros(self.ZERO_WORDS + self.NAN_WORDS, device=dev)
+        self.begin()
+
+    def begin(self):
+        self.armed = False
+        self.nz = self.nn = 0
+
+    def carve(self, n, nan):
+        n4 = (n + 3) // 4 * 4
+        if not self.armed:
+            return None
+        if nan:
+            if self.nn + n4 > self.NAN_WORDS:
+                return None
+            o = self.ZERO_WORDS + self.nn
+            self.nn += n4
+        else:
+            if self.nz + n4 > self.ZERO_WORDS:
+                return None
+            o = self.nz
+            self.nz += n4
+        return self.buf[o:o + n]
+
+
+_SCRATCH = None
+
+
+def step_scratch(dev):
+    s = _SCRATCH
+    return s if (s is not None and FOLD_FILLS and s.buf.device == dev) else None
+
+
+def step_zeros(n, dev):
+    s = step_scratch(dev)
+    t = s.carve(n, False) if s is not None else None
+    return t if t is not None else torch.zeros(n, device=dev)
+
+
+def step_nans(n, dev):
+    s = step_scratch(dev)
+    return s.carve(n, True) if s is not None else None
+
+
+class step_scratch_scope:
+
+    def __init__(self, scratch):
+        self.s = scratch
+
+    def __enter__(self):
+        global _SCRATCH
+        self.prev, _SCRATCH = _SCRATCH, self.s
+        if self.s is not None:
+            self.s.begin()
+
+    def __exit__(self, *exc):
+        global _SCRATCH
+        _SCRATCH = self.prev
+        return False
 
 
 def call_timed(cls, detail, nbytes, name, *args, units=0.0):
@@ -1061,7 +1128,8 @@
         ex_fly = second and EX_FLY and PRECISION != "fp32" and not _isblk(X[L]) and CHAIN_TILE in (0, 32, 64)
         tn2 = (TN_F16X2 and PRECISION == "bf16x3" and TN_SPLIT and grouped and head4_path and not _isblk(X[L]) and not _is16(X[L])
                and CHAIN_TILE in (0, 32, 64))
-        amax = torch.zeros(2, device=dev) if tn2 else None
+        amax = step_zeros(2, dev) if tn2 else None
+        self.last_amax = amax
         bsc = _sweep_dtype("bwd") == "f16x2"
         TA = torch.empty(pad_rows(P) // 32, device=dev) if (bsc and second) else None
         if second:
@@ -1404,7 +1472,8 @@
              ptr(Dv[n - 1]), Dv[n - 1].shape[1])
         dVIN = _buf(P, self.view[0].inp, dev, zero=False)
         tn2 = TN_F16X2 and PRECISION == "bf16x3" and TN_SPLIT and not _is16(HV[1]) and COLOR_TILE in (0, 32, 64)
-        amax = torch.zeros(1, device=dev) if tn2 else None
+        amax = step_zeros(1, dev) if tn2 else None
+        self.last_amax = amax
         cb = ChainBuilder(P, "LOAD", k8(plv.out), tile_rows=COLOR_TILE, site=("col_bwd_view", _memo_token(self)))
         cb.init_load(Dv[n - 1], Dv[n - 1].shape[1])
         if tn2:
diff --git a/neuraludf_amd/models/udf_renderer_blending.py b/neuraludf_amd/models/udf_renderer_blending.py
--- a/neuraludf_amd/models/udf_renderer_blending.py
+++ b/neuraludf_amd/models/udf_renderer_blending.py
@@ -6,11 +6,12 @@
 import os
 
 from .. import _lib
-from .._lib import Composite, CompositeGrad, Upsample, call, ptr
+from .._lib import Composite, CompositeGrad, Upsample, UpsampleTail, call, ptr
 from .. import dist as nudf_dist
 from .. import mlp
 
 UPSAMPLE_FLAGS = int(os.environ.get("NUDF_UP_FLAGS", str(512 | 1024 | 2048 | 4096)))
+FOLD_LAST_MERGE = os.environ.get("NUDF_FOLD_LAST_MERGE", "1") == "1"
 FUSE_SCALARS = os.environ.get("NUDF_FUSE_SCALARS", "1") == "1"
 FUSE_COLOUR = os.environ.get("NUDF_FUSE_COLOUR", "1") == "1"
 
@@ -74,7 +75,12 @@
                 diag.append(d)
         if c.get("defer_sums"):
             a.defer_sums = 1
-            sums.fill_(float("nan"))
+            poisoned = mlp.step_nans(5, dev)
+            if poisoned is not None:
+                sums = poisoned
+                a.sums = ptr(sums)
+            else:
+                sums.fill_(float("nan"))
             sums._nudf_ws = (ws, (N + 3) // 4)
         ST = weights.shape[1]
         mlp.call_timed("composite", "composite_fwd N=%d S=%d" % (N, ST), (48.0 if color is not None else 24.0) * N * ST + 68.0 * N,
@@ -309,7 +315,7 @@
         return self.udf_network.udf_only(pts).reshape(N, M)
 
     def _upsample(self, rays_o, rays_d, z, udf, sample_dist, k, mode, inv_s, beta, gamma, gamma_dev=None, dbg=None,
-                  pending=None):
+                  pending=None, last=False):
         dev = rays_o.device
         a = Upsample()
         keep = None
@@ -329,8 +335,19 @@
         z_new = torch.empty(N, k, device=dev)
         pts_new = torch.empty(N * k, 3, device=dev)
         a.z_new, a.pts_new, a.dbg = ptr(z_new), ptr(pts_new), ptr(dbg)
-        mlp.call_timed("upsample", "upsample N=%d M=%d K=%d" % (N, M, k), float(N) * (8 * M + 4 * k + 8 * (M + k) + 24),
-                       "nudf_upsample", a, units=N * M)
+        self._mid = None
+        nc = (M + 63) // 64
+        if last and FOLD_LAST_MERGE and 16 * (k + 4 * (M + k)) + 3072 * (nc if nc <= 4 else 8) <= 65536:
+            zo, pts, feat, F, ld = self._last_buffers(N, M + k, dev)
+            tl = UpsampleTail()
+            tl.z_out, tl.pts, tl.ldx, tl.xcols = ptr(zo), ptr(pts), ld, ld - F
+            tl.xrows = (ptr(feat) + 4 * F) if feat is not None else None
+            mlp.call_timed("upsample", "upsample N=%d M=%d K=%d" % (N, M, k), float(N) * (8 * M + 4 * k + 8 * (M + k) + 24),
+                           "nudf_upsample_merge_points", a, tl, units=N * M)
+            self._mid = (zo, pts, feat)
+        else:
+            mlp.call_timed("upsample", "upsample N=%d M=%d K=%d" % (N, M, k), float(N) * (8 * M + 4 * k + 8 * (M + k) + 24),
+                           "nudf_upsample", a, units=N * M)
         if pending is not None:
             return z_new, pts_new, z, udf
         return z_new, pts_new
@@ -344,13 +361,7 @@
              ptr(uo))
         return zo, uo
 
-    def _merge_last(self, rays_o, rays_d, z, z_new, sample_dist, for_render=False):
-        if not for_render:
-            return self._merge(z, None, z_new, None)[0]
-        N, M = z.shape
-        K = z_new.shape[1]
-        S = M + K
-        dev = z.device
+    def _last_buffers(self, N, S, dev):
         zo = torch.empty(N, S, device=dev)
         pts = torch.empty(N * S, 3, device=dev)
         ceng = self.color_network.engine()
@@ -358,6 +369,17 @@
         feat = None
         if ld >= F + 3:
             feat = torch.empty(mlp.pad_rows(N * S), ld, device=dev)
+        return zo, pts, feat, F, ld
+
+    def _merge_last(self, rays_o, rays_d, z, z_new, sample_dist, for_render=False):
+        if not for_render:
+            return self._merge(z, None, z_new, None)[0]
+        mid = getattr(self, "_mid", None)
+        if mid is not None:
+            return mid[0]
+        N, M = z.shape
+        K = z_new.shape[1]
+        zo, pts, feat, F, ld = self._last_buffers(N, M + K, z.device)
         call("nudf_merge_points", ptr(z.contiguous()), ptr(z_new), N, M, K, ptr(zo), ptr(rays_o), ptr(rays_d),
              ptr(sample_dist), ptr(pts), (ptr(feat) + 4 * F) if feat is not None else None, ld, ld - F)
         self._mid = (zo, pts, feat)
@@ -374,10 +396,11 @@
             gamma = float(np.clip(20 * 2 ** (steps - i), 20, 320))
             if pend is None:
                 z_new, pts_new = self._upsample(rays_o, rays_d, z_vals, udf, sample_dist, k, 0, 64 * 2 ** i,
-                                                64 * 2 ** (i + 1), gamma)
+                                                64 * 2 ** (i + 1), gamma, last=for_render and i + 1 == steps)
             else:
                 z_new, pts_new, z_vals, udf = self._upsample(rays_o, rays_d, None, None, sample_dist, k, 0, 64 * 2 ** i,
-                                                             64 * 2 ** (i + 1), gamma, pending=pend)
+                                                             64 * 2 ** (i + 1), gamma, pending=pend,
+                                                             last=for_render and i + 1 == steps)
             if i + 1 == steps:
                 return self._merge_last(rays_o, rays_d, z_vals, z_new, sample_dist, for_render)
             pend = (z_vals, udf, z_new, self.udf_network.udf_only(pts_new).reshape(N, k))
@@ -402,10 +425,10 @@
         i = steps - 1
         if pend is None:
             z_new, _ = self._upsample(rays_o, rays_d, z_vals, udf, sample_dist, k, 0, 64 * 2 ** i, 64 * 2 ** (i + 1),
-                                      20 if i < 4 else 10)
+                                      20 if i < 4 else 10, last=for_render)
         else:
             z_new, _, z_vals, udf = self._upsample(rays_o, rays_d, None, None, sample_dist, k, 0, 64 * 2 ** i,
-                                                   64 * 2 ** (i + 1), 20 if i < 4 else 10, pending=pend)
+                                                   64 * 2 ** (i + 1), 20 if i < 4 else 10, pending=pend, last=for_render)
         return self._merge_last(rays_o, rays_d, z_vals, z_new, sample_dist, for_render)
 
     def render_core_outside(self, rays_o, rays_d, z_out, sample_dist, z_in=None):
@@ -563,8 +586,15 @@
         sample_dist = torch.empty(1, device=dev)
         want_pts0 = z_vals_override is None and self.n_importance > 0 and self.upsampling_type in ('classical', 'mix')
         pts0 = torch.empty(N * self.n_samples, 3, device=dev) if want_pts0 else None
-        call("nudf_coarse_start", ptr(near), ptr(far), nf_stride, ptr(t_rand), 1, N, self.n_samples, ptr(z_vals),
-             ptr(sample_dist), ptr(rays_o), ptr(rays_d), ptr(pts0))
+        scratch = mlp.step_scratch(dev)
+        if scratch is not None:
+            call("nudf_coarse_start_scratch", ptr(near), ptr(far), nf_stride, ptr(t_rand), 1, N, self.n_samples,
+                 ptr(z_vals), ptr(sample_dist), ptr(rays_o), ptr(rays_d), ptr(pts0), ptr(scratch.buf), scratch.ZERO_WORDS,
+                 scratch.NAN_WORDS)
+            scratch.armed = True
+        else:
+            call("nudf_coarse_start", ptr(near), ptr(far), nf_stride, ptr(t_rand), 1, N, self.n_samples, ptr(z_vals),
+                 ptr(sample_dist), ptr(rays_o), ptr(rays_d), ptr(pts0))
         z_out = None
         if self.n_outside > 0:
             z_out = torch.empty(N, self.n_outside, device=dev)
diff --git a/neuraludf_amd/train.py b/neuraludf_amd/train.py
--- a/neuraludf_amd/train.py
+++ b/neuraludf_amd/train.py
@@ -8,6 +8,7 @@
 import torch
 
 from . import dist as nudf_dist
+from . import mlp
 from ._lib import LW, LW_COUNT
 from .loss.loss import ColorLoss
 from .models import fields
@@ -171,6 +172,7 @@
         tr.loss_weights().bind(sc.dev[sc.LOSSW:sc.LOSSW + LW_COUNT])
         if blend is not None:
             tr.color_loss.prefill_constants(dev)
+        tr.step_scratch(dev)
         g = torch.cuda.CUDAGraph()
         torch.cuda.synchronize()
         import gc
@@ -231,6 +233,7 @@
         self._beta_flag = True
         self.fuse_loss = not data_parallel
         self._one = {}
+        self._scratch = {}
         self.defer_sums_reduce = True
         import os
         self.fuse_blend_loss = os.environ.get("NUDF_FUSE_BLEND_LOSS", "1") != "0"
@@ -342,6 +345,18 @@
         return loss, out
 
     def step(self, batch, **kw):
+        with mlp.step_scratch_scope(self.step_scratch(batch["rays_o"].device)):
+            return self._step(batch, **kw)
+
+    def step_scratch(self, dev):
+        if dev.type != "cuda":
+            return None
+        sc = self._scratch.get(dev)
+        if sc is None:
+            sc = self._scratch[dev] = mlp.StepScratch(dev)
+        return sc
+
+    def _step(self, batch, **kw):
         loss, out = self.loss(batch, **kw)
         self.optimizer.zero_grad(set_to_none=True)
         one = self._one.get(loss.device)
```

Result: no change. 19.78 million (median of 3 runs) (+0.3%).
